# Kolkir/mono_slam_framework

Hardware: AMD Instinct MI355X
Metric: frame-pairs/sec (extract+match) (higher is better)
Workload: dtype u8; 1 GPU; ORB extract+match, 1280x720 pairs, 1024 pairs/GPU/step resident in HBM, ratio 0.60; pairs_per_gpu=1024, width=1280, height=720, synth_mode=0, overflow_pairs=0, ranks=1, rccl_ranks=0

## Files before the change

### include/msf_abi.h

```cpp
#ifndef MSF_ABI_H
#define MSF_ABI_H

#include <stddef.h>
#include <stdint.h>

#ifdef __cplusplus
extern "C" {
#endif

#define MSF_ABI_VERSION 4

typedef struct msf_handle msf_handle;

typedef enum msf_status {
  MSF_OK = 0,
  MSF_ERR_INVALID_ARG = -1,
  MSF_ERR_HIP = -2,
  MSF_ERR_UNSUPPORTED = -3,
  MSF_ERR_CAPACITY = -4,
  MSF_ERR_IO = -5
} msf_status;

typedef enum msf_kind {
  MSF_KIND_ORB = 0,
// ... 4 lines not shown
#define MSF_FLAG_PROFILE 2u
#define MSF_FLAG_KEEP_DEBUG 4u
#define MSF_FLAG_LEVEL_SIZE_MUL_INV 32u
#define MSF_FLAG_NO_FRAME_CACHE 16u
#define MSF_FLAG_FAST_STREAM 64u
#define MSF_FLAG_LOFTR_F32 128u
#define MSF_FLAG_BLUR_SUM256 256u
#define MSF_FLAG_FAST_DENSE 8u

typedef struct msf_config {
  uint32_t struct_size;
  int32_t kind;
  int32_t device;
  float threshold;
  int32_t image_width;
  int32_t image_height;
  int32_t max_batch_pairs;
  uint32_t flags;
  const char* weights_path;
} msf_config;

typedef struct msf_image {
  const uint8_t* data;
  int32_t width, height;
  int64_t stride;
} msf_image;

typedef struct msf_match {
  int32_t x1, y1, x2, y2;
} msf_match;

typedef struct msf_keypoint {
  float x, y;
  float response;
  float angle;
  int32_t octave;
  int32_t lx, ly;
  int32_t fast_score;
} msf_keypoint;

int msf_abi_version(void);
void msf_default_config(msf_config* cfg, int kind);

int msf_weights_info(const char* path, uint64_t* digest, int32_t* n_tensors, int64_t* n_floats);
int msf_convert_weights(const char* src_path, const char* dst_blob_path);

int msf_create(const msf_config* cfg, msf_handle** out);
void msf_destroy(msf_handle* h);
int msf_set_threshold(msf_handle* h, float value);
const char* msf_last_error(const msf_handle* h);

int msf_match_pair(msf_handle* h, const msf_image* a, const msf_image* b,
                   msf_match* out, int32_t cap, int32_t* n_out);
int msf_frame_cache_stats(msf_handle* h, uint64_t* hits, uint64_t* misses, int32_t* capacity);
int msf_match_batch(msf_handle* h, int32_t n_pairs, const msf_image* a, const msf_image* b,
                    msf_match* out, int32_t cap_per_pair, int32_t* n_out);

int msf_match_batch_device(msf_handle* h, int32_t n_pairs, const uint8_t* d_a, const uint8_t* d_b,
                           int64_t frame_stride, int64_t row_stride,
                           msf_match* d_out, int32_t cap_per_pair, int32_t* d_n_out, void* stream);

int msf_extract_device(msf_handle* h, int32_t n_frames, const uint8_t* d_frames, int64_t frame_stride,
                       int64_t row_stride, int32_t first_slot, void* stream);
int msf_match_slots_device(msf_handle* h, int32_t n_pairs, const int32_t* d_slot_a, const int32_t* d_slot_b,
                           msf_match* d_out, int32_t cap_per_pair, int32_t* d_n_out, void* stream);

int msf_set_mappoints(msf_handle* h, int32_t map_slot, const int32_t* keys, int32_t n_keys);
int msf_count_mappoint_matches_device(msf_handle* h, int32_t n_pairs, const msf_match* d_matches,
                                      int32_t cap_per_pair, const int32_t* d_n_matches, const int32_t* d_map_a,
                                      const int32_t* d_map_b, int32_t* d_num_mp, void* stream);

int msf_store_frame(msf_handle* h, int32_t slot, const msf_image* img);
int msf_match_one_to_many(msf_handle* h, int32_t query_slot, int32_t n, const int32_t* slots, int32_t* num_matches,
                          int32_t* num_mp, msf_match* out, int32_t cap_per_pair);

#define MSF_MODEL_HOMOGRAPHY 0
#define MSF_MODEL_FUNDAMENTAL 1
int msf_check_hypotheses(msf_handle* h, int32_t model, int32_t n_hyp, const float* m21, const float* m12,
                         int32_t n_matches, const msf_match* matches, float sigma, float* scores, int32_t* best,
                         uint8_t* best_inliers);

typedef struct msf_ransac_result {
  uint32_t struct_size;
  uint32_t reserved;
  float* m21;
  float* m12;
  float* fn;
  float* null_vec;
  float* scores;
  int32_t* best;
  uint8_t* best_inliers;
  float* T1;
  float* T2;
} msf_ransac_result;
int msf_find_models(msf_handle* h, int32_t n_matches, const msf_match* matches, int32_t n_hyp, const int32_t* sets,
                    float sigma, msf_ransac_result* homography, msf_ransac_result* fundamental);
typedef struct msf_ransac_batch {
  uint32_t struct_size;
  uint32_t reserved;
  int32_t* sets;
  msf_ransac_result homography;
  msf_ransac_result fundamental;
} msf_ransac_batch;
int msf_find_models_device(msf_handle* h, int32_t n_lists, const msf_match* d_matches, int32_t cap_per_pair,
                           const int32_t* d_n_out, int32_t n_hyp, uint64_t seed, float sigma,
                           msf_ransac_batch* out, void* stream);

int msf_render_match_image(msf_handle* h, const msf_image* f1, const msf_image* f2, const msf_match* matches,
                           int32_t n_matches, const uint8_t* has_mp1, const uint8_t* has_mp2, uint8_t* out_rgb,
                           int64_t out_stride);

int msf_pack_matches_device(msf_handle* h, int32_t n_pairs, const msf_match* d_in, int32_t cap_per_pair,
                            const int32_t* d_n_out, msf_match* d_packed, int32_t* d_offsets, void* stream);

typedef struct msf_multi msf_multi;
int msf_multi_create(const msf_config* cfg, int32_t n_devices, const int32_t* device_ids, msf_multi** out);
void msf_multi_destroy(msf_multi* m);
int32_t msf_multi_device_count(const msf_multi* m);
msf_handle* msf_multi_handle(msf_multi* m, int32_t shard);
int msf_multi_set_threshold(msf_multi* m, float value);
const char* msf_multi_last_error(const msf_multi* m);
void msf_multi_shard_range(int32_t n_pairs, int32_t n_shards, int32_t shard, int32_t* first, int32_t* count);
int msf_multi_match_batch(msf_multi* m, int32_t n_pairs, const msf_image* a, const msf_image* b, msf_match* out,
                          int32_t cap_per_pair, int32_t* n_out);
int msf_multi_match_batch_device(msf_multi* m, const int32_t* n_pairs, const uint8_t* const* d_a,
                                 const uint8_t* const* d_b, int64_t frame_stride, int64_t row_stride,
                                 msf_match* const* d_out, int32_t cap_per_pair, int32_t* const* d_n_out);

typedef struct msf_gather msf_gather;
int msf_gather_unique_id(uint8_t* id128);
int msf_gather_create(int32_t device, int32_t rank, int32_t n_ranks, const uint8_t* id128, int32_t pairs_per_rank,
                      int64_t cap_records, msf_gather** out);
void msf_gather_destroy(msf_gather* g);
const char* msf_gather_last_error(const msf_gather* g);
int msf_gather_plan(int32_t n_ranks, int32_t pairs_per_rank, const int32_t* all_offsets, int64_t cap_records,
                    int32_t* totals, int64_t* recv_first);
int msf_gather_matches_device(msf_gather* g, const msf_match* d_packed, const int32_t* d_offsets, int32_t* d_all_offsets,
                              msf_match* d_recv, int32_t* totals, void* stream);


typedef enum msf_debug_what {
  MSF_DBG_LEVEL_SIZES = 0,
  MSF_DBG_LEVEL_PIXELS = 1,
  MSF_DBG_FAST_CANDS = 2,
  MSF_DBG_KEYPOINTS = 3,
  MSF_DBG_DESCRIPTORS = 4,
  MSF_DBG_STAGE1 = 5,
  MSF_DBG_LOFTR_CONF = 6,
  MSF_DBG_LOFTR_FEAT = 7,
  MSF_DBG_FAST_TAU = 8,
  MSF_DBG_WALK_MODE = 10,
  MSF_DBG_LOFTR_ACT = 9,
  MSF_DBG_LOFTR_TOK = 11,
  MSF_DBG_ORB_MATCH_FORM = 12
} msf_debug_what;
int msf_debug_get(msf_handle* h, int32_t what, int32_t slot, int32_t level,
                  void* host_out, size_t cap_bytes, size_t* n_bytes);
int msf_debug_loftr_head(msf_handle* h, int32_t n_pairs, const float* d_feat0, const float* d_feat1,
                         msf_match* d_out, int32_t cap_per_pair, int32_t* d_n_out, void* stream);

int msf_debug_loftr_transformer(msf_handle* h, int32_t n_pairs, int32_t first_block, int32_t n_blocks,
                                const float* d_in0, const float* d_in1, float* d_out0, float* d_out1, void* stream);

int msf_debug_loftr_backbone(msf_handle* h, int32_t n, const uint8_t* d_a, const uint8_t* d_b, int64_t frame_stride,
                             int64_t row_stride, int32_t act_image, float* d_tok_a, float* d_tok_b, void* stream);

int msf_debug_orb_set_features(msf_handle* h, int32_t slot, int32_t n, const msf_keypoint* kp, const uint8_t* desc);

int msf_debug_orb_tail(msf_handle* h, int32_t n_frames, const uint8_t* d_frames, int64_t frame_stride, int64_t row_stride,
                       int32_t first_slot, const int32_t* counts, const int32_t* cands, int32_t form);

int msf_stage_times(msf_handle* h, const char** names, float* ms, int32_t cap);

#ifdef __cplusplus
}
#endif
#endif
```

### mono_slam_framework_amd/_lib.py

```python
import ctypes as C
import os

import numpy as np

from . import build as _build

MSF_OK = 0
MSF_ERR_INVALID_ARG = -1
MSF_ERR_HIP = -2
MSF_ERR_UNSUPPORTED = -3
MSF_ERR_CAPACITY = -4
MSF_ERR_IO = -5

MSF_KIND_ORB = 0
MSF_KIND_LOFTR = 1

MSF_FLAG_BLUR_TIE_HALF_UP = 1
MSF_FLAG_PROFILE = 2
MSF_FLAG_KEEP_DEBUG = 4
MSF_FLAG_FAST_DENSE = 8
MSF_FLAG_NO_FRAME_CACHE = 16
MSF_FLAG_LEVEL_SIZE_MUL_INV = 32
MSF_FLAG_FAST_STREAM = 64
MSF_FLAG_LOFTR_F32 = 128
MSF_FLAG_BLUR_SUM256 = 256

(DBG_LEVEL_SIZES, DBG_LEVEL_PIXELS, DBG_FAST_CANDS, DBG_KEYPOINTS, DBG_DESCRIPTORS, DBG_STAGE1,
 DBG_LOFTR_CONF, DBG_LOFTR_FEAT, DBG_FAST_TAU, DBG_LOFTR_ACT, DBG_WALK_MODE, DBG_LOFTR_TOK,
 DBG_ORB_MATCH_FORM) = range(13)

ABI_SYMBOLS = ["msf_abi_version", "msf_default_config", "msf_create", "msf_destroy", "msf_set_threshold",
               "msf_last_error", "msf_match_pair", "msf_match_batch", "msf_match_batch_device",
               "msf_extract_device", "msf_match_slots_device", "msf_pack_matches_device", "msf_debug_get",
               "msf_debug_loftr_head", "msf_debug_loftr_transformer", "msf_debug_loftr_backbone",
               "msf_debug_orb_set_features", "msf_debug_orb_tail",
               "msf_stage_times", "msf_set_mappoints", "msf_count_mappoint_matches_device",
               "msf_store_frame", "msf_match_one_to_many", "msf_check_hypotheses",
               "msf_find_models", "msf_find_models_device",
               "msf_render_match_image", "msf_weights_info", "msf_convert_weights",
               "msf_frame_cache_stats", "msf_multi_create", "msf_multi_destroy", "msf_multi_device_count",
               "msf_multi_handle", "msf_multi_set_threshold", "msf_multi_last_error", "msf_multi_shard_range",
               "msf_multi_match_batch", "msf_multi_match_batch_device",
               "msf_gather_unique_id", "msf_gather_create", "msf_gather_destroy", "msf_gather_last_error",
               "msf_gather_plan", "msf_gather_matches_device"]

INITIALIZER_SYMBOLS = ["msf_initializer_version", "msf_reconstruct", "msf_reconstruct_device"]

LOCAL_MAPPING_SYMBOLS = ["msf_local_mapping_version", "msf_new_points", "msf_new_points_device", "msf_create_map_points"]

PNP_SYMBOLS = ["msf_pnp_version", "msf_pnp_ransac", "msf_pnp_ransac_device"]

POSE_SYMBOLS = ["msf_pose_version", "msf_pose_optimize", "msf_pose_optimize_device"]

BA_SYMBOLS = ["msf_ba_version", "msf_bundle_adjust", "msf_bundle_adjust_device"]

GLOBAL_BA_SYMBOLS = ["msf_global_ba_version", "msf_global_ba_tile_rows", "msf_global_bundle_adjust",
                     "msf_global_bundle_adjust_device"]
GBA_MAX_FREE_CAMS = 1024

TRACKING_SYMBOLS = ["msf_tracking_version", "msf_frustum", "msf_frustum_device", "msf_claim_points_device",
                    "msf_search_local_points"]
MSF_POINT_BAD, MSF_POINT_SEEN = 1, 2
MSF_SEARCH_KEEP_ON_DEVICE = 1


class Config(C.Structure):
    _fields_ = [("struct_size", C.c_uint32), ("kind", C.c_int32), ("device", C.c_int32), ("threshold", C.c_float),
                ("image_width", C.c_int32), ("image_height", C.c_int32), ("max_batch_pairs", C.c_int32),
                ("flags", C.c_uint32), ("weights_path", C.c_char_p)]


class Image(C.Structure):
    _fields_ = [("data", C.c_void_p), ("width", C.c_int32), ("height", C.c_int32), ("stride", C.c_int64)]


class RansacResult(C.Structure):
    _fields_ = [("struct_size", C.c_uint32), ("reserved", C.c_uint32), ("m21", C.c_void_p), ("m12", C.c_void_p),
                ("fn", C.c_void_p), ("null_vec", C.c_void_p), ("scores", C.c_void_p), ("best", C.c_void_p),
                ("best_inliers", C.c_void_p), ("T1", C.c_void_p), ("T2", C.c_void_p)]


class RansacBatch(C.Structure):
    _fields_ = [("struct_size", C.c_uint32), ("reserved", C.c_uint32), ("sets", C.c_void_p),
                ("homography", RansacResult), ("fundamental", RansacResult)]


class MotionParams(C.Structure):
    _fields_ = [("struct_size", C.c_uint32), ("reserved", C.c_uint32), ("K", C.c_float * 9), ("sigma", C.c_float),
                ("min_triangulated", C.c_int32), ("min_parallax", C.c_float)]


MOTION_ARRAYS = [("ok", "int32", "list", ()), ("model", "int32", "list", ()), ("R21", "float32", "list", (9,)),
                 ("t21", "float32", "list", (3,)), ("points", "float32", "list", ("cap", 3)),
                 ("triangulated", "uint8", "list", ("cap",)), ("n_cand", "int32", "list", ()),
                 ("cand_R", "float32", "list", (8, 9)), ("cand_t", "float32", "list", (8, 3)),
                 ("cand_good", "int32", "list", (8,)), ("cand_parallax", "float32", "list", (8,)),
                 ("winner", "int32", "list", ())]


class MotionResult(C.Structure):
    _fields_ = [("struct_size", C.c_uint32), ("reserved", C.c_uint32)] + [(a[0], C.c_void_p) for a in MOTION_ARRAYS]


class View(C.Structure):
    _fields_ = [("Rcw", C.c_float * 9), ("tcw", C.c_float * 3), ("fx", C.c_float), ("fy", C.c_float),
                ("cx", C.c_float), ("cy", C.c_float)]


class NewPointsParams(C.Structure):
    _fields_ = [("struct_size", C.c_uint32), ("reserved", C.c_uint32), ("max_cos_parallax", C.c_double),
                ("chi2", C.c_double)]


NEW_POINT_DTYPE = np.dtype([("match", "<i4"), ("x", "<f4"), ("y", "<f4"), ("z", "<f4")])
NEW_POINTS_ARRAYS = [("n_new", "int32", "list", ()), ("packed", NEW_POINT_DTYPE, "list", ("cap",)),
                     ("status", "uint8", "list", ("cap",)), ("points", "float32", "list", ("cap", 3)),
                     ("hom", "float32", "list", ("cap", 4)), ("cos_parallax", "float64", "list", ("cap",))]


class NewPointsResult(C.Structure):
    _fields_ = [("struct_size", C.c_uint32), ("reserved", C.c_uint32)] + [(a[0], C.c_void_p) for a in NEW_POINTS_ARRAYS]


class PnpParams(C.Structure):
    _fields_ = [("struct_size", C.c_uint32), ("reserved", C.c_uint32), ("fx", C.c_float), ("fy", C.c_float),
                ("cx", C.c_float), ("cy", C.c_float), ("th2", C.c_float), ("min_inliers", C.c_int32),
                ("n_iterations", C.c_int32), ("max_records", C.c_int32), ("seed", C.c_uint64)]


PNP_ARRAYS = [("n_records", "int32", "list", ()), ("counts", "int32", "hyp", ()),
              ("iteration", "int32", "rec", ()), ("n_inliers", "int32", "rec", ()), ("refined_ok", "int32", "rec", ()),
              ("n_refined", "int32", "rec", ()), ("Tcw_best", "float32", "rec", (12,)), ("Tcw_refined", "float32", "rec", (12,)),
              ("inliers_best", "uint8", "rec", ("cap",)), ("inliers_refined", "uint8", "rec", ("cap",)),
              ("sets", "int32", "hyp", (4,)), ("pose_f64", "float64", "hyp", (12,)), ("cws", "float64", "hyp", (4, 3)),
              ("ut_tail", "float64", "hyp", (4, 12)), ("betas", "float64", "hyp", (3, 4)), ("rep_errors", "float64", "hyp", (3,)),
              ("pca", "float64", "hyp", (3, 3)),
              ("rec_pose_f64", "float64", "rec", (12,)), ("rec_cws", "float64", "rec", (4, 3)),
              ("rec_ut_tail", "float64", "rec", (4, 12)), ("rec_betas", "float64", "rec", (3, 4)),
              ("rec_rep_errors", "float64", "rec", (3,)), ("rec_pca", "float64", "rec", (3, 3))]


class PnpResult(C.Structure):
    _fields_ = [("struct_size", C.c_uint32), ("reserved", C.c_uint32)] + [(a[0], C.c_void_p) for a in PNP_ARRAYS]


def pnp_shapes(lists, n_iterations, max_records, cap):
    lead = {"list": (lists,), "hyp": (lists, n_iterations), "rec": (lists, max_records)}
    return {name: (lead[per] + tuple(cap if t == "cap" else t for t in tail), dt) for name, dt, per, tail in PNP_ARRAYS}


class PoseParams(C.Structure):
    _fields_ = [("struct_size", C.c_uint32), ("reserved", C.c_uint32), ("fx", C.c_float), ("fy", C.c_float),
                ("cx", C.c_float), ("cy", C.c_float), ("chi2", C.c_float)]


POSE_ARRAYS = [("n_good", "int32", "list", ()), ("Tcw", "float32", "list", (12,)), ("outliers", "uint8", "list", ("cap",)),
               ("n_edges", "int32", "list", ()), ("rounds_run", "int32", "list", ()), ("pose_f64", "float64", "list", (12,)),
               ("round_pose_f64", "float64", "round", (12,)), ("round_n_bad", "int32", "round", ()),
               ("round_iterations", "int32", "round", ()),
               ("it_trials", "int32", "it", ()), ("it_lambda_in", "float64", "it", ()), ("it_lambda_out", "float64", "it", ()),
               ("it_cost_in", "float64", "it", ()), ("it_cost_out", "float64", "it", ()), ("it_H", "float64", "it", (21,)),
               ("it_b", "float64", "it", (6,)), ("it_pose_out", "float64", "it", (7,))]


class PoseResult(C.Structure):
    _fields_ = [("struct_size", C.c_uint32), ("reserved", C.c_uint32)] + [(a[0], C.c_void_p) for a in POSE_ARRAYS]


def pose_shapes(lists, cap):
    lead = {"list": (lists,), "round": (lists, 4), "it": (lists, 4, 10)}
    return {name: (lead[per] + tuple(cap if t == "cap" else t for t in tail), dt) for name, dt, per, tail in POSE_ARRAYS}


class BaParams(C.Structure):
    _fields_ = [("struct_size", C.c_uint32), ("reserved", C.c_uint32), ("fx", C.c_float), ("fy", C.c_float),
                ("cx", C.c_float), ("cy", C.c_float), ("n_rounds", C.c_int32), ("iterations", C.c_int32 * 2),
                ("robust", C.c_int32 * 2), ("huber_delta2", C.c_double), ("chi2", C.c_double)]


BA_SLOTS = 64
BA_PROBLEM_DTYPE = np.dtype([("n_cams", "<i4"), ("n_points", "<i4"), ("n_edges", "<i4"), ("cam0", "<i4"), ("point0", "<i4"),
                             ("edge0", "<i4")])
# ... 176 lines not shown
```

### mono_slam_framework_amd/csrc/orb_kernels.hip

```cpp
#include <type_traits>
#include "orb_pipeline.h"

#include <math.h>
#include <stdlib.h>
#include <string.h>

#include "orb_blur_tiles.h"
#include "orb_pattern.h"

namespace msf {

constexpr int SW = TW + 2, SH = TH + 2;
constexpr int kTileCandCap = TW * TH / 4;
constexpr int kTileY0 = kEdge;

constexpr uint32_t kStatusOverflow = 1u;

__constant__ __attribute__((aligned(16))) signed char c_pattern[1024];
__constant__ uint32_t c_disc[2 * kDiscTasks];

__device__ __forceinline__ __amdgpu_buffer_rsrc_t uniform_rsrc(const void* p, uint32_t bytes) {
  const unsigned long long v = (unsigned long long)p;
  const uint32_t lo = (uint32_t)__builtin_amdgcn_readfirstlane((int)(uint32_t)v);
  const uint32_t hi = (uint32_t)__builtin_amdgcn_readfirstlane((int)(uint32_t)(v >> 32));
// ... 233 lines not shown
  const int txlo = max(-1, kLo - x0), txhi = min(TW, L.w - kLo - 1 - x0);
  const bool inner1 = txlo == -1 && txhi == TW && y0 - 1 >= kLo && y0 + TH < L.h - kLo;
  for (int i0 = 0; i0 < GPR * SH; i0 += kFastThreads) {
    const int i = i0 + tid;
    if (i0 + (tid & ~63) >= GPR * SH) continue;
    const int ic = i < GPR * SH ? i : GPR * SH - 1;
    const int sr = ic / GPR, gq = ic % GPR;
    const int ty = sr - 1, tx0 = 4 * gq - 4;
    const int b = ((ty + HY) * PW2 + tx0 + HX) >> 2;
    const uint32_t C = T[b], Lf = T[b - 1], Rt = T[b + 1];
    const uint32_t U = T[b - 3 * (PW2 / 4)], D = T[b + 3 * (PW2 / 4)];
    const uint32_t W3 = __builtin_amdgcn_alignbyte(C, Lf, 1);
    const uint32_t E3 = __builtin_amdgcn_alignbyte(Rt, C, 3);
    const uint32_t nC = ~C;
    const uint32_t l0 = __builtin_amdgcn_lerp(D, nC, 0), l4 = __builtin_amdgcn_lerp(E3, nC, 0);
    const uint32_t l8 = __builtin_amdgcn_lerp(U, nC, 0), l12 = __builtin_amdgcn_lerp(W3, nC, 0);
    const uint32_t b0 = __builtin_amdgcn_lerp(l0, lerp_bright, 0), b4 = __builtin_amdgcn_lerp(l4, lerp_bright, 0);
    const uint32_t b8 = __builtin_amdgcn_lerp(l8, lerp_bright, 0), b12 = __builtin_amdgcn_lerp(l12, lerp_bright, 0);
    const uint32_t n0 = __builtin_amdgcn_lerp(l0, lerp_not_dark, 0), n4 = __builtin_amdgcn_lerp(l4, lerp_not_dark, 0);
    const uint32_t n8 = __builtin_amdgcn_lerp(l8, lerp_not_dark, 0), n12 = __builtin_amdgcn_lerp(l12, lerp_not_dark, 0);
    uint32_t vm = 0;
    if (inner1) {
      vm = gq == 0 ? 0x80000000u : gq == GPR - 1 ? 0x00000080u : 0x80808080u;
      vm = i < GPR * SH ? vm : 0u;
    } else {
      const int gy = y0 + ty;
      int first = txlo - tx0, last = txhi - tx0;
      first = first < 0 ? 0 : first;
      last = last > 3 ? 3 : last;
      if (i < GPR * SH && gy >= kLo && gy < L.h - kLo && first <= last)
        vm = (0x80808080u << (8 * first)) & (0x80808080u >> (8 * (3 - last)));
    }
    const uint32_t cb = ((b0 | b8) & (b4 | b12)) & vm;
    const uint32_t cd = ~((n0 & n8) | (n4 & n12)) & vm;
    if (__ballot((cb | cd) != 0u) == 0ull) continue;
    const uint32_t e0 = (uint32_t)b << 2;
    const uint32_t slots = reserve_packed(__popc(cb) | (__popc(cd) << 16), &S_.nbd, lane);
    uint32_t k = slots & 0xFFFFu;
    if (cb & 0x80u) list1[k++] = (uint16_t)e0;
    if (cb & 0x8000u) list1[k++] = (uint16_t)(e0 + 1);
    if (cb & 0x800000u) list1[k++] = (uint16_t)(e0 + 2);
    if (cb & 0x80000000u) list1[k++] = (uint16_t)(e0 + 3);
    k = kList1Cap - 1 - (slots >> 16);
    if (cd & 0x80u) list1[k--] = (uint16_t)e0;
    if (cd & 0x8000u) list1[k--] = (uint16_t)(e0 + 1);
    if (cd & 0x800000u) list1[k--] = (uint16_t)(e0 + 2);
    if (cd & 0x80000000u) list1[k--] = (uint16_t)(e0 + 3);
  }
  __syncthreads();

  const uint32_t mb = S_.nbd & 0xFFFFu, md = S_.nbd >> 16;
  if (mb | md) {
    for (uint32_t i = tid; i < mb; i += kFastThreads) {
      const int e = list1[i];
      const int s = fast_score_pol<true>(&px[e], tau);
      if (s) sc[SCO + e] = (uint8_t)s;
    }
    for (uint32_t i = tid; i < md; i += kFastThreads) {
      const int e = list1[kList1Cap - 1 - i];
      const int s = fast_score_pol<false>(&px[e], tau);
      if (s) sc[SCO + e] = (uint8_t)s;
    }
    __syncthreads();

    const uint32_t* S = reinterpret_cast<const uint32_t*>(sc) + SCO / 4;
    constexpr int SPD = PW2 / 4;
    const int txlo3 = max(0, kEdge - x0), txhi3 = min(TW - 1, L.w - kEdge - 1 - x0);
    const bool inner3 = txlo3 == 0 && txhi3 == TW - 1;
    for (int i = tid; i < (TW / 4) * TH; i += kFastThreads) {
      const int ty = i / (TW / 4), j = i % (TW / 4);
      const int w = (ty + HY) * SPD + HX / 4 + j;
      const uint32_t C = S[w];
      uint32_t keep = 0;
      const int gy = y0 + ty;
      const bool live = C != 0 && gy >= kEdge && gy < L.h - kEdge;
      if (__ballot(live) == 0ull) continue;
      if (live) {
        const uint32_t Cl = S[w - 1], Cr = S[w + 1];
        const uint32_t U = S[w - SPD], Ul = S[w - SPD - 1], Ur = S[w - SPD + 1];
        const uint32_t D = S[w + SPD], Dl = S[w + SPD - 1], Dr = S[w + SPD + 1];
        keep = __builtin_amdgcn_lerp(C, ~__builtin_amdgcn_alignbyte(C, Cl, 3), 0);
        keep &= __builtin_amdgcn_lerp(C, ~__builtin_amdgcn_alignbyte(Cr, C, 1), 0);
        keep &= __builtin_amdgcn_lerp(C, ~U, 0);
        keep &= __builtin_amdgcn_lerp(C, ~__builtin_amdgcn_alignbyte(U, Ul, 3), 0);
        keep &= __builtin_amdgcn_lerp(C, ~__builtin_amdgcn_alignbyte(Ur, U, 1), 0);
        keep &= __builtin_amdgcn_lerp(C, ~D, 0);
        keep &= __builtin_amdgcn_lerp(C, ~__builtin_amdgcn_alignbyte(D, Dl, 3), 0);
        keep &= __builtin_amdgcn_lerp(C, ~__builtin_amdgcn_alignbyte(Dr, D, 1), 0);
        if (!inner3) {
          int first = txlo3 - 4 * j, last = txhi3 - 4 * j;
          first = first < 0 ? 0 : first;
          last = last > 3 ? 3 : last;
          keep &= first <= last ? (0x80808080u << (8 * first)) & (0x80808080u >> (8 * (3 - last))) : 0u;
        } else {
          keep &= 0x80808080u;
        }
        if (emit_min > 0u) {
          uint32_t ge = 0u;
#pragma unroll
          for (int b = 0; b < 4; b++)
            if (((C >> (8 * b)) & 0xFFu) >= emit_min) ge |= 0x80u << (8 * b);
          keep &= ge;
        }
      }
      const uint32_t mine = __popc(keep);
      uint32_t k = reserve_packed(mine, &S_.lcount, lane);
      const uint32_t key = ((uint32_t)gy << 16) | (uint32_t)(x0 + 4 * j);
      if (keep & 0x80u) llist[k++] = make_uint2(key, C & 0xFFu);
      if (keep & 0x8000u) llist[k++] = make_uint2(key + 1, (C >> 8) & 0xFFu);
      if (keep & 0x800000u) llist[k++] = make_uint2(key + 2, (C >> 16) & 0xFFu);
      if (keep & 0x80000000u) llist[k++] = make_uint2(key + 3, C >> 24);
    }
    __syncthreads();
    const uint32_t n = S_.lcount;
    if (hist) {
      uint32_t* const hl = hist + (size_t)(slot * kOrbLevels + l) * 256u;
      for (uint32_t i = tid; i < n; i += kFastThreads) atomicAdd(&hl[llist[i].y], 1u);
    } else if (n != 0) {
      if (tid == 0) S_.gbase = atomicAdd(&cand_cnt[slot * kOrbLevels + l], n);
      __syncthreads();
      const uint32_t base = S_.gbase;
      const uint2 cm = cmap[slot * kOrbLevels + l];
      uint32_t* outk = cand_key + cm.x;
      uint8_t* outs = cand_sc + cm.x;
      for (uint32_t i = tid; i < n; i += kFastThreads)
        if (base + i < cm.y) {
          const uint2 e = llist[i];
          outk[base + i] = e.x;
          outs[base + i] = (uint8_t)e.y;
        }
    }
  }
}

__global__ __launch_bounds__(kFastThreads) void k_fast(OrbGeometry g, FrameSrc src, const uint8_t* pyr,
                                                       uint32_t* cand_cnt, uint32_t* cand_key, uint8_t* cand_sc,
                                                       const uint2* cmap) {
  __shared__ FastSmem sm;
  int G;
  {
    const uint32_t total = gridDim.x, lin = blockIdx.x;
    const uint32_t xcd = lin & 7u, q = total >> 3, r = total & 7u;
    G = (int)(xcd * q + (xcd < r ? xcd : r) + (lin >> 3));
  }
  const int fi = G / g.total_tiles, bt = G - fi * g.total_tiles;
  int l = 0;
#pragma unroll
  for (int i = 1; i < kOrbLevels; i++)
    if (i < g.nlevels && bt >= g.lv[i].tile_base) l = i;
  fast_tile(g, src, pyr, fi, l, bt - g.lv[l].tile_base, kFastT, cand_cnt, cand_key, cand_sc, cmap, sm);
}

constexpr int kTauBins = 64;
constexpr int kQDone = kTauBins, kQTau = kTauBins + 1, kQFirst = kTauBins + 2, kQAll = kTauBins + 3;
constexpr int kQStat = kTauBins + 4;
constexpr uint32_t kQReady = 0x80000000u;
constexpr int RK = 16;
constexpr int kSGCap = 288, kSPCap = 256, kSHCap = 64, kSOCap = 64;
constexpr uint32_t kSGFlush = 32;
static_assert(kSGCap >= (int)kSGFlush + 256, "record list capacity");
constexpr int kFlushRows = 8;
static_assert(kFlushRows < RK - 5 && kFlushRows % 4 == 0, "ring too short for the flush interval");
constexpr int kTau2MarginPct = 200, kTau2MinStrips = 1;
constexpr int kTau2MarginPctMany = 150, kTau2ManyStrips = 8;

struct StreamSmem {
  __attribute__((aligned(16))) uint8_t px[RK * 256];
  __attribute__((aligned(16))) uint8_t sc[RK * 256];
  uint32_t g[kSGCap];
  uint16_t p[kSPCap];
  uint16_t h[kSHCap];
  uint32_t opk[kSOCap];
};
static_assert(sizeof(StreamSmem) == 10240, "16 waves per CU need 10 240 B per wave");

__device__ __forceinline__ int stream_score(const uint8_t* ring, uint32_t r0, uint32_t x, bool dark, int tau) {
  uint32_t rb[7];
#pragma unroll
  for (int d = 0; d < 7; d++) rb[d] = (((r0 + (uint32_t)(d + RK - 3)) & (uint32_t)(RK - 1)) << 8) + x;
  constexpr int dx[16] = {0, 1, 2, 3, 3, 3, 2, 1, 0, -1, -2, -3, -3, -3, -2, -1};
  constexpr int dy[16] = {3, 3, 2, 1, 0, -1, -2, -3, -3, -3, -2, -1, 0, 1, 2, 3};
  const uint32_t flip = dark ? 255u : 0u;
  int q[16];
#pragma unroll
  for (int k = 0; k < 16; k++) q[k] = (int)((uint32_t)ring[rb[dy[k] + 3] + dx[k]] ^ flip);
  const int v = (int)((uint32_t)ring[rb[3]] ^ flip);
  int m3[16];
#pragma unroll
  for (int k = 0; k < 16; k++) m3[k] = min(min(q[k], q[(k + 1) & 15]), q[(k + 2) & 15]);
  int W = -1;
#pragma unroll
  for (int k = 0; k < 16; k++) W = max(W, min(min(m3[k], m3[(k + 3) & 15]), m3[(k + 6) & 15]));
  const int A = W - v;
  return A > tau ? A - 1 : 0;
}

constexpr uint32_t kSpinMax = 1u << 19;

__device__ __forceinline__ uint32_t ld_agent(const uint32_t* p) {
  return __hip_atomic_load(p, __ATOMIC_RELAXED, __HIP_MEMORY_SCOPE_AGENT);
}
__device__ __forceinline__ void unit_stall(uint32_t* status, int slot, uint32_t* abort_word, int lane) {
  if (lane == 0) {
    atomicOr(&status[slot], kStatusOverflow);
    __hip_atomic_store(abort_word, 1u, __ATOMIC_RELAXED, __HIP_MEMORY_SCOPE_AGENT);
    atomicAdd(abort_word + 1, 1u);
  }
}

template <bool RESIZE>
__device__ __forceinline__ void walk_strip(StreamSmem& sm, const OrbGeometry& g, const FrameSrc& src, uint8_t* pyr,
                                           const uint32_t* __restrict__ tab, uint32_t* qstat, uint32_t* cand_cnt,
                                           uint32_t* cand_key, uint8_t* cand_sc, const uint2* cmap, uint32_t* status,
                                           uint32_t* abort_word, int margin_pct, int dyn, int chain, const int l, const int fi,
                                           const int ts) {
  const int lane = threadIdx.x;
  const bool quarter = (ts & 3) == 0;
  const OrbLevelInfo L = g.lv[l];
  const int slot = src.slot0 + fi, idx = slot * kOrbLevels + l;
  const int sy = ts / L.wk_nx, sx = ts - sy * L.wk_nx;
  uint32_t* const qs = qstat + (size_t)idx * kQStat;
  const int n_strips = L.wk_nx * L.wk_ny;
  const int qa = (n_strips + 3) >> 2;
  const bool count_me = dyn && quarter;

  const int xs = sx * L.wk_px;
  const int xb = xs + 4 * lane;
  const int R0 = sy * L.wk_rows, R1 = min(R0 + L.wk_rows, L.h);
  const int ya = RESIZE ? R0 : max(R0, kEdge), yb = RESIZE ? R1 : min(R1, L.h - kEdge);
  const int ox0 = sx == 0 ? 0 : xs + 4, ox1 = sx == L.wk_nx - 1 ? L.w : xs + 4 + L.wk_px;
  const int y0 = ya - 1;
  int pitch;
  const uint8_t* img = level_ptr(g, src, pyr, fi, l, &pitch);
  const int need_lo = RESIZE ? xs : max(ox0 - 4, xs);
  const int need_hi = sx == L.wk_nx - 1 ? pitch : (RESIZE ? xs + L.wk_px + 16 : ox1 + 4);
  const int xl = min(max(xb, need_lo & ~3), ((need_hi + 3) & ~3) - 4);
  const uint32_t xoff = (uint32_t)(xl + 4 <= pitch ? xl : pitch - 4);
  const int ylim = L.h - 1;
  const uint32_t pitch_u = uniform_u32((uint32_t)pitch);
  const __amdgpu_buffer_rsrc_t img_rs = uniform_rsrc(img, (uint32_t)L.h * (uint32_t)pitch);
#define LOAD_ROW(y_) ((uint32_t)__builtin_amdgcn_raw_buffer_load_b32(img_rs, xoff, (uint32_t)max(min((y_), ylim), 0) * pitch_u, 0))
  const bool early = !(chain && l > 0);
  uint32_t w0_ = 0, w1_ = 0, w2_ = 0, w3_ = 0, w4_ = 0, w5_ = 0, q0 = 0, q1 = 0, q2 = 0, q3 = 0;
  if (early) {
    w0_ = LOAD_ROW(y0 - 3); w1_ = LOAD_ROW(y0 - 2); w2_ = LOAD_ROW(y0 - 1); w3_ = LOAD_ROW(y0); w4_ = LOAD_ROW(y0 + 1);
    w5_ = LOAD_ROW(y0 + 2);
    q0 = LOAD_ROW(y0 + 3); q1 = LOAD_ROW(y0 + 4); q2 = LOAD_ROW(y0 + 5); q3 = LOAD_ROW(y0 + 6);
  }

  const bool need_q = dyn && !quarter && qa >= kTau2MinStrips;
  uint32_t qv = ld_agent(&qs[lane]);
  uint32_t qx = ld_agent(&qs[kTauBins + (lane & 3)]);
  {
    bool ready = false;
    for (uint32_t it = 0; it < kSpinMax; it++) {
      const uint32_t first = (uint32_t)__builtin_amdgcn_readlane((int)qx, kQFirst - kTauBins);
      const uint32_t done = (uint32_t)__builtin_amdgcn_readlane((int)qx, kQDone - kTauBins);
      ready = (first & kQReady) != 0u && (!need_q || done >= (uint32_t)qa);
      if (ready || ld_agent(abort_word) != 0u) break;
      __builtin_amdgcn_s_sleep(20);
      qv = ld_agent(&qs[lane]);
      qx = ld_agent(&qs[kTauBins + (lane & 3)]);
    }
    if (!ready) {
      unit_stall(status, slot, abort_word, lane);
      return;
    }
  }
  if (!early) {
    __builtin_amdgcn_fence(__ATOMIC_ACQUIRE, "agent");
    w0_ = LOAD_ROW(y0 - 3); w1_ = LOAD_ROW(y0 - 2); w2_ = LOAD_ROW(y0 - 1); w3_ = LOAD_ROW(y0); w4_ = LOAD_ROW(y0 + 1);
    w5_ = LOAD_ROW(y0 + 2);
    q0 = LOAD_ROW(y0 + 3); q1 = LOAD_ROW(y0 + 4); q2 = LOAD_ROW(y0 + 5); q3 = LOAD_ROW(y0 + 6);
  }
  int tv = (int)((uint32_t)__builtin_amdgcn_readlane((int)qx, kQFirst - kTauBins) & ~kQReady);
  tv = max(tv, (int)__builtin_amdgcn_readlane((int)qx, kQTau - kTauBins));
  if (need_q && tv > kFastT) {
    uint32_t c = qv;
#pragma unroll
    for (int o = 1; o < 64; o <<= 1) {
      const uint32_t up = __shfl_down(c, o);
      if (lane + o < 64) c += up;
    }
    const uint32_t mp = (qa >= kTau2ManyStrips && margin_pct == kTau2MarginPct) ? (uint32_t)kTau2MarginPctMany : (uint32_t)margin_pct;
    const uint32_t den = 100u * (uint32_t)n_strips;
    const uint32_t need = (mp * 2u * (uint32_t)L.quota * (uint32_t)qa + den - 1u) / den;
    const unsigned long long ok = __ballot(c >= need && 4 * lane >= tv);
    if (ok) {
      const int t2 = 4 * (63 - __builtin_clzll(ok));
      if (t2 > tv) {
        tv = t2;
        if (lane == 0) atomicMax(&qs[kQTau], (uint32_t)t2);
      }
    }
  }
  const bool do_fast = tv > kFastT && L.tiles_x > 0;
  const bool empty = !RESIZE && (!do_fast || ya >= yb || max(ox0, kEdge) >= min(ox1, L.w - kEdge));
  if (!empty) {
  const int r_last = yb - y0;
  const int s_lo = max(0, kEdge - 1 - y0), s_hi = min(r_last, L.h - kEdge - y0);
  const int o_lo = max(1, kEdge - y0), o_hi = min(r_last, L.h - kEdge - y0);
  uint32_t vm = 0, om = 0;
  if (do_fast) {
#pragma unroll
    for (int j = 0; j < 4; j++) {
      const int x = xb + j;
      if (x >= max(ox0 - 1, kEdge - 1) && x < min(ox1 + 1, L.w - (kEdge - 1)) && x >= xs + 3 && x < xs + 253) vm |= 0x80u << (8 * j);
      if (x >= max(ox0, kEdge) && x < min(ox1, L.w - kEdge)) om |= 0x80u << (8 * j);
    }
  }
  const int ox_lo = max(ox0, kEdge), ox_hi = min(ox1, L.w - kEdge);
  const uint32_t lerp_bright = 0x01010101u * (uint32_t)(128 - tv / 2);
  const uint32_t lerp_not_dark = 0x01010101u * (uint32_t)(255 - (254 - tv) / 2);
  uint32_t* const out_cnt = cand_cnt + idx;
  const uint2 cm = cmap[idx];
  uint32_t* const outk = cand_key + cm.x;
  uint8_t* const outs = cand_sc + cm.x;
  const uint32_t out_cap = min(cm.y, (uint32_t)L.cand_cap);
  uint32_t* pxw = reinterpret_cast<uint32_t*>(sm.px);
  uint32_t* scw = reinterpret_cast<uint32_t*>(sm.sc);
  uint8_t* pxb = sm.px;
  uint8_t* scb = sm.sc;

  uint32_t rsel[4] = {0, 0, 0, 0}, rwxp[4] = {0, 0, 0, 0}, roff0 = 0, roff3 = 0, em0 = 0, em1 = 0, em2 = 0, em3 = 0;
  __amdgpu_buffer_rsrc_t dst_rs = img_rs;
  uint32_t dxoff = 0;
  bool rz_lane = false;
  uint32_t dpitch = 0;
  if (RESIZE) {
    const OrbLevelInfo Ld = g.lv[l + 1];
    const int groups = (Ld.w + 3) >> 2;
    const uint4* xsel = reinterpret_cast<const uint4*>(tab + Ld.tab_off);
    const uint4* xwxp = xsel + groups;
    const uint4* xoff = xwxp + groups;
    const uint32_t* yemit = tab + Ld.tab_yemit;
    const int g_first = g.lv[l + 1].wk_xg[sx], g_end = g.lv[l + 1].wk_xg[sx + 1];
    const int gq = min(g_first + lane, groups - 1);
    rz_lane = g_first + lane < g_end;
    const uint4 qsv = xsel[gq], qwv = xwxp[gq], qov = xoff[gq];
    rsel[0] = qsv.x; rsel[1] = qsv.y; rsel[2] = qsv.z; rsel[3] = qsv.w;
    rwxp[0] = qwv.x; rwxp[1] = qwv.y; rwxp[2] = qwv.z; rwxp[3] = qwv.w;
    roff0 = rz_lane ? qov.x - (uint32_t)xs : 0u;
    roff3 = rz_lane ? qov.w - (uint32_t)xs : 0u;
    dpitch = uniform_u32((uint32_t)Ld.pitch);
    dst_rs = uniform_rsrc(pyr + (long long)slot * g.pyr_bytes + Ld.pix_off, (uint32_t)Ld.h * (uint32_t)Ld.pitch);
    dxoff = rz_lane ? 4u * (uint32_t)gq : kRzNoStore;
    const int ra = R0 - 4 + lane, rb = ra + 64;
    if (ra >= R0 && ra < R1) em0 = yemit[ra];
    if (rb >= R0 && rb < R1) em1 = yemit[rb];
    if (rb + 64 >= R0 && rb + 64 < R1) em2 = yemit[rb + 64];
    if (rb + 128 >= R0 && rb + 128 < R1) em3 = yemit[rb + 128];
  }

  uint32_t em_a = em0, em_b = em1;
  int em_k = 0;
  uint32_t nG = 0, nH = 0, nO = 0;
  int nms_lo = 1, last_flush = -1;

#define PUT_ROW(k_, v_)                                                                      \
  do {                                                                                       \
    const int sl_ = (k_) & (RK - 1);                                                         \
    pxw[sl_ * 64 + lane] = (v_);                                                             \
    scw[sl_ * 64 + lane] = 0u;                                                               \
  } while (0)
#define RZ_HSUM(k_, h_)                                                                                                \
  do {                                                                                                                 \
    const uint8_t* rr_ = pxb + (((k_) & (RK - 1)) << 8);                                                               \
    const uint32_t* pa_ = reinterpret_cast<const uint32_t*>(rr_ + roff0);                                              \
    const uint32_t* pb_ = reinterpret_cast<const uint32_t*>(rr_ + roff3);                                              \
    const uint32_t a0_ = pa_[0], a1_ = pa_[1], b0_ = pb_[0], b1_ = pb_[1];                                             \
    h_[0] = udot2_u16(__builtin_amdgcn_perm(a1_, a0_, rsel[0]), rwxp[0], 0u);                                          \
    h_[1] = udot2_u16(__builtin_amdgcn_perm(a1_, a0_, rsel[1]), rwxp[1], 0u);                                          \
    h_[2] = udot2_u16(__builtin_amdgcn_perm(a1_, a0_, rsel[2]), rwxp[2], 0u);                                          \
    h_[3] = udot2_u16(__builtin_amdgcn_perm(b1_, b0_, rsel[3]), rwxp[3], 0u);                                          \
  } while (0)
#define RZ_EMIT(j_, hu_, hl_)                                                                                          \
  do {                                                                                                                 \
    const int jj_ = (j_);                                                                                              \
                                     \
    const uint32_t em_ = (uint32_t)__builtin_amdgcn_readlane((int)((jj_ >> 6) == em_k ? em_a : em_b), jj_ & 63);        \
    const uint32_t wy1_ = (em_ >> 16) & 0x1FFu, wy0_ = 256u - wy1_, rnd_ = 32768u;                                     \
    const uint32_t v0_ = mad_u24_s(hu_[0], wy0_, mad_u24_s(hl_[0], wy1_, rnd_));                                       \
    const uint32_t v1_ = mad_u24_s(hu_[1], wy0_, mad_u24_s(hl_[1], wy1_, rnd_));                                       \
    const uint32_t v2_ = mad_u24_s(hu_[2], wy0_, mad_u24_s(hl_[2], wy1_, rnd_));                                       \
    const uint32_t v3_ = mad_u24_s(hu_[3], wy0_, mad_u24_s(hl_[3], wy1_, rnd_));                                       \
    const uint32_t pk_ = __builtin_amdgcn_perm(v1_, v0_, 0x0c0c0602u) | __builtin_amdgcn_perm(v3_, v2_, 0x06020c0cu);   \
       \
        \
           \
          \
          \
                                                                                     \
    const bool has_ = (int)em_ < 0;                                                                                    \
    __builtin_amdgcn_raw_buffer_store_b32(pk_, dst_rs, dxoff | (has_ ? 0u : kRzNoStore),                                \
                                          (has_ ? em_ & 0xFFFFu : 0u) * dpitch, 16);                                   \
  } while (0)

  auto flush_out = [&]() {
    if (nO == 0) return;
    MSF_WAVE_SYNC();
    uint32_t base = 0;
    if (lane == 0) base = atomicAdd(out_cnt, nO);
    base = __builtin_amdgcn_readfirstlane(base);
    for (uint32_t i = lane; i < nO; i += 64) {
      const uint32_t pk = sm.opk[i], sc_ = pk >> 16;
      if (base + i < out_cap) {
        outk[base + i] = ((uint32_t)(y0 + (int)((pk >> 8) & 255u)) << 16) | (uint32_t)(xs + (int)(pk & 255u));
        outs[base + i] = (uint8_t)sc_;
      }
      if (count_me) atomicAdd(&qs[sc_ >> 2], 1u);
    }
    MSF_WAVE_SYNC();
    nO = 0;
  };

  static_assert(kSOCap >= 32, "output buffer smaller than one half-wave");
  auto emit = [&](bool keep, uint32_t xl, uint32_t rr, uint32_t score) {
    if (__ballot(keep) == 0ull) return;
#pragma unroll
    for (int half = 0; half < 2; half++) {
      const bool kh = keep && (lane >> 5) == half;
      const unsigned long long bal = __ballot(kh);
      if (bal == 0ull) continue;
      const uint32_t cnt = (uint32_t)__popcll(bal);
      if (nO + cnt > (uint32_t)kSOCap) flush_out();
      if (kh) sm.opk[nO + mbcnt64(bal)] = xl | (rr << 8) | (score << 16);
      MSF_WAVE_SYNC();
      nO += cnt;
    }
  };

  auto flush = [&](int s) __attribute__((always_inline)) {
    bool overflow = nH > (uint32_t)kSHCap;
    uint32_t nP = 0;
    auto score_pending = [&]() {
      MSF_WAVE_SYNC();
      for (uint32_t i0 = 0; i0 < nP; i0 += 64) {
        const uint32_t i = i0 + lane;
        int sv = 0;
        uint32_t pe = 0;
        if (i < nP) {
          pe = sm.p[i];
          sv = stream_score(pxb, (pe >> 8) & 15u, pe & 255u, (pe & 0x1000u) != 0u, tv);
          if (sv) scb[pe & 0xFFFu] = (uint8_t)sv;
        }
        const unsigned long long bal = __ballot(sv != 0);
        if (bal) {
          const uint32_t cnt = (uint32_t)__popcll(bal);
          if (overflow || nH + cnt > (uint32_t)kSHCap) overflow = true;
          else {
            if (sv) sm.h[nH + mbcnt64(bal)] = (uint16_t)(pe & 0x0FFFu);
            nH += cnt;
          }
        }
      }
      MSF_WAVE_SYNC();
      nP = 0;
    };
    for (uint32_t c0 = 0; c0 < nG;) {
      uint32_t e0 = 0, mb = 0, md = 0;
      if (c0 + lane < nG) {
        const uint32_t rec = sm.g[c0 + lane];
        e0 = ((rec & 63u) << 2) | ((rec + 0x300u) & 0xF00u);
        mb = rec & 0x80808080u;
        md = (rec << 1) & 0x80808080u;
      }
      const uint32_t mine = __popc(mb) + __popc(md);
      const uint32_t incl = wave_incl_scan(mine);
      uint32_t total = __builtin_amdgcn_readlane(incl, 63), take = 64;
      if (total > (uint32_t)kSPCap) {
        take = 32;
        total = __builtin_amdgcn_readlane(incl, 31);
        if (lane >= 32) mb = md = 0u;
      }
      if (nP + total > (uint32_t)kSPCap) score_pending();
      uint32_t k = nP + incl - mine;
      if (mb & 0x80u) sm.p[k++] = (uint16_t)e0;
      if (mb & 0x8000u) sm.p[k++] = (uint16_t)(e0 + 1);
      if (mb & 0x800000u) sm.p[k++] = (uint16_t)(e0 + 2);
      if (mb & 0x80000000u) sm.p[k++] = (uint16_t)(e0 + 3);
      e0 |= 0x1000u;
      if (md & 0x80u) sm.p[k++] = (uint16_t)e0;
      if (md & 0x8000u) sm.p[k++] = (uint16_t)(e0 + 1);
      if (md & 0x800000u) sm.p[k++] = (uint16_t)(e0 + 2);
      if (md & 0x80000000u) sm.p[k++] = (uint16_t)(e0 + 3);
      nP += total;
      c0 += take;
    }
    score_pending();
    nG = 0;
    const int hi = s - 1;
    if (!overflow) {
      for (uint32_t i0 = 0; i0 < nH; i0 += 64) {
        const uint32_t i = i0 + lane;
        bool keep = false;
        uint32_t key = 0, krr = 0, c = 0;
        if (i < nH) {
          const uint32_t he = sm.h[i];
          const uint32_t xl = he & 255u, row = (he >> 8) & 15u;
          const int rr = nms_lo + (int)((row - (uint32_t)(nms_lo + 3)) & (uint32_t)(RK - 1));
          const uint8_t* qc = scb + (row << 8) + xl;
          const uint8_t* qu = scb + (((row + RK - 1) & (RK - 1)) << 8) + xl;
          const uint8_t* qd = scb + (((row + 1) & (RK - 1)) << 8) + xl;
          c = qc[0];
          const int x = xs + (int)xl;
          keep = rr >= nms_lo && rr <= hi && rr >= o_lo && rr < o_hi && x >= ox_lo && x < ox_hi;
          keep = keep && c > qc[-1] && c > qc[1] && c > qu[-1] && c > qu[0] && c > qu[1] && c > qd[-1] && c > qd[0] &&
                 c > qd[1];
          key = xl;
          krr = (uint32_t)rr;
        }
        emit(keep, key, krr, c);
      }
    } else {
      for (int rr = nms_lo; rr <= hi; rr++) {
        if (rr < o_lo || rr >= o_hi) continue;
        const int row = (rr + 3) & (RK - 1);
        const int w = (row << 6) + lane, wu = (((row + RK - 1) & (RK - 1)) << 6) + lane, wd = (((row + 1) & (RK - 1)) << 6) + lane;
        const uint32_t C = scw[w];
        if (__ballot(C != 0u) == 0ull) continue;
        const uint32_t U = scw[wu], D = scw[wd];
#define SHR1(v_) __builtin_amdgcn_update_dpp(0u, (v_), 0x138, 0xf, 0xf, true)
#define SHL1(v_) __builtin_amdgcn_update_dpp(0u, (v_), 0x130, 0xf, 0xf, true)
        uint32_t keep = __builtin_amdgcn_lerp(C, ~__builtin_amdgcn_alignbyte(C, SHR1(C), 3), 0);
        keep &= __builtin_amdgcn_lerp(C, ~__builtin_amdgcn_alignbyte(SHL1(C), C, 1), 0);
        keep &= __builtin_amdgcn_lerp(C, ~U, 0);
        keep &= __builtin_amdgcn_lerp(C, ~__builtin_amdgcn_alignbyte(U, SHR1(U), 3), 0);
        keep &= __builtin_amdgcn_lerp(C, ~__builtin_amdgcn_alignbyte(SHL1(U), U, 1), 0);
        keep &= __builtin_amdgcn_lerp(C, ~D, 0);
        keep &= __builtin_amdgcn_lerp(C, ~__builtin_amdgcn_alignbyte(D, SHR1(D), 3), 0);
        keep &= __builtin_amdgcn_lerp(C, ~__builtin_amdgcn_alignbyte(SHL1(D), D, 1), 0);
#undef SHR1
#undef SHL1
        keep &= om;
#pragma unroll
        for (int j = 0; j < 4; j++) emit((keep >> (8 * j + 7)) & 1u, (uint32_t)(4 * lane + j), (uint32_t)rr, (C >> (8 * j)) & 255u);
      }
    }
    nH = 0;
    {
      const uint32_t row = (uint32_t)(s + 3) & (RK - 1);
      const uint32_t C = scw[(row << 6) + lane];
      if (__ballot(C != 0u) != 0ull)
#pragma unroll
      for (int j = 0; j < 4; j++) {
        const bool hit = ((C >> (8 * j)) & 255u) != 0u;
        const unsigned long long bal = __ballot(hit);
        if (bal) {
          const uint32_t cnt = (uint32_t)__popcll(bal);
          if (hit && nH + mbcnt64(bal) < (uint32_t)kSHCap) sm.h[nH + mbcnt64(bal)] = (uint16_t)((4u * lane + j) | (row << 8));
          nH += cnt;
        }
      }
    }
    MSF_WAVE_SYNC();
    nms_lo = s;
    last_flush = s;
  };

  PUT_ROW(0, w0_); PUT_ROW(1, w1_); PUT_ROW(2, w2_); PUT_ROW(3, w3_); PUT_ROW(4, w4_); PUT_ROW(5, w5_);
  uint32_t hp[4] = {0, 0, 0, 0};
  if (RESIZE) {
    uint32_t hu[4];
    RZ_HSUM(4, hu);
    RZ_HSUM(5, hp);
    RZ_EMIT(4, hu, hp);
  }
#define STREAM_PRE(C_, D_, bu_, nu_, vmr_, cb_, cd_, b0o_, n0o_)                                                        \
  do {                                                                                                                 \
    const uint32_t Lf_ = __builtin_amdgcn_update_dpp(0u, C_, 0x138, 0xf, 0xf, true);    \
    const uint32_t Rt_ = __builtin_amdgcn_update_dpp(0u, C_, 0x130, 0xf, 0xf, true);    \
    const uint32_t W3_ = __builtin_amdgcn_alignbyte(C_, Lf_, 1);                                                       \
    const uint32_t E3_ = __builtin_amdgcn_alignbyte(Rt_, C_, 3);                                                       \
    const uint32_t nC_ = ~(C_);                                                                                        \
    const uint32_t l0_ = __builtin_amdgcn_lerp(D_, nC_, 0), l4_ = __builtin_amdgcn_lerp(E3_, nC_, 0);                  \
    const uint32_t l12_ = __builtin_amdgcn_lerp(W3_, nC_, 0);                                                          \
    const uint32_t b0_ = __builtin_amdgcn_lerp(l0_, lerp_bright, 0), b4_ = __builtin_amdgcn_lerp(l4_, lerp_bright, 0);     \
    const uint32_t b12_ = __builtin_amdgcn_lerp(l12_, lerp_bright, 0);                                                 \
    const uint32_t n0_ = __builtin_amdgcn_lerp(l0_, lerp_not_dark, 0), n4_ = __builtin_amdgcn_lerp(l4_, lerp_not_dark, 0); \
    const uint32_t n12_ = __builtin_amdgcn_lerp(l12_, lerp_not_dark, 0);                                               \
    cb_ = ((b0_ | ~(nu_)) & (b4_ | b12_)) & (vmr_);                                                                    \
    cd_ = ~((n0_ & ~(bu_)) | (n4_ & n12_)) & (vmr_);                                                                   \
    b0o_ = b0_;                                                                                                        \
    n0o_ = n0_;                                                                                                        \
  } while (0)
#define STREAM_PRE_DOWN(C_, D_, b0o_, n0o_)                                                                            \
  do {                                                                                                                 \
    const uint32_t l0_ = __builtin_amdgcn_lerp(D_, ~(C_), 0);                                                          \
    b0o_ = __builtin_amdgcn_lerp(l0_, lerp_bright, 0);                                                                 \
    n0o_ = __builtin_amdgcn_lerp(l0_, lerp_not_dark, 0);                                                               \
  } while (0)
#define STREAM_APPEND(s_, cb_, cd_)                                                                                    \
  do {                                                                                                                 \
    const bool has_ = ((cb_) | (cd_)) != 0u;                                                                           \
    const unsigned long long bal_ = __ballot(has_);                                                                    \
    if (bal_) {                                                                                                        \
       \
      if (has_) sm.g[nG + mbcnt64(bal_)] = (cb_) | ((cd_) >> 1) | lane_rec | ((((uint32_t)(s_) & 63u) << 8) | (((uint32_t)(s_) >> 6) << 16)); \
      nG += (uint32_t)__popcll(bal_);                                                                                  \
    }                                                                                                                  \
  } while (0)
  const uint32_t lane_rec = (uint32_t)lane;
  static_assert(kWkMaxRows + 12 < 256, "rel rows: 8 bits in a buffered corner, 4 x 64 emit entries");
  static_assert(RK == 16, "the group body below exists in four copies, one per position of the group in the 16-row ring");
  uint32_t pb1, pn1, pb2, pn2, pb3, pn3;
  STREAM_PRE_DOWN(w0_, w3_, pb1, pn1);
  STREAM_PRE_DOWN(w1_, w4_, pb2, pn2);
  STREAM_PRE_DOWN(w2_, w5_, pb3, pn3);
  auto group = [&](auto ph_, const int s) __attribute__((always_inline)) {
    constexpr int P_ = decltype(ph_)::value * 4;
    if (RESIZE && ((s + 5) >> 6) != em_k) {
      em_k++;
      em_a = em_b;
      em_b = em_k == 1 ? em2 : em_k == 2 ? em3 : 0u;
    }
    const uint32_t d0 = q0, d1 = q1, d2 = q2, d3 = q3;
    PUT_ROW(P_ + 6, d0); q0 = LOAD_ROW(y0 + s + 7);
    PUT_ROW(P_ + 7, d1); q1 = LOAD_ROW(y0 + s + 8);
    PUT_ROW(P_ + 8, d2); q2 = LOAD_ROW(y0 + s + 9);
    PUT_ROW(P_ + 9, d3); q3 = LOAD_ROW(y0 + s + 10);
    const uint32_t c0 = pxw[((P_ + 3) & (RK - 1)) * 64 + lane];
    const uint32_t c1 = pxw[((P_ + 4) & (RK - 1)) * 64 + lane], c2 = pxw[((P_ + 5) & (RK - 1)) * 64 + lane];
    if (RESIZE) {
      uint32_t ha[4], hb[4], hc[4], hd[4];
      RZ_HSUM(P_ + 6, ha);
      RZ_HSUM(P_ + 7, hb);
      RZ_HSUM(P_ + 8, hc);
      RZ_HSUM(P_ + 9, hd);
      RZ_EMIT(s + 5, hp, ha);
      RZ_EMIT(s + 6, ha, hb);
      RZ_EMIT(s + 7, hb, hc);
      RZ_EMIT(s + 8, hc, hd);
#pragma unroll
      for (int k = 0; k < 4; k++) hp[k] = hd[k];
    }
    uint32_t cb0, cd0, cb1, cd1, cb2, cd2, cb3, cd3;
    uint32_t vm0 = vm, vm1 = vm, vm2 = vm, vm3 = vm;
    if (s < s_lo || s + 3 > s_hi) {
      vm0 = (s >= s_lo && s <= s_hi) ? vm : 0u;
      vm1 = (s + 1 >= s_lo && s + 1 <= s_hi) ? vm : 0u;
      vm2 = (s + 2 >= s_lo && s + 2 <= s_hi) ? vm : 0u;
      vm3 = (s + 3 >= s_lo && s + 3 <= s_hi) ? vm : 0u;
    }
    uint32_t rb0, rn0;
    STREAM_PRE(c0, d0, pb1, pn1, vm0, cb0, cd0, rb0, rn0);
    STREAM_PRE(c1, d1, pb2, pn2, vm1, cb1, cd1, pb1, pn1);
    STREAM_PRE(c2, d2, pb3, pn3, vm2, cb2, cd2, pb2, pn2);
    STREAM_PRE(d0, d3, rb0, rn0, vm3, cb3, cd3, pb3, pn3);
    STREAM_APPEND(s, cb0, cd0);
    STREAM_APPEND(s + 1, cb1, cd1);
    STREAM_APPEND(s + 2, cb2, cd2);
    STREAM_APPEND(s + 3, cb3, cd3);
  };
  auto after = [&](const int s) __attribute__((always_inline)) {
    const int sl = min(s + 3, r_last);
    if (do_fast && (nG > kSGFlush || sl - last_flush >= kFlushRows || sl == r_last)) {
      MSF_WAVE_SYNC();
      flush(sl);
    }
    return s + 4 > r_last;
  };
  if (r_last >= 0)
    for (int s = 0;; s += 16) {
      group(std::integral_constant<int, 0>{}, s);
      if (after(s)) break;
      group(std::integral_constant<int, 1>{}, s + 4);
      if (after(s + 4)) break;
      group(std::integral_constant<int, 2>{}, s + 8);
      if (after(s + 8)) break;
      group(std::integral_constant<int, 3>{}, s + 12);
      if (after(s + 12)) break;
    }
#undef STREAM_PRE
#undef STREAM_PRE_DOWN
#undef STREAM_APPEND
  flush_out();
#undef LOAD_ROW
#undef PUT_ROW
#undef RZ_HSUM
#undef RZ_EMIT
  }
  if (count_me || RESIZE) {
    asm volatile("s_waitcnt vmcnt(0)" ::: "memory");
    if (lane == 0) {
      if (count_me) atomicAdd(&qs[kQDone], 1u);
      if (RESIZE) atomicAdd(&qs[kQAll], 1u);
    }
  }
}

constexpr int kTauMinHits = 24;
constexpr int kTauOversample = 10;

__device__ __forceinline__ int fast_score_px(const uint8_t* p, int pitch) {
  const int off[16][2] = {{0, 3}, {1, 3}, {2, 2}, {3, 1}, {3, 0}, {3, -1}, {2, -2}, {1, -3},
                          {0, -3}, {-1, -3}, {-2, -2}, {-3, -1}, {-3, 0}, {-3, 1}, {-2, 2}, {-1, 3}};
  int q[16];
#pragma unroll
  for (int k = 0; k < 16; k++) q[k] = (int)p[off[k][1] * pitch + off[k][0]];
  int mn3[16], mx3[16];
#pragma unroll
  for (int k = 0; k < 16; k++) {
    mn3[k] = min(min(q[k], q[(k + 1) & 15]), q[(k + 2) & 15]);
    mx3[k] = max(max(q[k], q[(k + 1) & 15]), q[(k + 2) & 15]);
  }
  int Wb = -1, Wd = 1000;
#pragma unroll
  for (int k = 0; k < 16; k++) {
    Wb = max(Wb, min(min(mn3[k], mn3[(k + 3) & 15]), mn3[(k + 6) & 15]));
    Wd = min(Wd, max(max(mx3[k], mx3[(k + 3) & 15]), mx3[(k + 6) & 15]));
  }
  const int v = p[0];
  const int A = max(Wb - v, v - Wd);
  return A > kFastT ? A - 1 : 0;
}

__device__ __forceinline__ uint32_t hash_u32(uint32_t x) {
  x ^= x >> 16; x *= 0x7feb352du; x ^= x >> 15; x *= 0x846ca68bu; x ^= x >> 16;
  return x;
}

constexpr int kTauPre = 40, kTauPreHigh = 64;
constexpr int kTauListCap = 2048;
struct TauSmem {
  uint32_t hist[kTauBins];
  uint32_t nlist, pad[3];
  uint32_t list[kTauListCap];
};
static_assert(sizeof(TauSmem) <= sizeof(StreamSmem), "the threshold unit works in the walker's LDS block");

__device__ __forceinline__ void tau_unit(TauSmem& T, const OrbGeometry& g, const FrameSrc& src, const uint8_t* pyr,
                                         uint32_t* tau, uint32_t* tau_first, uint32_t* redo_cnt, uint32_t* redo_list,
                                         uint32_t* qstat, uint32_t* status, uint32_t* abort_word, int force_tau,
                                         int predict_pct, int chain, const int l, const int fi) {
  const int lane = threadIdx.x, slot = src.slot0 + fi, idx = slot * kOrbLevels + l;
  const OrbLevelInfo L = g.lv[l];
  uint32_t* const qs = qstat + (size_t)idx * kQStat;
  int tv = kFastT, pre_used = kTauPre, predicted = 0;
  if (chain && l > 0) {
    const OrbLevelInfo Lp = g.lv[l - 1];
    const uint32_t* pq = qstat + (size_t)(idx - 1) * kQStat;
    const int n_prev = Lp.wk_nx * Lp.wk_ny, qa = (n_prev + 3) >> 2;
    uint32_t pv = ld_agent(&pq[lane]);
    uint32_t px = ld_agent(&pq[kTauBins + (lane & 3)]);
    bool ready = false;
    for (uint32_t it = 0; it < kSpinMax; it++) {
      ready = (uint32_t)__builtin_amdgcn_readlane((int)px, kQAll - kTauBins) >= (uint32_t)n_prev;
      if (ready || ld_agent(abort_word) != 0u) break;
      __builtin_amdgcn_s_sleep(20);
      pv = ld_agent(&pq[lane]);
      px = ld_agent(&pq[kTauBins + (lane & 3)]);
    }
    if (!ready) {
      unit_stall(status, slot, abort_word, lane);
      return;
    }
    __builtin_amdgcn_fence(__ATOMIC_ACQUIRE, "agent");
    if (predict_pct > 0 && force_tau == 0 && L.tiles_x > 0) {
      const uint32_t done = (uint32_t)__builtin_amdgcn_readlane((int)px, kQDone - kTauBins);
      const uint32_t t_q = (uint32_t)__builtin_amdgcn_readlane((int)px, kQFirst - kTauBins) & ~kQReady;
      uint32_t c = pv;
#pragma unroll
      for (int o = 1; o < 64; o <<= 1) {
        const uint32_t up = __shfl_down(c, o);
        if (lane + o < 64) c += up;
      }
      if (qa >= kTau2MinStrips && done >= (uint32_t)qa && t_q > (uint32_t)kFastT) {
        const long long a_prev = (long long)(Lp.w - 2 * kEdge) * (Lp.h - 2 * kEdge), a_cur = (long long)(L.w - 2 * kEdge) * (L.h - 2 * kEdge);
        const long long need = ((long long)predict_pct * 2 * L.quota * a_prev * qa + 100ll * a_cur * n_prev - 1) / (100ll * a_cur * n_prev);
        const unsigned long long ok = __ballot((long long)c >= need && 4u * (uint32_t)lane >= t_q);
        if (ok) predicted = 4 * (63 - __builtin_clzll(ok));
      }
    }
  }
  if (predicted > kFastT) {
    tv = predicted;
  } else if (force_tau > 0) {
    tv = force_tau;
  } else if (L.samp_rows > 0) {
    if (lane < kTauBins) T.hist[lane] = 0;
    if (lane == 0) T.nlist = 0;
    MSF_WAVE_SYNC();
    int pitch;
    const uint8_t* img = level_ptr(g, src, pyr, fi, l, &pitch);
    const int rh = L.h - 2 * kEdge;
    const uint32_t factor_px = (uint32_t)(L.samp_sx * L.samp_sy);
    uint32_t need_hits = ((uint32_t)kTauOversample * 2u * (uint32_t)L.quota + factor_px - 1u) / factor_px;
    need_hits = need_hits < (uint32_t)kTauMinHits ? (uint32_t)kTauMinHits : need_hits;
    int pre = kTauPreHigh;
    for (int attempt = 0; attempt < 2; attempt++) {
      const uint32_t lb = 0x01010101u * (uint32_t)(128 - pre / 2), lnd = 0x01010101u * (uint32_t)(255 - (254 - pre) / 2);
      const int x_first = (kEdge + 3) & ~3;
      const int n_dw = (L.w - kEdge - x_first) >> 2;
      for (int j0 = 0; j0 < L.samp_rows; j0 += 4) {
        for (int k = lane; k < L.samp_cols; k += 64) {
          uint32_t Cv[4], Lv[4], Rv[4], Uv[4], Dv[4], pos[4];
#pragma unroll
          for (int u = 0; u < 4; u++) {
            const int j = min(j0 + u, L.samp_rows - 1);
            const uint32_t hj = hash_u32((uint32_t)(l * 4099 + j) * 2654435761u + 12345u);
            int y = j * L.samp_sy + (int)(hj % (uint32_t)L.samp_sy);
            y = kEdge + (y < rh ? y : rh - 1);
            int d = k * L.samp_sx + (int)((hj >> 16) % (uint32_t)L.samp_sx);
            d = d < n_dw ? d : n_dw - 1;
            const int x = x_first + 4 * d;
            const uint8_t* p = img + (long long)y * pitch + x;
            Cv[u] = *reinterpret_cast<const uint32_t*>(p);
            Lv[u] = *reinterpret_cast<const uint32_t*>(p - 4);
            Rv[u] = *reinterpret_cast<const uint32_t*>(p + 4);
            Uv[u] = *reinterpret_cast<const uint32_t*>(p - 3 * pitch);
            Dv[u] = *reinterpret_cast<const uint32_t*>(p + 3 * pitch);
            pos[u] = ((uint32_t)y << 16) | (uint32_t)x;
          }
#pragma unroll
          for (int u = 0; u < 4; u++) {
            const uint32_t W3 = __builtin_amdgcn_alignbyte(Cv[u], Lv[u], 1), E3 = __builtin_amdgcn_alignbyte(Rv[u], Cv[u], 3);
            const uint32_t nC = ~Cv[u];
            const uint32_t l0 = __builtin_amdgcn_lerp(Dv[u], nC, 0), l4 = __builtin_amdgcn_lerp(E3, nC, 0);
            const uint32_t l8 = __builtin_amdgcn_lerp(Uv[u], nC, 0), l12 = __builtin_amdgcn_lerp(W3, nC, 0);
            const uint32_t cb = (__builtin_amdgcn_lerp(l0, lb, 0) | __builtin_amdgcn_lerp(l8, lb, 0)) &
                                (__builtin_amdgcn_lerp(l4, lb, 0) | __builtin_amdgcn_lerp(l12, lb, 0));
            const uint32_t cd = ~((__builtin_amdgcn_lerp(l0, lnd, 0) & __builtin_amdgcn_lerp(l8, lnd, 0)) |
                                  (__builtin_amdgcn_lerp(l4, lnd, 0) & __builtin_amdgcn_lerp(l12, lnd, 0)));
            uint32_t m = (cb | cd) & 0x80808080u;
            if (j0 + u >= L.samp_rows) m = 0u;
            if (m) {
              const uint32_t idx0 = atomicAdd(&T.nlist, (uint32_t)__popc(m));
              uint32_t q = idx0;
#pragma unroll
              for (int b4 = 0; b4 < 4; b4++)
                if ((m >> (8 * b4 + 7)) & 1u) {
                  if (q < (uint32_t)kTauListCap) T.list[q] = pos[u] + (uint32_t)b4;
                  q++;
                }
            }
          }
        }
      }
      MSF_WAVE_SYNC();
      if (attempt == 1 || T.nlist >= 6u * need_hits) break;
      MSF_WAVE_SYNC();
      if (lane == 0) T.nlist = 0;
      pre = kTauPre;
      MSF_WAVE_SYNC();
    }
    pre_used = pre;
    const uint32_t n = min(T.nlist, (uint32_t)kTauListCap);
    for (uint32_t i = lane; i < n; i += 64) {
      const uint32_t e = T.list[i];
      const int sc = fast_score_px(img + (long long)(e >> 16) * pitch + (e & 0xFFFFu), pitch);
      if (sc >= pre_used) atomicAdd(&T.hist[sc >> 2], 1u);
    }
    MSF_WAVE_SYNC();
    {
      uint32_t c = T.hist[lane];
#pragma unroll
      for (int o = 1; o < 64; o <<= 1) {
        const uint32_t up = __shfl_down(c, o);
        if (lane + o < 64) c += up;
      }
      const unsigned long long ok = __ballot(c >= need_hits && 4 * lane >= pre_used);
      const int top = ok ? 63 - __builtin_clzll(ok) : 0;
      tv = ok ? 4 * top : kFastT;
    }
    MSF_WAVE_SYNC();
  }
  if (lane == 0) {
    tau[idx] = (uint32_t)tv;
    tau_first[idx] = (uint32_t)tv;
    if (tv <= kFastT && L.tiles_x > 0) redo_list[atomicAdd(redo_cnt, 1u)] = (uint32_t)(fi * kOrbLevels + l);
    __hip_atomic_store(&qs[kQFirst], kQReady | (uint32_t)tv, __ATOMIC_RELAXED, __HIP_MEMORY_SCOPE_AGENT);
  }
}

__global__ __launch_bounds__(64) void k_walk(OrbGeometry g, FrameSrc src, uint8_t* pyr, const uint32_t* __restrict__ tab,
                                             uint32_t* tau, uint32_t* tau_first, uint32_t* qstat, uint32_t* cand_cnt,
                                             uint32_t* cand_key, uint8_t* cand_sc, const uint2* cmap,
                                             uint32_t* redo_cnt, uint32_t* redo_list,
                                             uint32_t* status, uint32_t* abort_word, int l_lo, int l_hi, int n_frames,
                                             int margin_pct, int dyn, int force_tau, int predict_pct, int chain,
                                             int resize_mask, int test_stall_frame) {
  __shared__ StreamSmem sm;
  const int xcd = (int)(blockIdx.x & 7u);
  int r = (int)(blockIdx.x >> 3);
  const int nf8 = n_frames >> 3, nrem = n_frames & 7;
  const int nfx = nf8 + (xcd < nrem ? 1 : 0), f0 = xcd * nf8 + (xcd < nrem ? xcd : nrem);
  int l = l_lo, S = 0;
  for (;; l++) {
    if (l > l_hi) return;
    S = g.lv[l].wk_nx * g.lv[l].wk_ny;
    const int units = nfx * (1 + S);
    if (r < units) break;
    r -= units;
  }
  if (r < nfx) {
    if (f0 + r == test_stall_frame && l == 3) return;
    tau_unit(*reinterpret_cast<TauSmem*>(&sm), g, src, pyr, tau, tau_first, redo_cnt, redo_list, qstat, status, abort_word,
             force_tau, predict_pct, chain, l, f0 + r);
    return;
  }
  r -= nfx;
  const int Sq = (S + 3) >> 2, Sr = S - Sq;
  int fi, ts;
  if (r < nfx * Sq) {
    fi = f0 + r / Sq;
    ts = 4 * (r % Sq);
  } else {
    r -= nfx * Sq;
    fi = f0 + r / Sr;
    const int ip = r % Sr;
    ts = 4 * (ip / 3) + ip % 3 + 1;
  }
  if ((resize_mask >> l) & 1)
    walk_strip<true>(sm, g, src, pyr, tab, qstat, cand_cnt, cand_key, cand_sc, cmap, status, abort_word, margin_pct, dyn, chain, l, fi, ts);
  else
    walk_strip<false>(sm, g, src, pyr, tab, qstat, cand_cnt, cand_key, cand_sc, cmap, status, abort_word, margin_pct, dyn, chain, l, fi, ts);
}

__global__ __launch_bounds__(64) void k_fast_check(OrbGeometry g, int slot0, int n_frames, uint32_t* tau, uint32_t* tau_first,
                                                   uint32_t* cand_cnt, const uint8_t* cand_sc, const uint2* cmap,
                                                   uint32_t* redo_cnt, uint32_t* redo_list, const uint32_t* qstat) {
  const int fi = blockIdx.x / kOrbLevels, l = blockIdx.x - fi * kOrbLevels, lane = threadIdx.x;
  if (fi >= n_frames || l >= g.nlevels) return;
  const int idx = (slot0 + fi) * kOrbLevels + l;
  if (tau[idx] <= (uint32_t)kFastT) return;
  const uint32_t T = max(tau[idx], qstat[(size_t)idx * kQStat + kQTau]);
  const OrbLevelInfo L = g.lv[l];
  const uint2 cm = cmap[idx];
  const bool over = cand_cnt[idx] > cm.y;
  const uint32_t n = min(cand_cnt[idx], cm.y);
  const uint8_t* scs = cand_sc + cm.x;
  uint32_t found = 0;
  for (uint32_t i = 16u * lane; i < n; i += 16u * 64u) {
    const uint4 v = *reinterpret_cast<const uint4*>(scs + i);
    const uint32_t w[4] = {v.x, v.y, v.z, v.w};
#pragma unroll
    for (int b = 0; b < 16; b++)
      if (i + b < n && ((w[b >> 2] >> (8 * (b & 3))) & 255u) >= T) found++;
  }
#pragma unroll
  for (int o = 32; o >= 1; o >>= 1) found += __shfl_xor(found, o);
  if (lane == 0) {
    if (over || found < 2u * (uint32_t)L.quota) {
      tau[idx] = kFastT;
      cand_cnt[idx] = 0;
      redo_list[atomicAdd(redo_cnt, 1u)] = (uint32_t)(fi * kOrbLevels + l);
    } else {
      tau[idx] = T;
      tau_first[idx] = T;
    }
  }
}

__global__ __launch_bounds__(kFastThreads) void k_fast_redo(OrbGeometry g, FrameSrc src, const uint8_t* pyr,
                                                            const uint32_t* __restrict__ redo_cnt,
                                                            const uint32_t* __restrict__ redo_list, int max_tiles,
                                                            uint32_t* cand_cnt, uint32_t* cand_key, uint8_t* cand_sc,
                                                            const uint2* cmap, uint32_t* hist, const uint32_t* emit_thr) {
  __shared__ FastSmem sm;
  const uint32_t n = *redo_cnt;
  const unsigned long long units = (unsigned long long)n * (unsigned)max_tiles;
  const unsigned long long per_xcd = (units + 7ull) >> 3;
  const unsigned long long u_begin = (blockIdx.x & 7u) * per_xcd;
  const unsigned long long u_end = u_begin + per_xcd < units ? u_begin + per_xcd : units;
  for (unsigned long long u = u_begin + (blockIdx.x >> 3); u < u_end; u += (gridDim.x >> 3)) {
    const uint32_t item = redo_list[u / (unsigned)max_tiles];
    const int t = (int)(u % (unsigned)max_tiles);
    const int fi = (int)(item / kOrbLevels), l = (int)(item % kOrbLevels);
    if (t >= g.lv[l].tiles_x * g.lv[l].tiles_y) continue;
    uint32_t emit_min = 0u;
    if (emit_thr) {
      emit_min = emit_thr[(src.slot0 + fi) * kOrbLevels + l];
      if (emit_min > 255u) continue;
    }
    fast_tile(g, src, pyr, fi, l, t, kFastT, cand_cnt, cand_key, cand_sc, cmap, sm, hist, emit_min);
    __syncthreads();
  }
}

__global__ __launch_bounds__(64) void k_redo_thr(OrbGeometry g, int slot0, const uint32_t* __restrict__ redo_cnt,
                                                 const uint32_t* __restrict__ redo_list, const uint2* cmap, uint32_t* hist,
                                                 uint32_t* emit_thr) {
  const uint32_t n = *redo_cnt;
  const int lane = threadIdx.x;
  for (uint32_t q = blockIdx.x; q < n; q += gridDim.x) {
    const uint32_t item = redo_list[q];
    const int fi = (int)(item / kOrbLevels), l = (int)(item % kOrbLevels);
    const int idx = (slot0 + fi) * kOrbLevels + l;
    uint4* const hl = reinterpret_cast<uint4*>(hist + (size_t)idx * 256u);
    const uint4 hv = hl[lane];
    hl[lane] = make_uint4(0u, 0u, 0u, 0u);
    const uint32_t keep = 2u * (uint32_t)g.lv[l].quota;
    uint32_t above = hv.x + hv.y + hv.z + hv.w;
#pragma unroll
    for (int o = 1; o < 64; o <<= 1) {
      const uint32_t up = __shfl_down(above, o);
      if (lane + o < 64) above += up;
    }
    const uint32_t total = __shfl(above, 0);
    above -= hv.x + hv.y + hv.z + hv.w;
    const uint32_t c3 = above + hv.w, c2 = c3 + hv.z, c1 = c2 + hv.y, c0 = c1 + hv.x;
    const int mine = c3 >= keep ? 4 * lane + 3 : c2 >= keep ? 4 * lane + 2 : c1 >= keep ? 4 * lane + 1 : c0 >= keep ? 4 * lane : -1;
    const unsigned long long ok = __ballot(mine >= 0);
    uint32_t thr = 0;
    if (total > keep && total > cmap[idx].y) {
      thr = 256;
      if (keep > 0 && ok) thr = (uint32_t)__shfl(mine, 63 - __builtin_clzll(ok));
    }
    if (lane == 0) emit_thr[idx] = thr;
  }
}

__device__ __forceinline__ float harris_at(const uint8_t* img, int step, int x0, int y0) {
  const int xb = (x0 - 4) & ~3;
  const uint32_t o = (uint32_t)(x0 - 4) & 3u;
  const uint8_t* base = img + (long long)(y0 - 4) * step + xb;
  constexpr int kWG = 0x000100FF;
  constexpr int kWH = 0x00010201;
  int Gm2[7], Gm1[7], Hm2[7], Hm1[7];
  int a = 0, b = 0, c = 0;
#pragma unroll
  for (int t = 0; t < 9; t++) {
    const uint32_t* rp = reinterpret_cast<const uint32_t*>(base + (long long)t * step);
    const uint32_t d0 = rp[0] ^ 0x80808080u, d1 = rp[1] ^ 0x80808080u, d2 = rp[2] ^ 0x80808080u;
    const uint32_t w0 = __builtin_amdgcn_alignbyte(d1, d0, o);
    const uint32_t w1 = __builtin_amdgcn_alignbyte(d2, d1, o);
    const uint32_t w2 = d2 >> (8u * o);
    const uint32_t win[7] = {w0, __builtin_amdgcn_alignbyte(w1, w0, 1), __builtin_amdgcn_alignbyte(w1, w0, 2),
                             __builtin_amdgcn_alignbyte(w1, w0, 3), w1, __builtin_amdgcn_alignbyte(w2, w1, 1),
                             __builtin_amdgcn_alignbyte(w2, w1, 2)};
    int G[7], H[7];
#pragma unroll
    for (int j = 0; j < 7; j++) {
      G[j] = __builtin_amdgcn_sdot4((int)win[j], kWG, 0, false);
      H[j] = __builtin_amdgcn_sdot4((int)win[j], kWH, 0, false);
    }
    if (t >= 2) {
#pragma unroll
      for (int j = 0; j < 7; j++) {
        const int Ix = Gm2[j] + 2 * Gm1[j] + G[j];
        const int Iy = H[j] - Hm2[j];
        a += Ix * Ix;
        b += Iy * Iy;
        c += Ix * Iy;
      }
    }
#pragma unroll
    for (int j = 0; j < 7; j++) { Gm2[j] = Gm1[j]; Gm1[j] = G[j]; Hm2[j] = Hm1[j]; Hm1[j] = H[j]; }
  }
  const float scale = 1.f / ((1 << 2) * 7 * 255.f);
  const float scale_sq_sq = scale * scale * scale * scale;
  const float fa = (float)a, fb = (float)b, fc = (float)c;
  return (fa * fb - fc * fc - 0.04f * (fa + fb) * (fa + fb)) * scale_sq_sq;
}

__global__ __launch_bounds__(256) void k_thr_harris(OrbGeometry g, FrameSrc src, const uint8_t* pyr,
                                                    const uint32_t* cand_cnt, const uint32_t* cand_key,
                                                    const uint8_t* cand_sc, const uint2* cmap,
                                                    uint32_t* s1_cnt, uint4* s1, uint32_t* status, int do_harris) {
  __shared__ uint32_t hist[256];
  __shared__ uint32_t thr_s, lcount;
  const int l = blockIdx.x, fi = blockIdx.y, slot = src.slot0 + fi, tid = threadIdx.x;
  const uint32_t nt = blockDim.x;
  if (l >= g.nlevels) return;
  const OrbLevelInfo L = g.lv[l];
  uint32_t n = cand_cnt[slot * kOrbLevels + l];
  const uint2 cm = cmap[slot * kOrbLevels + l];
  if (n > cm.y) {
    if (tid == 0) atomicOr(&status[slot], kStatusOverflow);
    n = cm.y;
  }
  const uint32_t* keys = cand_key + cm.x;
  const uint8_t* scs = cand_sc + cm.x;
  uint4* out = s1 + (long long)slot * g.s1_total + L.s1_off;
  for (uint32_t b = tid; b < 256u; b += nt) hist[b] = 0;
  if (tid == 0) lcount = 0;
  __syncthreads();
  for (uint32_t i = 16u * tid; i < n; i += 16u * nt) {
    const uint4 v = *reinterpret_cast<const uint4*>(scs + i);
    const uint32_t w[4] = {v.x, v.y, v.z, v.w};
#pragma unroll
    for (int b = 0; b < 16; b++)
      if (i + b < n) atomicAdd(&hist[(w[b >> 2] >> (8 * (b & 3))) & 255u], 1u);
  }
  __syncthreads();
  if (tid < 64) {
    const uint32_t keep = 2u * (uint32_t)L.quota;
    const uint32_t h0 = hist[4 * tid], h1 = hist[4 * tid + 1], h2 = hist[4 * tid + 2], h3 = hist[4 * tid + 3];
    uint32_t above = h0 + h1 + h2 + h3;
#pragma unroll
    for (int o = 1; o < 64; o <<= 1) {
      const uint32_t up = __shfl_down(above, o);
      if (tid + o < 64) above += up;
    }
    above -= h0 + h1 + h2 + h3;
    const uint32_t c3 = above + h3, c2 = c3 + h2, c1 = c2 + h1, c0 = c1 + h0;
    const int mine = c3 >= keep ? 4 * tid + 3 : c2 >= keep ? 4 * tid + 2 : c1 >= keep ? 4 * tid + 1 : c0 >= keep ? 4 * tid : -1;
    const unsigned long long ok = __ballot(mine >= 0);
    uint32_t thr = 0;
    if (n > keep) {
      thr = 256;
      if (keep > 0 && ok) thr = (uint32_t)__shfl(mine, 63 - __builtin_clzll(ok));
    }
    if (tid == 0) thr_s = thr;
  }
  __syncthreads();
  const uint32_t thr = thr_s;
  int pitch;
  const uint8_t* img = level_ptr(g, src, pyr, fi, l, &pitch);
  for (uint32_t i0 = 0; i0 < n; i0 += 16u * nt) {
    const uint32_t i = i0 + 16u * tid;
    uint32_t mask = 0;
    uint4 v = make_uint4(0u, 0u, 0u, 0u);
    if (i < n) {
      v = *reinterpret_cast<const uint4*>(scs + i);
      const uint32_t w[4] = {v.x, v.y, v.z, v.w};
#pragma unroll
      for (int b = 0; b < 16; b++)
        if (i + b < n && ((w[b >> 2] >> (8 * (b & 3))) & 255u) >= thr) mask |= 1u << b;
    }
    if (__ballot(mask != 0u) == 0ull) continue;
    uint32_t k = reserve_packed(__popc(mask), &lcount, tid & 63);
    const uint32_t w[4] = {v.x, v.y, v.z, v.w};
    while (mask) {
      const int b = __ffs(mask) - 1;
      mask &= mask - 1;
      if (k < (uint32_t)kS1Cap)
        out[k] = make_uint4(keys[i + b], 0u, (w[b >> 2] >> (8 * (b & 3))) & 255u, 0u);
      k++;
    }
  }
  __syncthreads();
  const uint32_t kept = !do_harris ? 0u : min(lcount, (uint32_t)kS1Cap);
  for (uint32_t i = tid; i < kept; i += nt) {
    const uint32_t key = out[i].x;
    const float r = harris_at(img, pitch, key & 0xFFFF, key >> 16);
    out[i].y = __float_as_uint(r);
  }
  __syncthreads();
  if (tid == 0) {
    uint32_t m = lcount;
    if (m > (uint32_t)kS1Cap) { atomicOr(&status[slot], kStatusOverflow); m = kS1Cap; }
    s1_cnt[slot * kOrbLevels + l] = m;
  }
}

__global__ __launch_bounds__(256) void k_harris_flat(OrbGeometry g, FrameSrc src, const uint8_t* pyr, HarrisUnits hw,
                                                     const uint32_t* __restrict__ s1_cnt, uint4* s1) {
  const int fi = blockIdx.y, slot = src.slot0 + fi, lane = threadIdx.x & 63;
  const int u = blockIdx.x * 4 + (threadIdx.x >> 6);
  if (u >= hw.base[g.nlevels]) return;
  int l = 0;
#pragma unroll
  for (int i = 1; i < kOrbLevels; i++)
    if (i < g.nlevels && u >= hw.base[i]) l = i;
  const OrbLevelInfo L = g.lv[l];
  const uint32_t kept = min(s1_cnt[slot * kOrbLevels + l], (uint32_t)kS1Cap);
  uint4* out = s1 + (long long)slot * g.s1_total + L.s1_off;
  int pitch;
  const uint8_t* img = level_ptr(g, src, pyr, fi, l, &pitch);
  const uint32_t step = 64u * (uint32_t)hw.n[l];
  for (uint32_t i = 64u * (uint32_t)(u - hw.base[l]) + lane; i < kept; i += step) {
    const uint32_t key = out[i].x;
    out[i].y = __float_as_uint(harris_at(img, pitch, key & 0xFFFF, key >> 16));
  }
}

constexpr int kSelCap = kKpCap;
__global__ __launch_bounds__(256) void k_select(OrbGeometry g, int slot0, const uint32_t* s1_cnt, const uint4* s1,
                                                msf_keypoint* kp, uint32_t* kp_cnt, uint32_t* status) {
  __shared__ uint4 kept[kSelCap];
  constexpr int kRespCap = 4096;
  __shared__ __attribute__((aligned(16))) float resp[kRespCap];
  __shared__ __attribute__((aligned(16))) uint32_t keys[kSelCap];
  __shared__ uint32_t nkept;
  const int slot = slot0 + blockIdx.x, tid = threadIdx.x;
  msf_keypoint* out = kp + (long long)slot * kKpCap;
  uint32_t base = 0;
  bool overflow = false;
  for (int l = 0; l < g.nlevels; l++) {
    const OrbLevelInfo L = g.lv[l];
    const uint32_t n = s1_cnt[slot * kOrbLevels + l];
    const uint4* in = s1 + (long long)slot * g.s1_total + L.s1_off;
    const uint32_t keep = (uint32_t)L.quota;
    if (tid == 0) nkept = 0;
    const bool staged = n > keep && n <= (uint32_t)kRespCap;
    const uint32_t n4 = (n + 3) >> 2;
    if (staged)
      for (uint32_t i = tid; i < 4 * n4; i += 256) resp[i] = i < n ? __uint_as_float(in[i].y) : -INFINITY;
    __syncthreads();
    for (uint32_t i = tid; i < n; i += 256) {
      const uint4 e = in[i];
      bool k = true;
      if (n > keep) {
        const float v = __uint_as_float(e.y);
        uint32_t greater = 0;
        if (staged) {
          const float4* r4 = reinterpret_cast<const float4*>(resp);
          for (uint32_t j = 0; j < n4; j++) {
            const float4 r = r4[j];
            greater += (uint32_t)(r.x > v) + (uint32_t)(r.y > v) + (uint32_t)(r.z > v) + (uint32_t)(r.w > v);
          }
        } else {
          for (uint32_t j = 0; j < n; j++) greater += (__uint_as_float(in[j].y) > v) ? 1u : 0u;
        }
        k = greater < keep;
      }
      if (k) {
        const uint32_t q = atomicAdd(&nkept, 1u);
        if (q < (uint32_t)kSelCap) kept[q] = e;
      }
    }
    __syncthreads();
    uint32_t m = nkept;
    if (m > (uint32_t)kSelCap) { overflow = true; m = kSelCap; }
    if (base + m > (uint32_t)kKpCap) { overflow = true; m = kKpCap - base; }
    const uint32_t m4 = (m + 3) >> 2;
    for (uint32_t i = tid; i < 4 * m4; i += 256) keys[i] = i < m ? kept[i].x : 0xFFFFFFFFu;
    __syncthreads();
    for (uint32_t i = tid; i < m; i += 256) {
      const uint4 e = kept[i];
      uint32_t rank = 0;
      const uint4* k4 = reinterpret_cast<const uint4*>(keys);
      for (uint32_t j = 0; j < m4; j++) {
        const uint4 kk = k4[j];
        rank += (uint32_t)(kk.x < e.x) + (uint32_t)(kk.y < e.x) + (uint32_t)(kk.z < e.x) + (uint32_t)(kk.w < e.x);
      }
      msf_keypoint k;
      k.lx = e.x & 0xFFFF;
      k.ly = e.x >> 16;
      k.x = (float)k.lx * L.scale;
      k.y = (float)k.ly * L.scale;
      k.response = __uint_as_float(e.y);
      k.angle = -1.f;
      k.octave = l;
      k.fast_score = (int)e.z;
      out[base + rank] = k;
    }
    base += m;
    __syncthreads();
  }
  if (tid == 0) {
    kp_cnt[slot] = base;
    if (overflow) atomicOr(&status[slot], kStatusOverflow);
  }
}

__device__ __forceinline__ float fast_atan2_deg(float y, float x) {
  const float k = (float)(180.0 / 3.14159265358979323846);
  const float p1 = 0.9997878412794807f * k, p3 = -0.3258083974640975f * k, p5 = 0.1555786518463281f * k,
              p7 = -0.04432655554792128f * k;
  const float ax = fabsf(x), ay = fabsf(y);
  float a, c, c2;
  if (ax >= ay) {
    c = ay / (ax + (float)2.2204460492503131e-16);
    c2 = c * c;
    a = (((p7 * c2 + p5) * c2 + p3) * c2 + p1) * c;
  } else {
    c = ax / (ay + (float)2.2204460492503131e-16);
    c2 = c * c;
    a = 90.f - (((p7 * c2 + p5) * c2 + p3) * c2 + p1) * c;
  }
  if (x < 0) a = 180.f - a;
  if (y < 0) a = 360.f - a;
  return a;
}

__device__ __forceinline__ void det_sincosf(float t, float* s, float* c) {
  const double x = (double)t;
  const int k = (int)(x * 6.36619772367581382433e-01 + 0.5);
  const double kd = (double)k;
  const double r = (x - kd * 1.57079632673412561417e+00) - kd * 6.07710050650619224932e-11;
  const double z = r * r;
  double p = 1.58969099521155010221e-10;
  p = p * z + -2.50507602534068634195e-08;
  p = p * z + 2.75573137070700676789e-06;
  p = p * z + -1.98412698298579493134e-04;
  p = p * z + 8.33333333332248946124e-03;
  p = p * z + -1.66666666666666324348e-01;
  const double sr = r + (r * z) * p;
  double q = -1.13596475577881948265e-11;
  q = q * z + 2.08757232129817482790e-09;
  q = q * z + -2.75573143513906633035e-07;
  q = q * z + 2.48015872894767294178e-05;
  q = q * z + -1.38888888888741095749e-03;
  q = q * z + 4.16666666666666019037e-02;
  const double cr = (1.0 - 0.5 * z) + (z * z) * q;
  double sv, cv;
  switch (k & 3) {
    case 0: sv = sr; cv = cr; break;
    case 1: sv = cr; cv = -sr; break;
    case 2: sv = -sr; cv = -cr; break;
    default: sv = -cr; cv = sr; break;
  }
  *s = (float)sv;
  *c = (float)cv;
}

constexpr int PR = 22;
constexpr int PD = 2 * PR + 1;
constexpr int PP = blur_tiles::kRawPitch;
constexpr int HP = blur_tiles::kHbCols;
constexpr int HC = blur_tiles::kHbPitch;
static_assert(PD == blur_tiles::kRawRows && PD * (PP / 4) == blur_tiles::kFetchLoads * blur_tiles::kFetchLanes, "patch fetch");
typedef int v4i_t __attribute__((ext_vector_type(4)));

template <bool HALF_UP, bool SUM256>
__global__ __launch_bounds__(256) void k_describe(OrbGeometry g, FrameSrc src, const uint8_t* pyr,
// ... 210 lines not shown
    const bool pass = have_q && n2 >= 2 && ((float)d0 < ratio * (float)d1);
    const unsigned long long bal = __ballot(pass);
    const uint32_t before = __popcll(bal & ((1ull << lane) - 1ull));
    if (lane == 0) wave_cnt[wave] = __popcll(bal);
    __syncthreads();
    uint32_t off = running;
    for (int w = 0; w < wave; w++) off += wave_cnt[w];
    if (pass) {
      const uint32_t idx = off + before;
      if (idx < (uint32_t)cap) {
        msf_match m;
        m.x1 = (int)ka[q].x; m.y1 = (int)ka[q].y;
        m.x2 = (int)kb[i0].x; m.y2 = (int)kb[i0].y;
        o[idx] = m;
      }
    }
    __syncthreads();
    if (tid == 0) running += wave_cnt[0] + wave_cnt[1] + wave_cnt[2] + wave_cnt[3];
    __syncthreads();
  }
  if (tid == 0) n_out[pair] = (int32_t)running;
}

constexpr int kSplitBlocks = kKpCap / 64;
constexpr int kSplitMaxPairs = 128;
__global__ __launch_bounds__(256) void k_match_split(int n_pairs, const int32_t* slot_a, const int32_t* slot_b,
                                                     const msf_keypoint* kp, const uint32_t* kp_cnt,
                                                     const uint8_t* desc, const uint32_t* status, float ratio,
                                                     msf_match* out, int cap, int32_t* n_out, int chunk,
                                                     uint32_t* qres, uint32_t* done, int slot_base, int max_slots) {
  __shared__ __attribute__((aligned(16))) unsigned long long train[kTrainChunk * 4];
  __shared__ int part[3][4][64];
  __shared__ uint32_t wave_cnt[4];
  __shared__ uint32_t running, last_s;
  const int pair = blockIdx.y, qb = blockIdx.x, tid = threadIdx.x, lane = tid & 63, wave = tid >> 6;
  const int sa = slot_a ? slot_a[pair] : slot_base + pair;
  const int sb = slot_b ? slot_b[pair] : slot_base + n_pairs + pair;
  if (sa < 0 || sa >= max_slots || sb < 0 || sb >= max_slots || ((status[sa] | status[sb]) & kStatusOverflow)) {
    if (qb == 0 && tid == 0) n_out[pair] = -1;
    return;
  }
  const uint32_t n1 = min(kp_cnt[sa], (uint32_t)kKpCap), n2 = min(kp_cnt[sb], (uint32_t)kKpCap);
  const unsigned long long* tsrc = reinterpret_cast<const unsigned long long*>(desc + (long long)sb * kKpCap * 32);
  uint32_t* qr = qres + (long long)pair * kKpCap;
  const uint32_t q = (uint32_t)qb * 64u + lane;
  if ((uint32_t)qb * 64u < n1) {
    const bool have_q = q < n1;
    unsigned long long q0w = 0, q1w = 0, q2w = 0, q3w = 0;
    if (have_q) {
      const unsigned long long* qd = reinterpret_cast<const unsigned long long*>(desc + ((long long)sa * kKpCap + q) * 32);
      q0w = qd[0]; q1w = qd[1]; q2w = qd[2]; q3w = qd[3];
    }
    int d0 = 0x7fffffff, d1 = 0x7fffffff, i0 = 0x7fffffff;
    for (uint32_t t0 = 0; t0 < n2; t0 += chunk) {
      const uint32_t tn = min(n2 - t0, (uint32_t)chunk);
      __syncthreads();
      for (uint32_t i = tid; i < tn * 4; i += 256) train[i] = tsrc[(size_t)t0 * 4 + i];
      __syncthreads();
      const uint32_t ta = (tn * wave) >> 2, tb = (tn * (wave + 1)) >> 2;
      for (uint32_t t = ta; t < tb; t++) {
        const unsigned long long* tr = &train[t * 4];
        const int d = __popcll(q0w ^ tr[0]) + __popcll(q1w ^ tr[1]) + __popcll(q2w ^ tr[2]) + __popcll(q3w ^ tr[3]);
        if (d < d1) {
          if (d < d0) { d1 = d0; d0 = d; i0 = (int)(t0 + t); }
          else d1 = d;
        }
      }
    }
    part[0][wave][lane] = d0;
    part[1][wave][lane] = i0;
    part[2][wave][lane] = d1;
    __syncthreads();
    if (wave == 0) {
      int b0 = 0x7fffffff, bi = 0x7fffffff, b1 = 0x7fffffff;
#pragma unroll
      for (int w = 0; w < 4; w++) {
        const int e0 = part[0][w][lane], ei = part[1][w][lane], e1 = part[2][w][lane];
        if (e0 < b0 || (e0 == b0 && ei < bi)) { b1 = min(b0, e1); b0 = e0; bi = ei; }
        else b1 = min(b1, e0);
        b1 = min(b1, e1);
      }
      const bool pass = have_q && n2 >= 2 && ((float)b0 < ratio * (float)b1);
      if (have_q) qr[q] = pass ? (0x80000000u | (uint32_t)bi) : 0u;
    }
  }
  __threadfence();
  __syncthreads();
  if (tid == 0) last_s = atomicAdd(&done[pair], 1u) == (uint32_t)gridDim.x - 1u;
  __syncthreads();
  if (!last_s) return;
  __threadfence();
  if (tid == 0) { running = 0; done[pair] = 0; }
  __syncthreads();
  const msf_keypoint* ka = kp + (long long)sa * kKpCap;
  const msf_keypoint* kb = kp + (long long)sb * kKpCap;
  msf_match* o = out + (long long)pair * cap;
  for (uint32_t q0 = 0; q0 < n1; q0 += 256) {
    const uint32_t qq = q0 + tid;
    const uint32_t r = qq < n1 ? __hip_atomic_load(&qr[qq], __ATOMIC_RELAXED, __HIP_MEMORY_SCOPE_AGENT) : 0u;
    const bool pass = (r & 0x80000000u) != 0u;
    const unsigned long long bal = __ballot(pass);
    const uint32_t before = __popcll(bal & ((1ull << lane) - 1ull));
    if (lane == 0) wave_cnt[wave] = __popcll(bal);
    __syncthreads();
    uint32_t off = running;
    for (int w = 0; w < wave; w++) off += wave_cnt[w];
    if (pass) {
      const uint32_t idx = off + before;
      if (idx < (uint32_t)cap) {
        const uint32_t t = r & 0x7fffffffu;
        msf_match m;
        m.x1 = (int)ka[qq].x; m.y1 = (int)ka[qq].y;
        m.x2 = (int)kb[t].x; m.y2 = (int)kb[t].y;
        o[idx] = m;
      }
    }
    __syncthreads();
    if (tid == 0) running += wave_cnt[0] + wave_cnt[1] + wave_cnt[2] + wave_cnt[3];
    __syncthreads();
  }
  if (tid == 0) n_out[pair] = (int32_t)running;
}

OrbPipeline::~OrbPipeline() { destroy(); }

void OrbPipeline::destroy() {
  if (h_walk_abort_) hipHostFree(h_walk_abort_);
  h_walk_abort_ = nullptr;
  for (auto& set : evr_)
    for (auto& e : set.ev) {
      if (e) hipEventDestroy(e);
      e = nullptr;
    }
  ev_ok_ = false;
}

#define MSF_HIP_TRY(expr)                                                                 \
  do {                                                                                    \
    hipError_t e_ = (expr);                                                               \
    if (e_ != hipSuccess) return std::string(#expr) + ": " + hipGetErrorString(e_);       \
  } while (0)

void OrbPipeline::read_env() {
  if (const char* e = getenv("MSF_ORB_FAST_TAU")) {
    const int v = atoi(e) & ~1;
    if (v >= kFastT && v <= 254) force_tau_ = v;
  }
  if (const char* e = getenv("MSF_ORB_RESIZE_GENERIC")) resize_generic_ = atoi(e) != 0;
  if (const char* e = getenv("MSF_ORB_FAST_ONE_PART")) fast_two_part_ = atoi(e) == 0;
  if (const char* e = getenv("MSF_ORB_UNFUSED")) fused_ = atoi(e) == 0;
  if (getenv("MSF_TEST_HOOKS"))
    if (const char* e = getenv("MSF_ORB_TEST_STALL_FRAME")) test_stall_frame_ = atoi(e);
  if (const char* e = getenv("MSF_ORB_WALK_PER_LEVEL")) walk_per_level_ = atoi(e) != 0;
  if (const char* e = getenv("MSF_ORB_TAU_PREDICT")) {
    const int v = atoi(e);
    if (v >= 0 && v <= 2000) tau_predict_pct_ = v;
  }
  tau2_margin_pct_ = kTau2MarginPct;
  if (const char* e = getenv("MSF_ORB_TAU2_MARGIN_PCT")) {
    const int v = atoi(e);
    if (v >= 1 && v <= 10000) tau2_margin_pct_ = v;
  }
}

std::string OrbPipeline::init(const OrbOptions& o) {
  max_slots_ = o.max_slots;
  half_up_ = o.blur_half_up;
  blur_sum256_ = o.blur_sum256;
  profile_ = o.profile;
  force_tau_ = o.dense_fast ? kFastT : 0;
  stream_min_frames_ = o.stream_min_frames;
  read_env();

  OrbPlanRequest rq;
  rq.width = o.width;
  rq.height = o.height;
  rq.max_slots = o.max_slots;
  rq.work_frames = o.work_frames;
  rq.level_size_mul_inv = o.level_size_mul_inv;
  rq.resize_generic = resize_generic_;
  rq.force_tau = force_tau_;
  rq.stream_min_frames = stream_min_frames_;
  OrbPlan plan;
  const std::string err = plan_orb(rq, &plan);
  if (!err.empty()) return err;
  g_ = plan.g;
  prim_ = plan.prim;
  harris_ = plan.harris;
  work_frames_ = plan.work_frames;
  for (int l = 0; l < kOrbLevels; l++) resize_shared_[l] = plan.resize_shared[l];

  const OrbGeometry& g = g_;
  const size_t S = (size_t)max_slots_, Wk = (size_t)work_frames_;
  const size_t total = (size_t)(g.pool_base + (long long)g.pool_entries);
  MSF_HIP_TRY(d_pyr_.reserve(Wk * g.pyr_bytes));
  MSF_HIP_TRY(d_tab_.reserve(plan.tab.size() * sizeof(uint32_t)));
  MSF_HIP_TRY(hipMemcpy(d_tab_, plan.tab.data(), plan.tab.size() * sizeof(uint32_t), hipMemcpyHostToDevice));
  MSF_HIP_TRY(d_cand_cnt_.reserve(Wk * kOrbLevels * sizeof(uint32_t)));
  MSF_HIP_TRY(d_tau_.reserve(2 * Wk * kOrbLevels * sizeof(uint32_t)));
  MSF_HIP_TRY(hipMemset(d_tau_, 0, 2 * Wk * kOrbLevels * sizeof(uint32_t)));
  MSF_HIP_TRY(d_redo_.reserve((1 + Wk * kOrbLevels) * sizeof(uint32_t)));
  MSF_HIP_TRY(d_redo_hist_.reserve(Wk * kOrbLevels * 256 * sizeof(uint32_t)));
  MSF_HIP_TRY(hipMemset(d_redo_hist_, 0, Wk * kOrbLevels * 256 * sizeof(uint32_t)));
  MSF_HIP_TRY(d_redo_thr_.reserve(Wk * kOrbLevels * sizeof(uint32_t)));
  MSF_HIP_TRY(d_qstat_.reserve(Wk * kOrbLevels * kQStat * sizeof(uint32_t)));
  MSF_HIP_TRY(hipMemset(d_qstat_, 0, Wk * kOrbLevels * kQStat * sizeof(uint32_t)));
  MSF_HIP_TRY(d_cand_.reserve(total * sizeof(uint32_t)));
  MSF_HIP_TRY(d_cand_sc_.reserve(total));
  MSF_HIP_TRY(d_cmap_.reserve(Wk * kOrbLevels * sizeof(uint2)));
  MSF_HIP_TRY(hipMemset(d_cmap_, 0, Wk * kOrbLevels * sizeof(uint2)));
  MSF_HIP_TRY(d_walk_abort_.reserve(16));
  MSF_HIP_TRY(hipMemset(d_walk_abort_, 0, 16));
  MSF_HIP_TRY(hipHostMalloc(&h_walk_abort_, 16, hipHostMallocDefault));
  h_walk_abort_[0] = h_walk_abort_[1] = 0u;
  MSF_HIP_TRY(d_s1_cnt_.reserve(Wk * kOrbLevels * sizeof(uint32_t)));
  MSF_HIP_TRY(d_s1_.reserve(Wk * g.s1_total * sizeof(uint4)));
  MSF_HIP_TRY(d_kp_.reserve(S * kKpCap * sizeof(msf_keypoint)));
  MSF_HIP_TRY(d_desc_.reserve(S * kKpCap * 32));
  MSF_HIP_TRY(d_kp_cnt_.reserve(S * sizeof(uint32_t)));
  MSF_HIP_TRY(d_status_.reserve(S * sizeof(uint32_t)));
  MSF_HIP_TRY(d_qres_.reserve((size_t)kSplitMaxPairs * kKpCap * sizeof(uint32_t)));
  MSF_HIP_TRY(d_done_.reserve((size_t)kSplitMaxPairs * sizeof(uint32_t)));
  MSF_HIP_TRY(hipMemset(d_done_, 0, (size_t)kSplitMaxPairs * sizeof(uint32_t)));
  MSF_HIP_TRY(hipMemset(d_kp_cnt_, 0, S * sizeof(uint32_t)));
  MSF_HIP_TRY(hipMemset(d_status_, 0, S * sizeof(uint32_t)));
  MSF_HIP_TRY(hipMemset(d_cand_cnt_, 0, Wk * kOrbLevels * sizeof(uint32_t)));
  MSF_HIP_TRY(hipMemset(d_s1_cnt_, 0, Wk * kOrbLevels * sizeof(uint32_t)));
  MSF_HIP_TRY(hipMemcpyToSymbol(HIP_SYMBOL(c_pattern), k_orb_bit_pattern_31, 1024));
  MSF_HIP_TRY(hipMemcpyToSymbol(HIP_SYMBOL(c_disc), plan.disc.data(), sizeof(uint32_t) * 2 * kDiscTasks));
  if (profile_) {
    for (auto& set : evr_)
      for (auto& e : set.ev) MSF_HIP_TRY(hipEventCreate(&e));
    ev_ok_ = true;
  }
  return "";
}

__global__ __launch_bounds__(256) void k_fill_u32(uint32_t* a, uint32_t* b, uint32_t v, int n) {
  const int i = blockIdx.x * 256 + threadIdx.x;
  if (i < n) { a[i] = v; b[i] = v; }
}

hipError_t OrbPipeline::extract(const FrameSrc& src, int n, hipStream_t st) {
  if (n <= 0) return hipSuccess;
  if (src.slot0 < 0 || src.slot0 + n > max_slots_ || n > work_frames_) return hipErrorInvalidValue;
  last_src_ = src;
  last_n_ = n;
  if (h_walk_abort_ && !walk_per_level_ && __atomic_load_n(&h_walk_abort_[1], __ATOMIC_RELAXED) != 0u) {
    walk_per_level_ = true;
    degraded_note_ = true;
  }
  if (test_stall_frame_ >= 0 && test_stall_calls_++ > 0) test_stall_frame_ = -1;
  if (ev_ok_) ev_begin_call();
  const hipError_t e = extract_range(src, n, st, ev_ok_ ? ev_ : nullptr);
  if (ev_ok_) ev_extract_pending_ = true;
  return e;
}

hipError_t OrbPipeline::extract_range(const FrameSrc& src, int n, hipStream_t st, hipEvent_t* evs) {
  const OrbGeometry& g = g_;
  hipError_t e;
  const ptrdiff_t back = (ptrdiff_t)src.slot0;
  uint8_t* const d_pyr_ = this->d_pyr_ - back * g.pyr_bytes;
  uint32_t* const d_cand_cnt_ = this->d_cand_cnt_ - back * kOrbLevels;
  uint2* const d_cmap_ = this->d_cmap_ - back * kOrbLevels;
  uint32_t* const d_qstat_ = this->d_qstat_ - back * kOrbLevels * kQStat;
  uint32_t* const d_redo_hist_ = this->d_redo_hist_ - back * kOrbLevels * 256;
  uint32_t* const d_redo_thr_ = this->d_redo_thr_ - back * kOrbLevels;
  if ((e = hipMemsetAsync(this->d_cand_cnt_, 0, (size_t)n * kOrbLevels * 4, st))) return e;
  if ((e = hipMemsetAsync(d_status_ + src.slot0, 0, (size_t)n * 4, st))) return e;
  if ((e = hipMemsetAsync(d_redo_, 0, 4, st))) return e;
  if (evs) hipEventRecord(evs[0], st);
  uint32_t* tau = d_tau_ - back * kOrbLevels;
  uint32_t* tau_first = d_tau_ + (ptrdiff_t)work_frames_ * kOrbLevels - back * kOrbLevels;
  const int force_tau = call_force_tau(n);
  const bool dense = force_tau == kFastT;
  if (dense && (long long)n * g.cand_total > (long long)g.pool_entries) return hipErrorInvalidValue;
  hipLaunchKernelGGL(k_cand_reset, dim3((n * kOrbLevels + 255) / 256), dim3(256), 0, st, g, prim_, this->d_cmap_, n, dense ? 1 : 0);
  const int dyn = (fast_two_part_ && force_tau == 0) ? 1 : 0;
  bool fused = fused_ && !dense && g.total_tiles > 0;
  for (int l = 1; l < g.nlevels; l++) fused = fused && g.lv[l].wk_fused != 0;
  auto launch_walk = [&](int l_lo, int l_hi, int chain, int resize_mask, int predict_pct) {
    long long per_frame = 0;
    for (int l = l_lo; l <= l_hi; l++) per_frame += 1 + g.lv[l].wk_nx * g.lv[l].wk_ny;
    const long long wgs = 8ll * ((n + 7) / 8) * per_frame;
    hipLaunchKernelGGL(k_walk, dim3((unsigned)wgs), dim3(64), 0, st, g, src, d_pyr_, d_tab_, tau, tau_first, d_qstat_,
                       d_cand_cnt_, d_cand_, d_cand_sc_, d_cmap_, d_redo_, d_redo_ + 1, d_status_, d_walk_abort_, l_lo, l_hi, n,
                       tau2_margin_pct_, dyn, force_tau, predict_pct, chain, resize_mask, test_stall_frame_);
  };
  last_fused_ = fused;
  last_dense_ = dense;
  if (!dense && g.total_tiles > 0) {
    if ((e = hipMemsetAsync(this->d_qstat_, 0, (size_t)n * kOrbLevels * kQStat * 4, st))) return e;
    if ((e = hipMemsetAsync(d_walk_abort_, 0, 4, st))) return e;
  }
  if (fused) {
    const int mask = (1 << (g.nlevels - 1)) - 1;
    const int predict = dyn ? tau_predict_pct_ : 0;
    if (walk_per_level_) {
      for (int l = 0; l < g.nlevels; l++) launch_walk(l, l, 1, mask, predict);
    } else {
      launch_walk(0, g.nlevels - 1, 1, mask, predict);
    }
    hipMemcpyAsync(h_walk_abort_, d_walk_abort_, 8, hipMemcpyDeviceToHost, st);
    if (evs) hipEventRecord(evs[1], st);
  } else {
    for (int l = 1; l < g.nlevels; l++) launch_resize(src, n, l, st);
    if (evs) hipEventRecord(evs[1], st);
    if (g.total_tiles > 0) {
      if (dense) {
        hipLaunchKernelGGL(k_fill_u32, dim3((n * kOrbLevels + 255) / 256), dim3(256), 0, st, tau + (size_t)src.slot0 * kOrbLevels,
                           tau_first + (size_t)src.slot0 * kOrbLevels, (uint32_t)kFastT, n * kOrbLevels);
        hipLaunchKernelGGL(k_fast, dim3((unsigned)g.total_tiles * (unsigned)n), dim3(kFastThreads), 0, st, g, src, d_pyr_,
                           d_cand_cnt_, d_cand_, d_cand_sc_, d_cmap_);
      } else {
        launch_walk(0, g.nlevels - 1, 0, 0, 0);
      }
    }
  }
  if (g.total_tiles > 0 && !dense) {
    hipLaunchKernelGGL(k_fast_check, dim3((unsigned)n * kOrbLevels), dim3(64), 0, st, g, src.slot0, n, tau, tau_first,
                       d_cand_cnt_, d_cand_sc_, d_cmap_, d_redo_, d_redo_ + 1, d_qstat_);
    long long units = (long long)n * kOrbLevels * g.max_level_tiles;
    unsigned grid = (unsigned)(units < 2048 ? units : 2048);
    grid = (grid + 7u) & ~7u;
    hipLaunchKernelGGL(k_fast_redo, dim3(grid), dim3(kFastThreads), 0, st, g, src, d_pyr_, d_redo_, d_redo_ + 1,
                       g.max_level_tiles, d_cand_cnt_, d_cand_, d_cand_sc_, d_cmap_, d_redo_hist_, (const uint32_t*)nullptr);
    hipLaunchKernelGGL(k_redo_thr, dim3((unsigned)std::min<long long>((long long)n * kOrbLevels, 1024)), dim3(64), 0, st, g,
                       src.slot0, d_redo_, d_redo_ + 1, d_cmap_, d_redo_hist_, d_redo_thr_);
    hipLaunchKernelGGL(k_fast_redo, dim3(grid), dim3(kFastThreads), 0, st, g, src, d_pyr_, d_redo_, d_redo_ + 1,
                       g.max_level_tiles, d_cand_cnt_, d_cand_, d_cand_sc_, d_cmap_, (uint32_t*)nullptr, d_redo_thr_);
  }
  if (evs) hipEventRecord(evs[2], st);
  launch_tail(src, n, dense, st, evs);
  return hipGetLastError();
}

void OrbPipeline::launch_resize(const FrameSrc& src, int n, int l, hipStream_t st) {
  const OrbGeometry& g = g_;
  uint8_t* const d_pyr_ = this->d_pyr_ - (ptrdiff_t)src.slot0 * g.pyr_bytes;
  const OrbLevelInfo& L = g.lv[l];
  const int sw16 = (g.lv[l - 1].w + 16 + 15) & ~15;
  const int groups = (L.w + 3) >> 2;
  int rth = 8;
  const int threads = 256;
  while (rth > 4 && ((rth * 5 + 3) / 4 + 3) * sw16 > 60000) rth -= 4;
  const int lds_rows = (rth * 5 + 3) / 4 + 3;
  const uint32_t magic_n16 = (uint32_t)(0x100000000ull / (uint32_t)(sw16 >> 4)) + 1u;
  const uint32_t magic_groups = groups > 1 ? (uint32_t)(0x100000000ull / (uint32_t)groups) + 1u : 0u;
  hipLaunchKernelGGL(resize_shared_[l] ? k_resize<true> : k_resize<false>, dim3((L.h + rth - 1) / rth, n), dim3(threads),
                     (size_t)lds_rows * sw16 + 8 * kResizeMaxRows, st, g, src, d_pyr_, d_tab_, l, rth, lds_rows, magic_n16,
                     magic_groups);
}

void OrbPipeline::launch_tail(const FrameSrc& src, int n, bool dense, hipStream_t st, hipEvent_t* evs) {
  const OrbGeometry& g = g_;
  const ptrdiff_t back = (ptrdiff_t)src.slot0;
  uint8_t* const d_pyr_ = this->d_pyr_ - back * g.pyr_bytes;
  uint32_t* const d_cand_cnt_ = this->d_cand_cnt_ - back * kOrbLevels;
  uint2* const d_cmap_ = this->d_cmap_ - back * kOrbLevels;
  uint32_t* const d_s1_cnt_ = this->d_s1_cnt_ - back * kOrbLevels;
  uint4* const d_s1_ = this->d_s1_ - back * g.s1_total;
  hipLaunchKernelGGL(k_thr_harris, dim3(g.nlevels, n), dim3(dense ? 256 : 64), 0, st, g, src, d_pyr_,
                     d_cand_cnt_, d_cand_, d_cand_sc_, d_cmap_, d_s1_cnt_, d_s1_, d_status_, dense ? 1 : 0);
  if (!dense) {
    const HarrisUnits& hw = harris_;
    const int nu = hw.base[kOrbLevels];
    hipLaunchKernelGGL(k_harris_flat, dim3((nu + 3) / 4, n), dim3(256), 0, st, g, src, d_pyr_, hw, d_s1_cnt_, d_s1_);
  }
  hipLaunchKernelGGL(k_select, dim3(n), dim3(256), 0, st, g, src.slot0, d_s1_cnt_, d_s1_, d_kp_, d_kp_cnt_,
                     d_status_);
  if (evs) hipEventRecord(evs[3], st);
  {
    int bx = 2048 / n;
    bx = bx < 8 ? 8 : bx > 128 ? 128 : bx;
    auto kd = blur_sum256_ ? k_describe<true, true> : half_up_ ? k_describe<true, false> : k_describe<false, false>;
    hipLaunchKernelGGL(kd, dim3(bx, n), dim3(256), 0, st, g, src, d_pyr_, d_kp_, d_kp_cnt_, d_desc_);
  }
  if (evs) hipEventRecord(evs[4], st);
}

std::string OrbPipeline::tail_refusal(int n, const int32_t* counts, const int32_t* cands) const {
  if (n < 1 || n > work_frames_) return "n_frames outside [1, 2*max_batch_pairs]";
  const bool dense = call_force_tau(n) == kFastT;
  int cap[kOrbLevels];
  for (int l = 0; l < kOrbLevels; l++) cap[l] = l < g_.nlevels ? (dense ? g_.lv[l].cand_cap : prim_.cap[l]) : 0;
  return check_tail_lists(g_, cap, n, counts, cands);
}

hipError_t OrbPipeline::tail(const FrameSrc& src, int n, const int32_t* counts, const int32_t* cands, int form,
                             hipStream_t st) {
  if (n <= 0) return hipSuccess;
  if (src.slot0 < 0 || src.slot0 + n > max_slots_ || n > work_frames_) return hipErrorInvalidValue;
  const OrbGeometry& g = g_;
  const bool dense = call_force_tau(n) == kFastT;
  if (dense && (long long)n * g.cand_total > (long long)g.pool_entries) return hipErrorInvalidValue;
  last_src_ = src;
  last_n_ = n;
  last_fused_ = false;
  last_dense_ = true;
  hipError_t e;
  if ((e = hipMemsetAsync(d_status_ + src.slot0, 0, (size_t)n * 4, st))) return e;
  hipLaunchKernelGGL(k_cand_reset, dim3((n * kOrbLevels + 255) / 256), dim3(256), 0, st, g, prim_, this->d_cmap_, n, dense ? 1 : 0);
  hipLaunchKernelGGL(k_fill_u32, dim3((n * kOrbLevels + 255) / 256), dim3(256), 0, st, d_tau_,
                     d_tau_ + (size_t)work_frames_ * kOrbLevels, (uint32_t)kFastT, n * kOrbLevels);
  for (int l = 1; l < g.nlevels; l++) launch_resize(src, n, l, st);
  std::vector<uint2> cmap((size_t)n * kOrbLevels);
  if ((e = hipMemcpyAsync(cmap.data(), this->d_cmap_, cmap.size() * sizeof(uint2), hipMemcpyDeviceToHost, st))) return e;
  if ((e = hipStreamSynchronize(st))) return e;
  size_t total = 0;
  for (int i = 0; i < n * kOrbLevels; i++) total += (size_t)counts[i];
  std::vector<uint32_t> keys(total ? total : 1), cnt((size_t)n * kOrbLevels);
  std::vector<uint8_t> scs(total ? total : 1);
  for (size_t i = 0; i < total; i++) {
    keys[i] = (uint32_t)cands[3 * i] | (uint32_t)cands[3 * i + 1] << 16;
    scs[i] = (uint8_t)cands[3 * i + 2];
  }
  size_t off = 0;
  for (int i = 0; i < n * kOrbLevels; i++) {
    cnt[i] = (uint32_t)counts[i];
    const size_t m = std::min<size_t>(cnt[i], cmap[i].y);
    if (m) {
      if ((e = hipMemcpyAsync(d_cand_ + (size_t)cmap[i].x, keys.data() + off, m * 4, hipMemcpyHostToDevice, st))) break;
      if ((e = hipMemcpyAsync(d_cand_sc_ + (size_t)cmap[i].x, scs.data() + off, m, hipMemcpyHostToDevice, st))) break;
    }
    off += cnt[i];
  }
  if (!e) e = hipMemcpyAsync(this->d_cand_cnt_, cnt.data(), cnt.size() * 4, hipMemcpyHostToDevice, st);
  if (!e) {
    launch_tail(src, n, form == 0, st, nullptr);
    e = hipGetLastError();
  }
  const hipError_t es = hipStreamSynchronize(st);
  return e ? e : es;
}

static int train_chunk() {
  static const int chunk = [] {
    const char* e = getenv("MSF_ORB_TRAIN_CHUNK");
    const int v = e ? atoi(e) : kTrainChunk;
    return v >= 16 && v <= kTrainChunk ? v : kTrainChunk;
  }();
  return chunk;
}

hipError_t OrbPipeline::set_features(int slot, int n, const msf_keypoint* kp, const uint8_t* desc, hipStream_t st) {
  hipError_t e = hipSuccess;
  if (n > 0) {
    e = hipMemcpyAsync(d_kp_ + (size_t)slot * kKpCap, kp, (size_t)n * sizeof(msf_keypoint), hipMemcpyHostToDevice, st);
    if (e != hipSuccess) return e;
    e = hipMemcpyAsync(d_desc_ + (size_t)slot * kKpCap * 32, desc, (size_t)n * 32, hipMemcpyHostToDevice, st);
    if (e != hipSuccess) return e;
  }
  set_words_[0] = (uint32_t)n;
  set_words_[1] = 0u;
  e = hipMemcpyAsync(d_kp_cnt_ + slot, &set_words_[0], sizeof(uint32_t), hipMemcpyHostToDevice, st);
  if (e != hipSuccess) return e;
  return hipMemcpyAsync(d_status_ + slot, &set_words_[1], sizeof(uint32_t), hipMemcpyHostToDevice, st);
}

hipError_t OrbPipeline::match(int n_pairs, const int32_t* d_slot_a, const int32_t* d_slot_b, float ratio,
                              msf_match* d_out, int cap, int32_t* d_n_out, hipStream_t st, int slot_base, int slot_limit) {
  if (n_pairs <= 0) return hipSuccess;
  const int limit = slot_limit > 0 && slot_limit < max_slots_ ? slot_limit : max_slots_;
  if (ev_ok_ && !ev_extract_pending_) {
    ev_begin_call();
    hipEventRecord(ev_[4], st);
  }
  const int chunk = train_chunk();
  const bool split = n_pairs <= kSplitMaxPairs && d_qres_;
  last_match_form_ = split ? 1 : 2;
  if (split)
    hipLaunchKernelGGL(k_match_split, dim3(kSplitBlocks, n_pairs), dim3(256), 0, st, n_pairs, d_slot_a, d_slot_b, d_kp_,
                       d_kp_cnt_, d_desc_, d_status_, ratio, d_out, cap, d_n_out, chunk, d_qres_, d_done_, slot_base, limit);
  else
    hipLaunchKernelGGL(k_match, dim3(n_pairs), dim3(256), 0, st, n_pairs, d_slot_a, d_slot_b, d_kp_, d_kp_cnt_,
                       d_desc_, d_status_, ratio, d_out, cap, d_n_out, chunk, slot_base, limit);
  if (ev_ok_) {
    hipEventRecord(ev_[5], st);
    EvSet& set = evr_[ev_cur_];
    set.recorded = true;
    set.match_only = !ev_extract_pending_;
    ev_extract_pending_ = false;
  }
  return hipGetLastError();
}

void OrbPipeline::ev_begin_call() {
  if (evr_[ev_cur_].recorded) {
    ev_cur_ = (ev_cur_ + 1) % kEvRing;
    if (evr_[ev_cur_].recorded) ev_harvest(ev_cur_);
  }
  ev_ = evr_[ev_cur_].ev;
}

void OrbPipeline::ev_harvest(int i) {
  EvSet& set = evr_[i];
  if (!set.recorded) return;
  set.recorded = false;
  if (hipEventSynchronize(set.ev[5]) != hipSuccess) return;
  for (int k = set.match_only ? 4 : 0; k < 5; k++) {
    float t = 0.f;
    if (hipEventElapsedTime(&t, set.ev[k], set.ev[k + 1]) == hipSuccess) acc_ms_[k] += t;
  }
  if (set.match_only) acc_match_only_++;
  else acc_full_++;
}

int OrbPipeline::stage_times(const char** names, float* ms, int cap) {
  const char* kNames[5] = {last_fused_ ? "pyramid_fast" : "pyramid", "fast_nms", "select_harris", "orient_describe", "match"};
  if (!ev_ok_) return 0;
  for (int k = 0; k < kEvRing; k++) ev_harvest((ev_cur_ + 1 + k) % kEvRing);
  if (acc_full_ + acc_match_only_ == 0) return 0;
  int n = 0;
  for (int i = acc_full_ ? 0 : 4; i < 5 && n < cap; i++, n++) {
    names[n] = kNames[i];
    ms[n] = acc_ms_[i];
  }
  for (auto& a : acc_ms_) a = 0.f;
  acc_full_ = acc_match_only_ = 0;
  return n;
}

int OrbPipeline::debug_get(int what, int slot, int level, void* host_out, size_t cap, size_t* n_bytes,
                           std::string* err) {
  const OrbGeometry& g = g_;
  auto fail = [&](const char* m) { *err = m; return (int)MSF_ERR_INVALID_ARG; };
  auto copy_out = [&](const void* dsrc, size_t bytes) -> int {
    *n_bytes = bytes;
    const size_t n = bytes < cap ? bytes : cap;
    if (n && hipMemcpy(host_out, dsrc, n, hipMemcpyDeviceToHost) != hipSuccess) {
      *err = "hipMemcpy failed in debug_get";
      return (int)MSF_ERR_HIP;
    }
    return 0;
  };
  if (hipDeviceSynchronize() != hipSuccess) { *err = "hipDeviceSynchronize failed"; return MSF_ERR_HIP; }
  if (what == MSF_DBG_LEVEL_SIZES) {
    int32_t v[kOrbLevels][4];
    for (int l = 0; l < kOrbLevels; l++) { v[l][0] = g.lv[l].w; v[l][1] = g.lv[l].h; v[l][2] = g.lv[l].pitch; v[l][3] = g.lv[l].quota; }
    *n_bytes = sizeof(v);
    memcpy(host_out, v, sizeof(v) < cap ? sizeof(v) : cap);
    return 0;
  }
  if (what == MSF_DBG_ORB_MATCH_FORM) {
    const int32_t v[2] = {last_match_form_, train_chunk()};
    *n_bytes = sizeof(v);
    memcpy(host_out, v, sizeof(v) < cap ? sizeof(v) : cap);
    return 0;
  }
  if (what == MSF_DBG_WALK_MODE) {
    uint32_t stalls = 0;
    if (d_walk_abort_ && hipMemcpy(&stalls, d_walk_abort_ + 1, 4, hipMemcpyDeviceToHost) != hipSuccess) {
      *err = "hipMemcpy failed in debug_get";
      return (int)MSF_ERR_HIP;
    }
    const int32_t v[2] = {walk_per_level_ || stalls != 0u ? 1 : 0, (int32_t)stalls};
    *n_bytes = sizeof(v);
    memcpy(host_out, v, sizeof(v) < cap ? sizeof(v) : cap);
    return 0;
  }
  if (slot < 0 || slot >= max_slots_) return fail("slot out of range");
  const int row = slot - last_src_.slot0;
  if (what != MSF_DBG_KEYPOINTS && what != MSF_DBG_DESCRIPTORS && (row < 0 || row >= last_n_))
    return fail("only the frames of the last extraction have a pyramid / candidate lists (per-call workspace)");
  switch (what) {
    case MSF_DBG_LEVEL_PIXELS: {
      if (level < 1 || level >= g.nlevels) return fail("level must be 1..7 (level 0 is the input frame)");
      return copy_out(d_pyr_ + (size_t)row * g.pyr_bytes + g.lv[level].pix_off, (size_t)g.lv[level].pitch * g.lv[level].h);
    }
    case MSF_DBG_FAST_CANDS: {
      if (level < 0 || level >= g.nlevels) return fail("bad level");
      uint32_t n = 0;
      uint2 cm = make_uint2(0u, 0u);
      hipMemcpy(&n, d_cand_cnt_ + (size_t)row * kOrbLevels + level, 4, hipMemcpyDeviceToHost);
      hipMemcpy(&cm, d_cmap_ + (size_t)row * kOrbLevels + level, sizeof(cm), hipMemcpyDeviceToHost);
      if (n > cm.y) n = cm.y;
      std::vector<uint32_t> tk(n);
      std::vector<uint8_t> ts(n);
      if (n) {
        hipMemcpy(tk.data(), d_cand_ + (size_t)cm.x, n * sizeof(uint32_t), hipMemcpyDeviceToHost);
        hipMemcpy(ts.data(), d_cand_sc_ + (size_t)cm.x, n, hipMemcpyDeviceToHost);
      }
      uint32_t tfin = 0;
      hipMemcpy(&tfin, d_tau_ + (size_t)row * kOrbLevels + level, 4, hipMemcpyDeviceToHost);
      uint32_t cut = 0;
      if (!last_dense_ && tfin == (uint32_t)kFastT && level >= 1)
        hipMemcpy(&cut, d_redo_thr_ + (size_t)row * kOrbLevels + level, 4, hipMemcpyDeviceToHost);
      if (cut > 0u) {
        const OrbLevelInfo& L = g.lv[level];
        const size_t cap_l = (size_t)L.cand_cap;
        DevBuf<uint32_t> d_tmp;
        const size_t words = 2 + kOrbLevels + 2 * kOrbLevels + cap_l + (cap_l + 3) / 4;
        if (d_tmp.reserve(words * 4) != hipSuccess) return fail("hipMalloc failed in debug_get");
        if (hipDeviceSynchronize() != hipSuccess) return fail("hipDeviceSynchronize failed in debug_get");
        uint32_t head[2 + kOrbLevels + 2 * kOrbLevels] = {};
        head[0] = 1u;
        head[1] = (uint32_t)(row * kOrbLevels + level);
        head[2 + kOrbLevels + 2 * level] = (uint32_t)(2 + 3 * kOrbLevels);
        head[2 + kOrbLevels + 2 * level + 1] = (uint32_t)cap_l;
        hipMemcpy(d_tmp, head, sizeof(head), hipMemcpyHostToDevice);
        const ptrdiff_t back = (ptrdiff_t)slot * kOrbLevels;
        uint32_t* const cnt = d_tmp + 2 - back;
        const uint2* const map = reinterpret_cast<const uint2*>(d_tmp + 2 + kOrbLevels) - back;
        uint32_t* const keys = d_tmp;
        uint8_t* const scs = reinterpret_cast<uint8_t*>(d_tmp + 2 + 3 * kOrbLevels + cap_l) - (2 + 3 * kOrbLevels);
        const uint8_t* const pyr = d_pyr_ - (ptrdiff_t)last_src_.slot0 * g.pyr_bytes;
        const int tiles = L.tiles_x * L.tiles_y;
        if (tiles > 0)
          hipLaunchKernelGGL(k_fast_redo, dim3((unsigned)((std::min(tiles, 2048) + 7) & ~7)), dim3(kFastThreads), 0, 0, g,
                             last_src_, pyr, d_tmp, d_tmp + 1, tiles, cnt, keys, scs, map, (uint32_t*)nullptr,
                             (const uint32_t*)nullptr);
        hipError_t e2 = hipDeviceSynchronize();
        n = 0;
        if (e2 == hipSuccess) e2 = hipMemcpy(&n, d_tmp + 2 + level, 4, hipMemcpyDeviceToHost);
        if (n > (uint32_t)cap_l) n = (uint32_t)cap_l;
        tk.assign(n, 0u);
        ts.assign(n, 0u);
        if (e2 == hipSuccess && n) {
          e2 = hipMemcpy(tk.data(), d_tmp + 2 + 3 * kOrbLevels, n * sizeof(uint32_t), hipMemcpyDeviceToHost);
          if (e2 == hipSuccess) e2 = hipMemcpy(ts.data(), d_tmp + 2 + 3 * kOrbLevels + cap_l, n, hipMemcpyDeviceToHost);
        }
        if (e2 != hipSuccess) return fail("dense FAST pass failed in debug_get");
      }
      std::vector<int32_t> o;
      o.reserve(n * 3);
      for (uint32_t i = 0; i < n; i++)
        if (tfin <= (uint32_t)kFastT || ts[i] >= tfin) {
          o.push_back(tk[i] & 0xFFFF); o.push_back(tk[i] >> 16); o.push_back(ts[i]);
        }
      *n_bytes = o.size() * 4;
      memcpy(host_out, o.data(), *n_bytes < cap ? *n_bytes : cap);
      return 0;
    }
    case MSF_DBG_FAST_TAU: {
      int32_t v[kOrbLevels][2];
      uint32_t t[2][kOrbLevels];
      hipMemcpy(t[0], d_tau_ + (size_t)row * kOrbLevels, sizeof(t[0]), hipMemcpyDeviceToHost);
      hipMemcpy(t[1], d_tau_ + ((size_t)work_frames_ + row) * kOrbLevels, sizeof(t[1]), hipMemcpyDeviceToHost);
      for (int l = 0; l < kOrbLevels; l++) { v[l][0] = (int32_t)t[0][l]; v[l][1] = (int32_t)t[1][l]; }
      *n_bytes = sizeof(v);
      memcpy(host_out, v, sizeof(v) < cap ? sizeof(v) : cap);
      return 0;
    }
    case MSF_DBG_STAGE1: {
      if (level < 0 || level >= g.nlevels) return fail("bad level");
      uint32_t n = 0;
      hipMemcpy(&n, d_s1_cnt_ + (size_t)row * kOrbLevels + level, 4, hipMemcpyDeviceToHost);
      std::vector<uint4> tmp(n);
      if (n) hipMemcpy(tmp.data(), d_s1_ + (size_t)row * g.s1_total + g.lv[level].s1_off, n * sizeof(uint4), hipMemcpyDeviceToHost);
      std::vector<msf_keypoint> o(n);
      for (uint32_t i = 0; i < n; i++) {
        o[i].lx = tmp[i].x & 0xFFFF; o[i].ly = tmp[i].x >> 16; o[i].x = (float)o[i].lx; o[i].y = (float)o[i].ly;
        memcpy(&o[i].response, &tmp[i].y, 4); o[i].angle = -1.f; o[i].octave = level; o[i].fast_score = tmp[i].z;
      }
      *n_bytes = o.size() * sizeof(msf_keypoint);
      memcpy(host_out, o.data(), *n_bytes < cap ? *n_bytes : cap);
      return 0;
    }
    case MSF_DBG_KEYPOINTS:
    case MSF_DBG_DESCRIPTORS: {
      uint32_t n = 0;
      hipMemcpy(&n, d_kp_cnt_ + slot, 4, hipMemcpyDeviceToHost);
      if (n > (uint32_t)kKpCap) n = kKpCap;
      if (what == MSF_DBG_KEYPOINTS) return copy_out(d_kp_ + (size_t)slot * kKpCap, n * sizeof(msf_keypoint));
      return copy_out(d_desc_ + (size_t)slot * kKpCap * 32, (size_t)n * 32);
    }
    default:
      return fail("unknown debug item for ORB");
  }
}

}
```

### mono_slam_framework_amd/csrc/orb_pipeline.h

```cpp
#pragma once

#include <hip/hip_runtime.h>
#include <stdint.h>

#include <string>
#include <vector>

#include "dev_buf.h"
#include "msf_abi.h"
#include "orb_plan.h"

namespace msf {

constexpr int kOrbStages = 6;

struct FrameSrc {
  const uint8_t* a;
  const uint8_t* b;
  int n_a;
  int slot0;
  long long frame_stride;
  int row_stride;
};

struct OrbOptions {
  int width = 0, height = 0;
  int max_slots = 0;
  int work_frames = 0;
  bool blur_half_up = false;
  bool blur_sum256 = false;
  bool profile = false;
  bool dense_fast = false;
  bool level_size_mul_inv = false;
  int stream_min_frames = 8;
};

class OrbPipeline {
 public:
  OrbPipeline() = default;
  ~OrbPipeline();
  std::string init(const OrbOptions& o);
  void destroy();

  hipError_t extract(const FrameSrc& src, int n_frames, hipStream_t st);
  hipError_t match(int n_pairs, const int32_t* d_slot_a, const int32_t* d_slot_b, float ratio,
                   msf_match* d_out, int cap_per_pair, int32_t* d_n_out, hipStream_t st, int slot_base = 0,
                   int slot_limit = 0);
  hipError_t set_features(int slot, int n, const msf_keypoint* kp, const uint8_t* desc, hipStream_t st);
  hipError_t tail(const FrameSrc& src, int n, const int32_t* counts, const int32_t* cands, int form, hipStream_t st);
  std::string tail_refusal(int n, const int32_t* counts, const int32_t* cands) const;

  const OrbGeometry& geom() const { return g_; }
  int max_slots() const { return max_slots_; }
  int debug_get(int what, int slot, int level, void* host_out, size_t cap, size_t* n_bytes, std::string* err);
  int stage_times(const char** names, float* ms, int cap);
  bool take_degraded_note() { const bool d = degraded_note_; degraded_note_ = false; return d; }
  bool walk_per_level() const { return walk_per_level_; }

 private:
  OrbGeometry g_{};
  OrbPrimLists prim_{};
  HarrisUnits harris_{};
  int max_slots_ = 0;
  int work_frames_ = 0;
  int last_n_ = 0;
  bool half_up_ = false, profile_ = false, blur_sum256_ = false;
  int stream_min_frames_ = 8;
  int force_tau_ = 0;
  DevBuf<uint8_t> d_pyr_;
  DevBuf<uint32_t> d_tab_;
  bool resize_shared_[kOrbLevels] = {};
  DevBuf<uint32_t> d_qstat_;
  DevBuf<uint32_t> d_walk_abort_;
  uint32_t* h_walk_abort_ = nullptr;
  bool degraded_note_ = false;
  int test_stall_calls_ = 0;
  bool fast_two_part_ = true;
  int tau_predict_pct_ = 300;
  bool fused_ = true;
  bool walk_per_level_ = false;
  int test_stall_frame_ = -1;
  int tau2_margin_pct_ = 200;
  bool resize_generic_ = false;
  DevBuf<uint32_t> d_cand_cnt_;
  DevBuf<uint32_t> d_tau_;
  DevBuf<uint32_t> d_redo_;
  DevBuf<uint32_t> d_redo_hist_;
  DevBuf<uint32_t> d_redo_thr_;
  DevBuf<uint32_t> d_cand_;
  DevBuf<uint8_t> d_cand_sc_;
  DevBuf<uint2> d_cmap_;
  DevBuf<uint32_t> d_s1_cnt_;
  DevBuf<uint4> d_s1_;
  DevBuf<msf_keypoint> d_kp_;
  DevBuf<uint8_t> d_desc_;
  DevBuf<uint32_t> d_kp_cnt_;
  DevBuf<uint32_t> d_status_;
  DevBuf<uint32_t> d_qres_;
  DevBuf<uint32_t> d_done_;
  int last_match_form_ = 0;
  uint32_t set_words_[2] = {};
  static constexpr int kEvRing = 32;
  struct EvSet {
    hipEvent_t ev[kOrbStages + 1] = {};
    bool recorded = false, match_only = false;
  };
  EvSet evr_[kEvRing];
  int ev_cur_ = 0;
  hipEvent_t* ev_ = evr_[0].ev;
  float acc_ms_[5] = {};
  int acc_full_ = 0, acc_match_only_ = 0;
  void ev_begin_call();
  void ev_harvest(int i);
  bool ev_ok_ = false, ev_extract_pending_ = false;
  FrameSrc last_src_{};
  bool last_fused_ = false;
  bool last_dense_ = false;
  void read_env();
  hipError_t extract_range(const FrameSrc& src, int n, hipStream_t st, hipEvent_t* evs);
  int call_force_tau(int n) const { return (force_tau_ == 0 && n < stream_min_frames_) ? kFastT : force_tau_; }
  void launch_resize(const FrameSrc& src, int n, int l, hipStream_t st);
  void launch_tail(const FrameSrc& src, int n, bool dense_form, hipStream_t st, hipEvent_t* evs);
};

}
```

### mono_slam_framework_amd/csrc/orb_plan.h

```cpp
#pragma once

#include <math.h>
#include <stdint.h>

#include <algorithm>
#include <string>
#include <vector>

namespace msf {

constexpr int kOrbLevels = 8;
constexpr int kKpCap = 2048;
constexpr int kS1Cap = 8192;

constexpr int kEdge = 31;
constexpr int kFastT = 20;
constexpr int TW = 128, TH = 32;
constexpr int kTileX0 = 16;
constexpr int kDiscTasks = 256;

constexpr int kWkMaxNx = 17;
constexpr int kWkMaxPx = 244;
constexpr int kWkMaxRows = 240;
constexpr int kWkRowsTall = 240, kWkRowsShort = 80, kWkTallMinSlots = 4 * 64;
constexpr int kTauSites = 1024;
constexpr uint32_t kRzNoStore = 0x40000000u;

struct OrbLevelInfo {
  int w, h, pitch;
  int quota;
  float scale;
  int cand_cap;
  int cand_off;
  int s1_off;
  int tiles_x, tiles_y, tile_base;
  int wk_nx, wk_ny, wk_px, wk_rows, wk_base;
  int wk_fused;
  int tab_yemit;
  int tab_xstrip;
  int wk_xg[kWkMaxNx + 1];
  int tab_off;
  int samp_sx, samp_sy, samp_rows, samp_cols;
  long long pix_off;
};

struct OrbPrimLists {
  int cap[kOrbLevels], off[kOrbLevels];
};

struct OrbGeometry {
  int nlevels;
  int w0, h0;
  int total_tiles;
  int total_strips;
  int max_level_tiles;
  int cand_total;
  int prim_total;
  long long pool_base;
  unsigned pool_entries;
  int s1_total;
  long long pyr_bytes;
  OrbLevelInfo lv[kOrbLevels];
  int umax[16];
};
static_assert(sizeof(OrbLevelInfo) == 176,"OrbLevelInfo is a kernel argument: members may not be added or moved");
static_assert(sizeof(OrbGeometry) == 1528, "OrbGeometry is a kernel argument: members may not be added or moved");

struct HarrisUnits {
  int base[kOrbLevels + 1];
  int n[kOrbLevels];
};

struct OrbPlanRequest {
  int width = 0, height = 0;
  int max_slots = 0;
  int work_frames = 0;
  bool level_size_mul_inv = false;
  bool resize_generic = false;
  int force_tau = 0;
  int stream_min_frames = 8;
};

struct OrbPlan {
  OrbGeometry g{};
  OrbPrimLists prim{};
  bool resize_shared[kOrbLevels] = {};
  std::vector<uint32_t> tab;
  std::vector<uint32_t> disc;
  int work_frames = 0;
  HarrisUnits harris{};
};

inline int cv_round_f(float v) { return (int)lrintf(v); }
inline int cv_round_d(double v) { return (int)lrint(v); }

inline void make_table(int src, int dst, uint32_t* tab) {
  const double inv_scale = (double)dst / (double)src;
  const double scale = 1.0 / inv_scale;
  for (int d = 0; d < dst; d++) {
    const double f = scale * ((double)d + 0.5) - 0.5;
    const int i = (int)floor(f);
    if (i >= 0 && src > 1) {
      if (i < src - 1) {
        tab[d] = (uint32_t)i | ((uint32_t)cv_round_d((f - (double)i) * 256.0) << 16);
      } else {
        tab[d] = (uint32_t)(src - 1);
      }
    } else {
      tab[d] = 0;
    }
  }
}

inline std::string plan_orb(const OrbPlanRequest& rq, OrbPlan* out) {
  const int width = rq.width, height = rq.height, max_slots = rq.max_slots, work_frames = rq.work_frames;
  if (width < 64 || height < 64 || width > 8192 || height > 8192) return "arg: ORB image size must be in [64, 8192] x [64, 8192]";
  if (max_slots < 2) return "arg: ORB max_slots < 2";
  *out = OrbPlan();
  out->work_frames = work_frames <= 0 || work_frames > max_slots ? max_slots : work_frames < 2 ? 2 : work_frames;
  OrbGeometry& g = out->g;
  OrbPrimLists& prim_ = out->prim;
  g.nlevels = kOrbLevels;
  g.w0 = width;
  g.h0 = height;
  const float scale_factor_f = 1.2f;
  const double scale_factor = (double)scale_factor_f;
  const int nfeatures = 500;
  {
    const float factor = (float)(1.0 / scale_factor);
    float nd = (float)nfeatures * (1 - factor) / (1 - (float)pow((double)factor, (double)g.nlevels));
    int sum = 0;
    for (int l = 0; l < g.nlevels - 1; l++) {
      g.lv[l].quota = cv_round_f(nd);
      sum += g.lv[l].quota;
      nd *= factor;
    }
    g.lv[g.nlevels - 1].quota = nfeatures - sum > 0 ? nfeatures - sum : 0;
  }
  {
    const int half = 15;
    int umax[17] = {0};
    const int vmax = (int)floor(half * sqrt(2.f) / 2 + 1);
    const int vmin = (int)ceil(half * sqrt(2.f) / 2);
    for (int v = 0; v <= vmax; ++v) umax[v] = cv_round_d(sqrt((double)half * half - v * v));
    for (int v = half, v0 = 0; v >= vmin; --v) {
      while (umax[v0] == umax[v0 + 1]) ++v0;
      umax[v] = v0;
      ++v0;
    }
    for (int v = 0; v < 16; v++) g.umax[v] = umax[v];
  }
  long long pix = 0;
  int cand = 0, prim = 0, tiles = 0, strips = 0, tab = 0, s1 = 0;
  g.max_level_tiles = 0;
  for (int l = 0; l < g.nlevels; l++) {
    OrbLevelInfo& L = g.lv[l];
    const float s = (float)pow(scale_factor, (double)l);
    const float inv = 1.0f / s;
    L.scale = s;
    L.w = rq.level_size_mul_inv ? cv_round_f((float)width * inv) : cv_round_f((float)width / s);
    L.h = rq.level_size_mul_inv ? cv_round_f((float)height * inv) : cv_round_f((float)height / s);
    L.pitch = (L.w + 15) & ~15;
    L.pix_off = pix;
    if (l > 0) pix += (long long)L.pitch * L.h;
    int cap = (int)((long long)L.w * L.h / 8);
    if (cap < 4096) cap = 4096;
    cap = (cap + 15) & ~15;
    L.cand_cap = cap;
    L.cand_off = cand;
    cand += cap;
    int pcap = (int)((long long)L.w * L.h / 64);
    if (pcap < kS1Cap) pcap = kS1Cap;
    pcap = (pcap + 15) & ~15;
    if (pcap > cap || cap <= 16384) pcap = cap;
    prim_.cap[l] = pcap;
    prim_.off[l] = prim;
    prim += pcap;
    L.s1_off = s1;
    s1 += kS1Cap;
    L.tiles_x = L.w > 2 * kEdge ? (L.w - kEdge - kTileX0 + TW - 1) / TW : 0;
    L.tiles_y = L.h > 2 * kEdge ? (L.h - 2 * kEdge + TH - 1) / TH : 0;
    if (L.tiles_x == 0 || L.tiles_y == 0) L.tiles_x = L.tiles_y = 0;
    L.tile_base = tiles;
    tiles += L.tiles_x * L.tiles_y;
    L.wk_nx = L.w > 256 ? (L.w - 256 + kWkMaxPx - 1) / kWkMaxPx + 1 : 1;
    L.wk_px = L.wk_nx > 1 ? (((L.w - 256 + L.wk_nx - 2) / (L.wk_nx - 1)) + 3) & ~3 : kWkMaxPx;
    const int rows_target = max_slots >= kWkTallMinSlots ? kWkRowsTall : kWkRowsShort;
    L.wk_ny = (L.h + rows_target - 1) / rows_target;
    L.wk_rows = (((L.h + L.wk_ny - 1) / L.wk_ny) + 3) & ~3;
    L.wk_ny = (L.h + L.wk_rows - 1) / L.wk_rows;
    L.wk_base = strips;
    strips += L.wk_nx * L.wk_ny;
    L.wk_fused = 0;
    L.tab_yemit = L.tab_xstrip = 0;
    if (L.tiles_x * L.tiles_y > g.max_level_tiles) g.max_level_tiles = L.tiles_x * L.tiles_y;
    L.samp_sx = L.samp_sy = 1;
    L.samp_rows = L.samp_cols = 0;
    if (L.tiles_x > 0) {
      const int rh = L.h - 2 * kEdge;
      const int n_dw = (L.w - kEdge - ((kEdge + 3) & ~3)) >> 2;
      const double s2 = (double)n_dw * rh / (double)kTauSites;
      int sx = (int)(sqrt(s2 > 1.0 ? s2 : 1.0) / 4.0);
      sx = (sx < 1 ? 1 : sx) | 1;
      int sy = (int)(s2 / sx + 0.5);
      sy = sy < 1 ? 1 : sy;
      L.samp_sx = sx;
      L.samp_sy = sy;
      L.samp_rows = (rh + sy - 1) / sy;
      L.samp_cols = n_dw > 0 ? (n_dw + sx - 1) / sx : 0;
      if (L.samp_cols == 0) L.samp_rows = 0;
    }
    L.tab_off = tab;
    if (l > 0) {
      tab += 12 * ((L.w + 3) >> 2) + ((L.h + 3) & ~3);
      L.tab_yemit = tab;
      tab += (g.lv[l - 1].h + 3) & ~3;
      L.tab_xstrip = tab;
      tab += (g.lv[l - 1].wk_nx + 1 + 3) & ~3;
    }
  }
  g.pyr_bytes = (pix + 255) & ~255ll;
  g.cand_total = cand;
  g.prim_total = prim;
  g.s1_total = s1;
// ... 127 lines not shown
```

### mono_slam_framework_amd/matcher.py

```python
import ctypes as C

import numpy as np

from . import _lib


class MsfError(RuntimeError):
    def __init__(self, code, msg):
        super().__init__("msf error %d: %s" % (code, msg))
        self.code = code


def _fill(res, arrays):
    res.struct_size = C.sizeof(type(res))
    for k, v in arrays.items():
        if isinstance(v, np.ndarray):
            setattr(res, k, v.ctypes.data)
        else:
            assert v.is_cuda and v.is_contiguous()
            setattr(res, k, v.data_ptr())
    return res


def _device_lists(d_matches, d_n_out):
# ... 585 lines not shown
        for t, dt in ((d_problems, torch.int32), (d_cam_Tcw, torch.float32), (d_cam_fixed, torch.uint8), (d_points, torch.float32),
                      (d_edge_cam, torch.int32), (d_edge_point, torch.int32), (d_edge_obs, torch.float32)):
            assert t.is_cuda and t.is_contiguous() and t.dtype == dt
        P = d_problems.numel() // 6
        cams, points, edges = d_cam_fixed.numel(), d_points.numel() // 3, d_edge_cam.numel()
        assert d_cam_Tcw.numel() == cams * 12 and d_edge_point.numel() == edges and d_edge_obs.numel() == edges * 2
        if d_stop is not None:
            assert d_stop.is_cuda and d_stop.dtype == torch.int32 and d_stop.numel() == 1
        d = out
        if d is None:
            z = _zeros_on(d_points.device)
            d = {k: z(shape, dt) for k, (shape, dt) in _lib.ba_shapes(P, cams, points, edges).items()}
            if not diagnostics:
                for name, _, per, _ in _lib.BA_ARRAYS:
                    if per.startswith("it"):
                        del d[name]
        res = _fill(_lib.BaResult(), d)
        prm = self._ba_params(K, schedule, huber_delta2, chi2)
        self._check(self._L.msf_bundle_adjust_device(self._h, P, d_problems.data_ptr(), d_cam_Tcw.data_ptr(),
                                                     d_cam_fixed.data_ptr(), d_points.data_ptr(), d_edge_cam.data_ptr(),
                                                     d_edge_point.data_ptr(), d_edge_obs.data_ptr(), cams, points, edges,
                                                     max_free_cams, d_stop.data_ptr() if d_stop is not None else None,
                                                     C.byref(prm), C.byref(res), stream))
        return d

    def global_bundle_adjust(self, cam_Tcw, cam_fixed, points, edge_cam, edge_point, edge_obs, K, schedule=(1, (10, 0), (0, 0)),
                             stop=None, huber_delta2=5.991, chi2=5.991, diagnostics=True):
        tcw = np.ascontiguousarray(cam_Tcw, np.float32).reshape(-1, 12)
        fixed = np.ascontiguousarray(cam_fixed, np.uint8).reshape(-1)
        pts = np.ascontiguousarray(points, np.float32).reshape(-1, 3)
        ec = np.ascontiguousarray(edge_cam, np.int32).reshape(-1)
        ep = np.ascontiguousarray(edge_point, np.int32).reshape(-1)
        obs = np.ascontiguousarray(edge_obs, np.float32).reshape(-1, 2)
        nc, npt, ne = len(tcw), len(pts), len(ec)
        assert len(fixed) == nc and len(ep) == ne and len(obs) == ne
        d = {k: np.zeros(shape, dt) for k, (shape, dt) in _lib.ba_shapes(1, nc, npt, ne).items()}
        if not diagnostics:
            for name, _, per, _ in _lib.BA_ARRAYS:
                if per.startswith("it"):
                    del d[name]
        res = _fill(_lib.BaResult(), d)
        prm = self._ba_params(K, schedule, huber_delta2, chi2)
        if stop is None or isinstance(stop, np.ndarray):
            st = stop
            assert st is None or (st.dtype == np.int32 and st.size == 1)
        else:
            st = np.array([stop], np.int32)
        self._check(self._L.msf_global_bundle_adjust(self._h, nc, tcw.ctypes.data, fixed.ctypes.data, npt, pts.ctypes.data,
                                                     ne, ec.ctypes.data, ep.ctypes.data, obs.ctypes.data,
                                                     st.ctypes.data if st is not None else None, C.byref(prm), C.byref(res)))
        out = dict(d)
        out["status"] = int(d["status"][0])
        out["round_iterations"] = d["round_iterations"][0]
        for name, _, per, _ in _lib.BA_ARRAYS:
            if name not in d:
                continue
            if per == "it":
                out[name] = d[name][0]
            elif per == "it_cam":
                out[name] = d[name].reshape((_lib.BA_SLOTS, nc) + d[name].shape[1:])
            elif per == "it_point":
                out[name] = d[name].reshape((_lib.BA_SLOTS, npt) + d[name].shape[1:])
        return out

    def global_bundle_adjust_device(self, d_cam_Tcw, d_cam_fixed, d_points, d_edge_cam, d_edge_point, d_edge_obs, K,
                                    schedule=(1, (10, 0), (0, 0)), max_free_cams=_lib.GBA_MAX_FREE_CAMS, d_stop=None,
                                    huber_delta2=5.991, chi2=5.991, out=None, diagnostics=True, stream=None):
        import torch
        for t, dt in ((d_cam_Tcw, torch.float32), (d_cam_fixed, torch.uint8), (d_points, torch.float32),
                      (d_edge_cam, torch.int32), (d_edge_point, torch.int32), (d_edge_obs, torch.float32)):
            assert t.is_cuda and t.is_contiguous() and t.dtype == dt
        cams, points, edges = d_cam_fixed.numel(), d_points.numel() // 3, d_edge_cam.numel()
        assert d_cam_Tcw.numel() == cams * 12 and d_edge_point.numel() == edges and d_edge_obs.numel() == edges * 2
        if d_stop is not None:
            assert d_stop.is_cuda and d_stop.dtype == torch.int32 and d_stop.numel() == 1
        d = out
        if d is None:
            z = _zeros_on(d_points.device)
            d = {k: z(shape, dt) for k, (shape, dt) in _lib.ba_shapes(1, cams, points, edges).items()}
            if not diagnostics:
                for name, _, per, _ in _lib.BA_ARRAYS:
                    if per.startswith("it"):
                        del d[name]
        res = _fill(_lib.BaResult(), d)
        prm = self._ba_params(K, schedule, huber_delta2, chi2)
        self._check(self._L.msf_global_bundle_adjust_device(self._h, cams, d_cam_Tcw.data_ptr(), d_cam_fixed.data_ptr(),
                                                            points, d_points.data_ptr(), edges, d_edge_cam.data_ptr(),
                                                            d_edge_point.data_ptr(), d_edge_obs.data_ptr(), max_free_cams,
                                                            d_stop.data_ptr() if d_stop is not None else None,
                                                            C.byref(prm), C.byref(res), stream))
        return d

    def render_match_image(self, frame1, frame2, matches, has_mp1=None, has_mp2=None):
        a, b = self._image(frame1), self._image(frame2)
        m = np.ascontiguousarray(matches, np.int32).reshape(-1, 4)
        f1 = None if has_mp1 is None else np.ascontiguousarray(has_mp1, np.uint8)
        f2 = None if has_mp2 is None else np.ascontiguousarray(has_mp2, np.uint8)
        out = np.zeros((self.height, 2 * self.width, 3), np.uint8)
        self._check(self._L.msf_render_match_image(self._h, C.byref(a), C.byref(b), m.ctypes.data, len(m),
                                                   None if f1 is None else f1.ctypes.data,
                                                   None if f2 is None else f2.ctypes.data, out.ctypes.data,
                                                   out.strides[0]))
        return out

    def store_frame(self, slot, frame):
        img = self._image(frame)
        self._check(self._L.msf_store_frame(self._h, slot, C.byref(img)))

    def match_one_to_many(self, query_slot, slots, with_map_points=False, cap=0):
        slots = np.ascontiguousarray(np.asarray(slots, np.int32).reshape(-1))
        n = slots.size
        num = np.zeros((n,), np.int32)
        nmp = np.zeros((n,), np.int32) if with_map_points else None
        out = np.zeros((n, cap), _lib.MATCH_DTYPE) if cap else None
        self._check(self._L.msf_match_one_to_many(self._h, query_slot, n, slots.ctypes.data, num.ctypes.data,
                                                  nmp.ctypes.data if with_map_points else None,
                                                  out.ctypes.data if cap else None, cap))
        lists = None
        if cap:
            lists = [out[i, :min(max(num[i], 0), cap)].view(np.int32).reshape(-1, 4).copy() for i in range(n)]
        return num, nmp, lists

    def last_error(self):
        return self._L.msf_last_error(self._h).decode()

    def stage_times(self):
        names = (C.c_char_p * 16)()
        ms = (C.c_float * 16)()
        n = self._L.msf_stage_times(self._h, names, ms, 16)
        return {names[i].decode(): float(ms[i]) for i in range(n)}

    def _debug(self, what, slot, level, dtype, cap_bytes):
        buf = np.zeros((cap_bytes,), np.uint8)
        nb = C.c_size_t(0)
        self._check(self._L.msf_debug_get(self._h, what, slot, level, buf.ctypes.data, cap_bytes, C.byref(nb)))
        if nb.value > cap_bytes:
            return self._debug(what, slot, level, dtype, nb.value)
        return buf[:nb.value].view(dtype).copy()


class FeatureMatcher(_Matcher):
    _kind = _lib.MSF_KIND_ORB

    def __init__(self, threshold=0.8, image_width=640, image_height=480, **kw):
        super().__init__(threshold, image_width, image_height, **kw)

    def level_sizes(self):
        return self._debug(_lib.DBG_LEVEL_SIZES, 0, 0, np.int32, 8 * 4 * 4).reshape(8, 4)

    def walk_mode(self):
        v = self._debug(_lib.DBG_WALK_MODE, 0, 0, np.int32, 8)
        return bool(v[0]), int(v[1])

    def walker_launches(self, stage):
        return 8 if (stage == "pyramid_fast" and self.walk_mode()[0]) else 1

    def _slot(self, slot, cache):
        return slot if cache else 2 * self.max_batch_pairs + slot

    def level_pixels(self, slot, level, cache=False):
        w, h, pitch, _ = self.level_sizes()[level]
        return self._debug(_lib.DBG_LEVEL_PIXELS, self._slot(slot, cache), level, np.uint8,
                           int(pitch) * int(h)).reshape(h, pitch)[:, :w]

    def fast_candidates(self, slot, level, cache=False):
        return self._debug(_lib.DBG_FAST_CANDS, self._slot(slot, cache), level, np.int32, 1 << 20).reshape(-1, 3)

    def fast_tau(self, slot, cache=False):
        return self._debug(_lib.DBG_FAST_TAU, self._slot(slot, cache), 0, np.int32, 64).reshape(-1, 2)

    def stage1(self, slot, level, cache=False):
        return self._debug(_lib.DBG_STAGE1, self._slot(slot, cache), level, _lib.KP_DTYPE, 1 << 18)

    def keypoints(self, slot, cache=False):
        return self._debug(_lib.DBG_KEYPOINTS, self._slot(slot, cache), 0, _lib.KP_DTYPE, 2048 * 32)

    def descriptors(self, slot, cache=False):
        return self._debug(_lib.DBG_DESCRIPTORS, self._slot(slot, cache), 0, np.uint8, 2048 * 32).reshape(-1, 32)

    def set_features(self, slot, kp, desc):
        kp = np.asarray(kp)
        if kp.dtype != _lib.KP_DTYPE:
            xy = np.asarray(kp, np.float32).reshape(-1, 2)
            kp = np.zeros(len(xy), _lib.KP_DTYPE)
            kp["x"], kp["y"] = xy[:, 0], xy[:, 1]
        kp = np.ascontiguousarray(kp.reshape(-1))
        desc = np.ascontiguousarray(np.asarray(desc, np.uint8).reshape(-1, 32))
        if len(desc) != len(kp):
            raise ValueError("one descriptor per key point")
        self._check(self._L.msf_debug_orb_set_features(self._h, slot, len(kp), kp.ctypes.data if len(kp) else None,
                                                       desc.ctypes.data if len(kp) else None))

    def orb_tail(self, d_frames, lists, first_slot=0, form=0):
        n = d_frames.shape[0]
        if len(lists) != n:
            raise ValueError("one list of levels per frame")
        counts = np.zeros((n, 8), np.int32)
        rows = []
        for f, levels in enumerate(lists):
            for l, c in enumerate(levels):
                c = np.asarray(c, np.int32).reshape(-1, 3)
                counts[f, l] = len(c)
                rows.append(c)
        cands = np.ascontiguousarray(np.concatenate(rows) if rows else np.zeros((0, 3), np.int32))
        self._check(self._L.msf_debug_orb_tail(self._h, n, d_frames.data_ptr(), d_frames.stride(0), d_frames.stride(1),
                                               first_slot, counts.ctypes.data, cands.ctypes.data if len(cands) else None,
                                               form))

    def match_form(self):
        v = self._debug(_lib.DBG_ORB_MATCH_FORM, 0, 0, np.int32, 8)
        return int(v[0]), int(v[1])


class DNNFeatureMatcher(_Matcher):
    _kind = _lib.MSF_KIND_LOFTR

    def __init__(self, model_file_path=None, threshold=0.15, image_width=640, image_height=480,
                 model_resolution=16, **kw):
        if model_resolution != 16:
            raise MsfError(_lib.MSF_ERR_UNSUPPORTED, "LoFTR_teacher works at 1/16 resolution only")
        super().__init__(threshold, image_width, image_height, weights_path=model_file_path, **kw)

    def conf_matrix(self, pair=0):
        return self._debug(_lib.DBG_LOFTR_CONF, pair, 0, np.float32, 1200 * 1200 * 4).reshape(1200, 1200)

    def coarse_features(self, pair=0):
        return self._debug(_lib.DBG_LOFTR_FEAT, pair, 0, np.float32, 2 * 1200 * 32 * 4).reshape(2, 1200, 32)

    def backbone_tokens(self, pair=0):
        return self._debug(_lib.DBG_LOFTR_TOK, pair, 0, np.float32, 2 * 1200 * 32 * 4).reshape(2, 1200, 32)

    def transformer_device(self, d_in0, d_in1, d_out0, d_out1, first=0, n=8, stream=None):
        import torch
        p = d_in0.shape[0]
        for t in (d_in0, d_in1, d_out0, d_out1):
            assert t.is_cuda and t.dtype == torch.float32 and t.is_contiguous() and tuple(t.shape) == (p, 1200, 32)
        self._check(self._L.msf_debug_loftr_transformer(self._h, p, first, n, d_in0.data_ptr(), d_in1.data_ptr(),
                                                        d_out0.data_ptr(), d_out1.data_ptr(), stream))

    def head_device(self, d_f0, d_f1, d_out, d_n_out, stream=None):
        import torch
        n = d_f0.shape[0]
        for t, dt in ((d_f0, torch.float32), (d_f1, torch.float32), (d_out, torch.int32), (d_n_out, torch.int32)):
            assert t.is_cuda and t.dtype == dt and t.is_contiguous()
        assert tuple(d_f0.shape) == (n, 1200, 32) and d_f1.shape == d_f0.shape
        assert d_out.dim() == 3 and d_out.shape[0] == n and d_out.shape[2] == 4 and tuple(d_n_out.shape) == (n,)
        self._check(self._L.msf_debug_loftr_head(self._h, n, d_f0.data_ptr(), d_f1.data_ptr(), d_out.data_ptr(),
                                                 d_out.shape[1], d_n_out.data_ptr(), stream))

    def backbone_device(self, d_a, d_b, d_tok_a, d_tok_b, act_image=0, frame_stride=None, row_stride=None, n=None,
                        stream=None):
        import torch
        if n is None:
            n = d_a.shape[0]
        row_stride = self.width if row_stride is None else row_stride
        frame_stride = row_stride * self.height if frame_stride is None else frame_stride
        for t in (d_a, d_b):
            assert t is None or (t.is_cuda and t.dtype == torch.uint8 and t.is_contiguous() and t.numel() >= n * frame_stride)
        for t in (d_tok_a,) + ((d_tok_b,) if d_b is not None else ()):
            assert t.is_cuda and t.dtype == torch.float32 and t.is_contiguous() and tuple(t.shape) == (n, 1200, 32)
        self._check(self._L.msf_debug_loftr_backbone(self._h, n, d_a.data_ptr(), None if d_b is None else d_b.data_ptr(),
                                                     frame_stride, row_stride, act_image, d_tok_a.data_ptr(),
                                                     None if d_tok_b is None or d_b is None else d_tok_b.data_ptr(), stream))

    def backbone_activation(self, stage):
        shape = [(8, 240, 320), (16, 120, 160), (32, 60, 80), (32, 30, 40)][stage]
        return self._debug(_lib.DBG_LOFTR_ACT, 0, stage, np.float32, int(np.prod(shape)) * 4).reshape(shape)


class MultiDeviceMatcher:

    def __init__(self, kind, threshold, image_width, image_height, devices=(0,), max_batch_pairs=1, flags=0,
                 weights_path=None):
        self._L = _lib.load()
        self._m = C.c_void_p()
        cfg = _lib.Config()
        self._L.msf_default_config(C.byref(cfg), {"orb": _lib.MSF_KIND_ORB, "loftr": _lib.MSF_KIND_LOFTR}[kind])
        cfg.threshold = threshold
        cfg.image_width = image_width
        cfg.image_height = image_height
        cfg.max_batch_pairs = max_batch_pairs
        cfg.flags = flags
        self._wpath = weights_path.encode() if weights_path else None
        cfg.weights_path = self._wpath
        ids = (C.c_int32 * len(devices))(*devices)
        rc = self._L.msf_multi_create(C.byref(cfg), len(devices), ids, C.byref(self._m))
        if rc != _lib.MSF_OK:
            msg = self._L.msf_multi_last_error(None).decode()
            self._m = C.c_void_p()
            raise MsfError(rc, msg)
        self.devices = tuple(devices)

    def close(self):
        if getattr(self, "_m", None) and self._m.value:
            self._L.msf_multi_destroy(self._m)
            self._m = C.c_void_p()

    def __del__(self):
        try:
            self.close()
        except Exception:
            pass

    def _check(self, rc):
        if rc != _lib.MSF_OK:
            raise MsfError(rc, self._L.msf_multi_last_error(self._m).decode())
# ... 33 lines not shown
```

Measured before the change: 165,900 frame-pairs/sec.

## Fuse per-level threshold and Harris stage-1 into the persistent walker kernel

Adds 'finish' work units to the walker grid. Each one waits until all strips of a level report done, then recounts scores, picks the threshold and computes Harris responses for that level inside the walker, marking a finish flag. The later threshold and Harris kernels check that flag and skip levels already handled. This overlaps stage-1 work with FAST walking of the next level and takes work out of the tail kernels, at the cost of spin-waiting workgroups, extra agent-scope atomic stores, and the risk of stalls if finish units are scheduled before the strips they wait on.

```diff
diff --git a/include/msf_abi.h b/include/msf_abi.h
--- a/include/msf_abi.h
+++ b/include/msf_abi.h
@@ -180,7 +180,8 @@
   MSF_DBG_WALK_MODE = 10,
   MSF_DBG_LOFTR_ACT = 9,
   MSF_DBG_LOFTR_TOK = 11,
-  MSF_DBG_ORB_MATCH_FORM = 12
+  MSF_DBG_ORB_MATCH_FORM = 12,
+  MSF_DBG_WALK_FINISHED = 13
 } msf_debug_what;
 int msf_debug_get(msf_handle* h, int32_t what, int32_t slot, int32_t level,
                   void* host_out, size_t cap_bytes, size_t* n_bytes);
diff --git a/mono_slam_framework_amd/_lib.py b/mono_slam_framework_amd/_lib.py
--- a/mono_slam_framework_amd/_lib.py
+++ b/mono_slam_framework_amd/_lib.py
@@ -27,7 +27,7 @@
 
 (DBG_LEVEL_SIZES, DBG_LEVEL_PIXELS, DBG_FAST_CANDS, DBG_KEYPOINTS, DBG_DESCRIPTORS, DBG_STAGE1,
  DBG_LOFTR_CONF, DBG_LOFTR_FEAT, DBG_FAST_TAU, DBG_LOFTR_ACT, DBG_WALK_MODE, DBG_LOFTR_TOK,
- DBG_ORB_MATCH_FORM) = range(13)
+ DBG_ORB_MATCH_FORM, DBG_WALK_FINISHED) = range(14)
 
 ABI_SYMBOLS = ["msf_abi_version", "msf_default_config", "msf_create", "msf_destroy", "msf_set_threshold",
                "msf_last_error", "msf_match_pair", "msf_match_batch", "msf_match_batch_device",
diff --git a/mono_slam_framework_amd/csrc/orb_kernels.hip b/mono_slam_framework_amd/csrc/orb_kernels.hip
--- a/mono_slam_framework_amd/csrc/orb_kernels.hip
+++ b/mono_slam_framework_amd/csrc/orb_kernels.hip
@@ -409,8 +409,8 @@
 }
 
 constexpr int kTauBins = 64;
-constexpr int kQDone = kTauBins, kQTau = kTauBins + 1, kQFirst = kTauBins + 2, kQAll = kTauBins + 3;
-constexpr int kQStat = kTauBins + 4;
+constexpr int kQDone = kTauBins, kQTau = kTauBins + 1, kQFirst = kTauBins + 2, kQAll = kTauBins + 3, kQFin = kTauBins + 4;
+constexpr int kQStat = kTauBins + 8;
 constexpr uint32_t kQReady = 0x80000000u;
 constexpr int RK = 16;
 constexpr int kSGCap = 288, kSPCap = 256, kSHCap = 64, kSOCap = 64;
@@ -456,6 +456,9 @@
 
 __device__ __forceinline__ uint32_t ld_agent(const uint32_t* p) {
   return __hip_atomic_load(p, __ATOMIC_RELAXED, __HIP_MEMORY_SCOPE_AGENT);
+}
+__device__ __forceinline__ void st_agent(uint32_t* p, uint32_t v) {
+  __hip_atomic_store(p, v, __ATOMIC_RELAXED, __HIP_MEMORY_SCOPE_AGENT);
 }
 __device__ __forceinline__ void unit_stall(uint32_t* status, int slot, uint32_t* abort_word, int lane) {
   if (lane == 0) {
@@ -662,8 +665,8 @@
     for (uint32_t i = lane; i < nO; i += 64) {
       const uint32_t pk = sm.opk[i], sc_ = pk >> 16;
       if (base + i < out_cap) {
-        outk[base + i] = ((uint32_t)(y0 + (int)((pk >> 8) & 255u)) << 16) | (uint32_t)(xs + (int)(pk & 255u));
-        outs[base + i] = (uint8_t)sc_;
+        st_agent(&outk[base + i], ((uint32_t)(y0 + (int)((pk >> 8) & 255u)) << 16) | (uint32_t)(xs + (int)(pk & 255u)));
+        __hip_atomic_store(&outs[base + i], (uint8_t)sc_, __ATOMIC_RELAXED, __HIP_MEMORY_SCOPE_AGENT);
       }
       if (count_me) atomicAdd(&qs[sc_ >> 2], 1u);
     }
@@ -937,11 +940,11 @@
 #undef RZ_HSUM
 #undef RZ_EMIT
   }
-  if (count_me || RESIZE) {
+  {
     asm volatile("s_waitcnt vmcnt(0)" ::: "memory");
     if (lane == 0) {
       if (count_me) atomicAdd(&qs[kQDone], 1u);
-      if (RESIZE) atomicAdd(&qs[kQAll], 1u);
+      atomicAdd(&qs[kQAll], 1u);
     }
   }
 }
@@ -1123,11 +1126,225 @@
     MSF_WAVE_SYNC();
   }
   if (lane == 0) {
-    tau[idx] = (uint32_t)tv;
-    tau_first[idx] = (uint32_t)tv;
+    st_agent(&tau[idx], (uint32_t)tv);
+    st_agent(&tau_first[idx], (uint32_t)tv);
     if (tv <= kFastT && L.tiles_x > 0) redo_list[atomicAdd(redo_cnt, 1u)] = (uint32_t)(fi * kOrbLevels + l);
     __hip_atomic_store(&qs[kQFirst], kQReady | (uint32_t)tv, __ATOMIC_RELAXED, __HIP_MEMORY_SCOPE_AGENT);
   }
+}
+
+template <int RG = 9>
+__device__ __forceinline__ float harris_at(const uint8_t* img, int step, int x0, int y0) {
+  static_assert(9 % RG == 0, "whole groups of rows");
+  const int xb = (x0 - 4) & ~3;
+  const uint32_t o = (uint32_t)(x0 - 4) & 3u;
+  const uint8_t* base = img + (long long)(y0 - 4) * step + xb;
+  constexpr int kWG = 0x000100FF;
+  constexpr int kWH = 0x00010201;
+  int Gm2[7], Gm1[7], Hm2[7], Hm1[7];
+  int a = 0, b = 0, c = 0;
+  auto row = [&](const int t, const uint32_t r0, const uint32_t r1, const uint32_t r2) __attribute__((always_inline)) {
+    const uint32_t d0 = r0 ^ 0x80808080u, d1 = r1 ^ 0x80808080u, d2 = r2 ^ 0x80808080u;
+    const uint32_t w0 = __builtin_amdgcn_alignbyte(d1, d0, o);
+    const uint32_t w1 = __builtin_amdgcn_alignbyte(d2, d1, o);
+    const uint32_t w2 = d2 >> (8u * o);
+    const uint32_t win[7] = {w0, __builtin_amdgcn_alignbyte(w1, w0, 1), __builtin_amdgcn_alignbyte(w1, w0, 2),
+                             __builtin_amdgcn_alignbyte(w1, w0, 3), w1, __builtin_amdgcn_alignbyte(w2, w1, 1),
+                             __builtin_amdgcn_alignbyte(w2, w1, 2)};
+    int G[7], H[7];
+#pragma unroll
+    for (int j = 0; j < 7; j++) {
+      G[j] = __builtin_amdgcn_sdot4((int)win[j], kWG, 0, false);
+      H[j] = __builtin_amdgcn_sdot4((int)win[j], kWH, 0, false);
+    }
+    if (t >= 2) {
+#pragma unroll
+      for (int j = 0; j < 7; j++) {
+        const int Ix = Gm2[j] + 2 * Gm1[j] + G[j];
+        const int Iy = H[j] - Hm2[j];
+        a += Ix * Ix;
+        b += Iy * Iy;
+        c += Ix * Iy;
+      }
+    }
+#pragma unroll
+    for (int j = 0; j < 7; j++) { Gm2[j] = Gm1[j]; Gm1[j] = G[j]; Hm2[j] = Hm1[j]; Hm1[j] = H[j]; }
+  };
+  if (RG == 9) {
+#pragma unroll
+    for (int t = 0; t < 9; t++) {
+      const uint32_t* rp = reinterpret_cast<const uint32_t*>(base + (long long)t * step);
+      row(t, rp[0], rp[1], rp[2]);
+    }
+  } else {
+    uint32_t step_g = (uint32_t)step;
+#pragma unroll
+    for (int t0 = 0; t0 < 9; t0 += RG) {
+      uint32_t ld[RG][3];
+#pragma unroll
+      for (int u = 0; u < RG; u++) {
+        const uint32_t* rp = reinterpret_cast<const uint32_t*>(base + (unsigned long long)((uint32_t)(t0 + u) * step_g));
+        ld[u][0] = rp[0]; ld[u][1] = rp[1]; ld[u][2] = rp[2];
+      }
+#pragma unroll
+      for (int u = 0; u < RG; u++) row(t0 + u, ld[u][0], ld[u][1], ld[u][2]);
+      asm volatile("" : "+v"(step_g) : "v"(a), "v"(b), "v"(c), "v"(Gm1[0]), "v"(Hm1[0]));
+    }
+  }
+  const float scale = 1.f / ((1 << 2) * 7 * 255.f);
+  const float scale_sq_sq = scale * scale * scale * scale;
+  const float fa = (float)a, fb = (float)b, fc = (float)c;
+  return (fa * fb - fc * fc - 0.04f * (fa + fb) * (fa + fb)) * scale_sq_sq;
+}
+
+__device__ __forceinline__ uint32_t count_scores_from(const uint8_t* scs, uint32_t n, uint32_t T, int lane) {
+  uint32_t found = 0;
+  for (uint32_t i = 16u * lane; i < n; i += 16u * 64u) {
+    const uint4 v = *reinterpret_cast<const uint4*>(scs + i);
+    const uint32_t w[4] = {v.x, v.y, v.z, v.w};
+#pragma unroll
+    for (int b = 0; b < 16; b++)
+      if (i + b < n && ((w[b >> 2] >> (8 * (b & 3))) & 255u) >= T) found++;
+  }
+#pragma unroll
+  for (int o = 32; o >= 1; o >>= 1) found += __shfl_xor(found, o);
+  return found;
+}
+
+struct Stage1Smem {
+  uint32_t hist[256];
+  uint32_t thr, lcount;
+};
+template <int RG>
+__device__ __forceinline__ void stage1_from_list(Stage1Smem& S, const OrbGeometry& g, const FrameSrc& src, const uint8_t* pyr,
+                                                 const int l, const int fi, const uint32_t n, const uint2 cm,
+                                                 const uint32_t* cand_key, const uint8_t* cand_sc, uint32_t* s1_cnt,
+                                                 uint4* s1, uint32_t* status, int do_harris, const int tid,
+                                                 const uint32_t nt) {
+  const int slot = src.slot0 + fi;
+  const OrbLevelInfo L = g.lv[l];
+  const uint32_t* keys = cand_key + cm.x;
+  const uint8_t* scs = cand_sc + cm.x;
+  uint4* out = s1 + (long long)slot * g.s1_total + L.s1_off;
+  for (uint32_t b = tid; b < 256u; b += nt) S.hist[b] = 0;
+  if (tid == 0) S.lcount = 0;
+  __syncthreads();
+  for (uint32_t i = 16u * tid; i < n; i += 16u * nt) {
+    const uint4 v = *reinterpret_cast<const uint4*>(scs + i);
+    const uint32_t w[4] = {v.x, v.y, v.z, v.w};
+#pragma unroll
+    for (int b = 0; b < 16; b++)
+      if (i + b < n) atomicAdd(&S.hist[(w[b >> 2] >> (8 * (b & 3))) & 255u], 1u);
+  }
+  __syncthreads();
+  if (tid < 64) {
+    const uint32_t keep = 2u * (uint32_t)L.quota;
+    const uint32_t h0 = S.hist[4 * tid], h1 = S.hist[4 * tid + 1], h2 = S.hist[4 * tid + 2], h3 = S.hist[4 * tid + 3];
+    uint32_t above = h0 + h1 + h2 + h3;
+#pragma unroll
+    for (int o = 1; o < 64; o <<= 1) {
+      const uint32_t up = __shfl_down(above, o);
+      if (tid + o < 64) above += up;
+    }
+    above -= h0 + h1 + h2 + h3;
+    const uint32_t c3 = above + h3, c2 = c3 + h2, c1 = c2 + h1, c0 = c1 + h0;
+    const int mine = c3 >= keep ? 4 * tid + 3 : c2 >= keep ? 4 * tid + 2 : c1 >= keep ? 4 * tid + 1 : c0 >= keep ? 4 * tid : -1;
+    const unsigned long long ok = __ballot(mine >= 0);
+    uint32_t thr = 0;
+    if (n > keep) {
+      thr = 256;
+      if (keep > 0 && ok) thr = (uint32_t)__shfl(mine, 63 - __builtin_clzll(ok));
+    }
+    if (tid == 0) S.thr = thr;
+  }
+  __syncthreads();
+  const uint32_t thr = S.thr;
+  int pitch;
+  const uint8_t* img = level_ptr(g, src, pyr, fi, l, &pitch);
+  for (uint32_t i0 = 0; i0 < n; i0 += 16u * nt) {
+    const uint32_t i = i0 + 16u * tid;
+    uint32_t mask = 0;
+    uint4 v = make_uint4(0u, 0u, 0u, 0u);
+    if (i < n) {
+      v = *reinterpret_cast<const uint4*>(scs + i);
+      const uint32_t w[4] = {v.x, v.y, v.z, v.w};
+#pragma unroll
+      for (int b = 0; b < 16; b++)
+        if (i + b < n && ((w[b >> 2] >> (8 * (b & 3))) & 255u) >= thr) mask |= 1u << b;
+    }
+    if (__ballot(mask != 0u) == 0ull) continue;
+    uint32_t k = reserve_packed(__popc(mask), &S.lcount, tid & 63);
+    const uint32_t w[4] = {v.x, v.y, v.z, v.w};
+    while (mask) {
+      const int b = __ffs(mask) - 1;
+      mask &= mask - 1;
+      if (k < (uint32_t)kS1Cap)
+        out[k] = make_uint4(keys[i + b], 0u, (w[b >> 2] >> (8 * (b & 3))) & 255u, 0u);
+      k++;
+    }
+  }
+  __syncthreads();
+  const uint32_t kept = !do_harris ? 0u : min(S.lcount, (uint32_t)kS1Cap);
+  for (uint32_t i = tid; i < kept; i += nt) {
+    const uint32_t key = out[i].x;
+    const float r = harris_at<RG>(img, pitch, key & 0xFFFF, key >> 16);
+    out[i].y = __float_as_uint(r);
+  }
+  __syncthreads();
+  if (tid == 0) {
+    uint32_t m = S.lcount;
+    if (m > (uint32_t)kS1Cap) { atomicOr(&status[slot], kStatusOverflow); m = kS1Cap; }
+    s1_cnt[slot * kOrbLevels + l] = m;
+  }
+}
+
+using FinishSmem = Stage1Smem;
+static_assert(sizeof(FinishSmem) <= sizeof(StreamSmem), "the finish unit works in the walker's LDS block");
+__device__ __forceinline__ void finish_unit(FinishSmem& S, const OrbGeometry& g, const FrameSrc& src, const uint8_t* pyr,
+                                            uint32_t* tau, uint32_t* tau_first, uint32_t* qstat, uint32_t* cand_cnt,
+                                            const uint32_t* cand_key, const uint8_t* cand_sc, const uint2* cmap,
+                                            uint32_t* redo_cnt, uint32_t* redo_list, uint32_t* s1_cnt, uint4* s1,
+                                            uint32_t* status, uint32_t* abort_word, const int l, const int fi) {
+  const int lane = threadIdx.x, slot = src.slot0 + fi, idx = slot * kOrbLevels + l;
+  uint32_t* const qs = qstat + (size_t)idx * kQStat;
+  const uint32_t n_strips = (uint32_t)(g.lv[l].wk_nx * g.lv[l].wk_ny);
+  uint32_t qx = ld_agent(&qs[kTauBins + (lane & 3)]);
+  bool ready = false;
+  for (uint32_t it = 0; it < kSpinMax; it++) {
+    ready = (uint32_t)__builtin_amdgcn_readlane((int)qx, kQAll - kTauBins) >= n_strips;
+    if (ready || ld_agent(abort_word) != 0u) break;
+    __builtin_amdgcn_s_sleep(20);
+    qx = ld_agent(&qs[kTauBins + (lane & 3)]);
+  }
+  if (!ready) {
+    unit_stall(status, slot, abort_word, lane);
+    return;
+  }
+  __builtin_amdgcn_fence(__ATOMIC_ACQUIRE, "agent");
+  const uint32_t first = (uint32_t)__builtin_amdgcn_readlane((int)qx, kQFirst - kTauBins) & ~kQReady;
+  const uint2 cm = cmap[idx];
+  const uint32_t cnt = ld_agent(&cand_cnt[idx]);
+  const uint32_t n = min(cnt, cm.y);
+  if (first <= (uint32_t)kFastT) {
+    if (g.lv[l].tiles_x > 0) return;
+  } else {
+    const uint32_t T = max(first, ld_agent(&qs[kQTau]));
+    const uint32_t found = count_scores_from(cand_sc + cm.x, n, T, lane);
+    if (cnt > cm.y || found < 2u * (uint32_t)g.lv[l].quota) {
+      if (lane == 0) {
+        st_agent(&tau[idx], (uint32_t)kFastT);
+        st_agent(&cand_cnt[idx], 0u);
+        redo_list[atomicAdd(redo_cnt, 1u)] = (uint32_t)(fi * kOrbLevels + l);
+      }
+      return;
+    }
+    if (lane == 0) {
+      st_agent(&tau[idx], T);
+      st_agent(&tau_first[idx], T);
+    }
+  }
+  stage1_from_list<3>(S, g, src, pyr, l, fi, n, cm, cand_key, cand_sc, s1_cnt, s1, status, 1, lane, 64u);
+  if (lane == 0) st_agent(&qs[kQFin], 1u);
 }
 
 __global__ __launch_bounds__(64) void k_walk(OrbGeometry g, FrameSrc src, uint8_t* pyr, const uint32_t* __restrict__ tab,
@@ -1136,37 +1353,22 @@
                                              uint32_t* redo_cnt, uint32_t* redo_list,
                                              uint32_t* status, uint32_t* abort_word, int l_lo, int l_hi, int n_frames,
                                              int margin_pct, int dyn, int force_tau, int predict_pct, int chain,
-                                             int resize_mask, int test_stall_frame) {
+                                             int resize_mask, int test_stall_frame, int finish, uint32_t* s1_cnt,
+                                             uint4* s1) {
   __shared__ StreamSmem sm;
-  const int xcd = (int)(blockIdx.x & 7u);
-  int r = (int)(blockIdx.x >> 3);
-  const int nf8 = n_frames >> 3, nrem = n_frames & 7;
-  const int nfx = nf8 + (xcd < nrem ? 1 : 0), f0 = xcd * nf8 + (xcd < nrem ? xcd : nrem);
-  int l = l_lo, S = 0;
-  for (;; l++) {
-    if (l > l_hi) return;
-    S = g.lv[l].wk_nx * g.lv[l].wk_ny;
-    const int units = nfx * (1 + S);
-    if (r < units) break;
-    r -= units;
-  }
-  if (r < nfx) {
-    if (f0 + r == test_stall_frame && l == 3) return;
+  const WalkUnit u = walk_unit(g, l_lo, l_hi, n_frames, finish, blockIdx.x);
+  if (u.kind == kWalkNone) return;
+  const int l = u.level, fi = u.frame, ts = u.strip;
+  if (u.kind == kWalkThreshold) {
+    if (fi == test_stall_frame && l == 3) return;
     tau_unit(*reinterpret_cast<TauSmem*>(&sm), g, src, pyr, tau, tau_first, redo_cnt, redo_list, qstat, status, abort_word,
-             force_tau, predict_pct, chain, l, f0 + r);
+             force_tau, predict_pct, chain, l, fi);
     return;
   }
-  r -= nfx;
-  const int Sq = (S + 3) >> 2, Sr = S - Sq;
-  int fi, ts;
-  if (r < nfx * Sq) {
-    fi = f0 + r / Sq;
-    ts = 4 * (r % Sq);
-  } else {
-    r -= nfx * Sq;
-    fi = f0 + r / Sr;
-    const int ip = r % Sr;
-    ts = 4 * (ip / 3) + ip % 3 + 1;
+  if (u.kind == kWalkFinish) {
+    finish_unit(*reinterpret_cast<FinishSmem*>(&sm), g, src, pyr, tau, tau_first, qstat, cand_cnt, cand_key, cand_sc, cmap,
+                redo_cnt, redo_list, s1_cnt, s1, status, abort_word, l, fi);
+    return;
   }
   if ((resize_mask >> l) & 1)
     walk_strip<true>(sm, g, src, pyr, tab, qstat, cand_cnt, cand_key, cand_sc, cmap, status, abort_word, margin_pct, dyn, chain, l, fi, ts);
@@ -1180,6 +1382,7 @@
   const int fi = blockIdx.x / kOrbLevels, l = blockIdx.x - fi * kOrbLevels, lane = threadIdx.x;
   if (fi >= n_frames || l >= g.nlevels) return;
   const int idx = (slot0 + fi) * kOrbLevels + l;
+  if (qstat[(size_t)idx * kQStat + kQFin] != 0u) return;
   if (tau[idx] <= (uint32_t)kFastT) return;
   const uint32_t T = max(tau[idx], qstat[(size_t)idx * kQStat + kQTau]);
   const OrbLevelInfo L = g.lv[l];
@@ -1187,16 +1390,7 @@
   const bool over = cand_cnt[idx] > cm.y;
   const uint32_t n = min(cand_cnt[idx], cm.y);
   const uint8_t* scs = cand_sc + cm.x;
-  uint32_t found = 0;
-  for (uint32_t i = 16u * lane; i < n; i += 16u * 64u) {
-    const uint4 v = *reinterpret_cast<const uint4*>(scs + i);
-    const uint32_t w[4] = {v.x, v.y, v.z, v.w};
-#pragma unroll
-    for (int b = 0; b < 16; b++)
-      if (i + b < n && ((w[b >> 2] >> (8 * (b & 3))) & 255u) >= T) found++;
-  }
-#pragma unroll
-  for (int o = 32; o >= 1; o >>= 1) found += __shfl_xor(found, o);
+  const uint32_t found = count_scores_from(scs, n, T, lane);
   if (lane == 0) {
     if (over || found < 2u * (uint32_t)L.quota) {
       tau[idx] = kFastT;
@@ -1268,142 +1462,27 @@
   }
 }
 
-__device__ __forceinline__ float harris_at(const uint8_t* img, int step, int x0, int y0) {
-  const int xb = (x0 - 4) & ~3;
-  const uint32_t o = (uint32_t)(x0 - 4) & 3u;
-  const uint8_t* base = img + (long long)(y0 - 4) * step + xb;
-  constexpr int kWG = 0x000100FF;
-  constexpr int kWH = 0x00010201;
-  int Gm2[7], Gm1[7], Hm2[7], Hm1[7];
-  int a = 0, b = 0, c = 0;
-#pragma unroll
-  for (int t = 0; t < 9; t++) {
-    const uint32_t* rp = reinterpret_cast<const uint32_t*>(base + (long long)t * step);
-    const uint32_t d0 = rp[0] ^ 0x80808080u, d1 = rp[1] ^ 0x80808080u, d2 = rp[2] ^ 0x80808080u;
-    const uint32_t w0 = __builtin_amdgcn_alignbyte(d1, d0, o);
-    const uint32_t w1 = __builtin_amdgcn_alignbyte(d2, d1, o);
-    const uint32_t w2 = d2 >> (8u * o);
-    const uint32_t win[7] = {w0, __builtin_amdgcn_alignbyte(w1, w0, 1), __builtin_amdgcn_alignbyte(w1, w0, 2),
-                             __builtin_amdgcn_alignbyte(w1, w0, 3), w1, __builtin_amdgcn_alignbyte(w2, w1, 1),
-                             __builtin_amdgcn_alignbyte(w2, w1, 2)};
-    int G[7], H[7];
-#pragma unroll
-    for (int j = 0; j < 7; j++) {
-      G[j] = __builtin_amdgcn_sdot4((int)win[j], kWG, 0, false);
-      H[j] = __builtin_amdgcn_sdot4((int)win[j], kWH, 0, false);
-    }
-    if (t >= 2) {
-#pragma unroll
-      for (int j = 0; j < 7; j++) {
-        const int Ix = Gm2[j] + 2 * Gm1[j] + G[j];
-        const int Iy = H[j] - Hm2[j];
-        a += Ix * Ix;
-        b += Iy * Iy;
-        c += Ix * Iy;
-      }
-    }
-#pragma unroll
-    for (int j = 0; j < 7; j++) { Gm2[j] = Gm1[j]; Gm1[j] = G[j]; Hm2[j] = Hm1[j]; Hm1[j] = H[j]; }
-  }
-  const float scale = 1.f / ((1 << 2) * 7 * 255.f);
-  const float scale_sq_sq = scale * scale * scale * scale;
-  const float fa = (float)a, fb = (float)b, fc = (float)c;
-  return (fa * fb - fc * fc - 0.04f * (fa + fb) * (fa + fb)) * scale_sq_sq;
-}
-
 __global__ __launch_bounds__(256) void k_thr_harris(OrbGeometry g, FrameSrc src, const uint8_t* pyr,
                                                     const uint32_t* cand_cnt, const uint32_t* cand_key,
                                                     const uint8_t* cand_sc, const uint2* cmap,
-                                                    uint32_t* s1_cnt, uint4* s1, uint32_t* status, int do_harris) {
-  __shared__ uint32_t hist[256];
-  __shared__ uint32_t thr_s, lcount;
+                                                    uint32_t* s1_cnt, uint4* s1, uint32_t* status, int do_harris,
+                                                    const uint32_t* fin) {
+  __shared__ Stage1Smem S;
   const int l = blockIdx.x, fi = blockIdx.y, slot = src.slot0 + fi, tid = threadIdx.x;
-  const uint32_t nt = blockDim.x;
   if (l >= g.nlevels) return;
-  const OrbLevelInfo L = g.lv[l];
+  if (fin && fin[(size_t)(slot * kOrbLevels + l) * kQStat + kQFin] != 0u) return;
   uint32_t n = cand_cnt[slot * kOrbLevels + l];
   const uint2 cm = cmap[slot * kOrbLevels + l];
   if (n > cm.y) {
     if (tid == 0) atomicOr(&status[slot], kStatusOverflow);
     n = cm.y;
   }
-  const uint32_t* keys = cand_key + cm.x;
-  const uint8_t* scs = cand_sc + cm.x;
-  uint4* out = s1 + (long long)slot * g.s1_total + L.s1_off;
-  for (uint32_t b = tid; b < 256u; b += nt) hist[b] = 0;
-  if (tid == 0) lcount = 0;
-  __syncthreads();
-  for (uint32_t i = 16u * tid; i < n; i += 16u * nt) {
-    const uint4 v = *reinterpret_cast<const uint4*>(scs + i);
-    const uint32_t w[4] = {v.x, v.y, v.z, v.w};
-#pragma unroll
-    for (int b = 0; b < 16; b++)
-      if (i + b < n) atomicAdd(&hist[(w[b >> 2] >> (8 * (b & 3))) & 255u], 1u);
-  }
-  __syncthreads();
-  if (tid < 64) {
-    const uint32_t keep = 2u * (uint32_t)L.quota;
-    const uint32_t h0 = hist[4 * tid], h1 = hist[4 * tid + 1], h2 = hist[4 * tid + 2], h3 = hist[4 * tid + 3];
-    uint32_t above = h0 + h1 + h2 + h3;
-#pragma unroll
-    for (int o = 1; o < 64; o <<= 1) {
-      const uint32_t up = __shfl_down(above, o);
-      if (tid + o < 64) above += up;
-    }
-    above -= h0 + h1 + h2 + h3;
-    const uint32_t c3 = above + h3, c2 = c3 + h2, c1 = c2 + h1, c0 = c1 + h0;
-    const int mine = c3 >= keep ? 4 * tid + 3 : c2 >= keep ? 4 * tid + 2 : c1 >= keep ? 4 * tid + 1 : c0 >= keep ? 4 * tid : -1;
-    const unsigned long long ok = __ballot(mine >= 0);
-    uint32_t thr = 0;
-    if (n > keep) {
-      thr = 256;
-      if (keep > 0 && ok) thr = (uint32_t)__shfl(mine, 63 - __builtin_clzll(ok));
-    }
-    if (tid == 0) thr_s = thr;
-  }
-  __syncthreads();
-  const uint32_t thr = thr_s;
-  int pitch;
-  const uint8_t* img = level_ptr(g, src, pyr, fi, l, &pitch);
-  for (uint32_t i0 = 0; i0 < n; i0 += 16u * nt) {
-    const uint32_t i = i0 + 16u * tid;
-    uint32_t mask = 0;
-    uint4 v = make_uint4(0u, 0u, 0u, 0u);
-    if (i < n) {
-      v = *reinterpret_cast<const uint4*>(scs + i);
-      const uint32_t w[4] = {v.x, v.y, v.z, v.w};
-#pragma unroll
-      for (int b = 0; b < 16; b++)
-        if (i + b < n && ((w[b >> 2] >> (8 * (b & 3))) & 255u) >= thr) mask |= 1u << b;
-    }
-    if (__ballot(mask != 0u) == 0ull) continue;
-    uint32_t k = reserve_packed(__popc(mask), &lcount, tid & 63);
-    const uint32_t w[4] = {v.x, v.y, v.z, v.w};
-    while (mask) {
-      const int b = __ffs(mask) - 1;
-      mask &= mask - 1;
-      if (k < (uint32_t)kS1Cap)
-        out[k] = make_uint4(keys[i + b], 0u, (w[b >> 2] >> (8 * (b & 3))) & 255u, 0u);
-      k++;
-    }
-  }
-  __syncthreads();
-  const uint32_t kept = !do_harris ? 0u : min(lcount, (uint32_t)kS1Cap);
-  for (uint32_t i = tid; i < kept; i += nt) {
-    const uint32_t key = out[i].x;
-    const float r = harris_at(img, pitch, key & 0xFFFF, key >> 16);
-    out[i].y = __float_as_uint(r);
-  }
-  __syncthreads();
-  if (tid == 0) {
-    uint32_t m = lcount;
-    if (m > (uint32_t)kS1Cap) { atomicOr(&status[slot], kStatusOverflow); m = kS1Cap; }
-    s1_cnt[slot * kOrbLevels + l] = m;
-  }
+  stage1_from_list<9>(S, g, src, pyr, l, fi, n, cm, cand_key, cand_sc, s1_cnt, s1, status, do_harris, tid, blockDim.x);
 }
 
 __global__ __launch_bounds__(256) void k_harris_flat(OrbGeometry g, FrameSrc src, const uint8_t* pyr, HarrisUnits hw,
-                                                     const uint32_t* __restrict__ s1_cnt, uint4* s1) {
+                                                     const uint32_t* __restrict__ s1_cnt, uint4* s1,
+                                                     const uint32_t* fin) {
   const int fi = blockIdx.y, slot = src.slot0 + fi, lane = threadIdx.x & 63;
   const int u = blockIdx.x * 4 + (threadIdx.x >> 6);
   if (u >= hw.base[g.nlevels]) return;
@@ -1411,6 +1490,7 @@
 #pragma unroll
   for (int i = 1; i < kOrbLevels; i++)
     if (i < g.nlevels && u >= hw.base[i]) l = i;
+  if (fin && fin[(size_t)(slot * kOrbLevels + l) * kQStat + kQFin] != 0u) return;
   const OrbLevelInfo L = g.lv[l];
   const uint32_t kept = min(s1_cnt[slot * kOrbLevels + l], (uint32_t)kS1Cap);
   uint4* out = s1 + (long long)slot * g.s1_total + L.s1_off;
@@ -1927,6 +2007,10 @@
   if (getenv("MSF_TEST_HOOKS"))
     if (const char* e = getenv("MSF_ORB_TEST_STALL_FRAME")) test_stall_frame_ = atoi(e);
   if (const char* e = getenv("MSF_ORB_WALK_PER_LEVEL")) walk_per_level_ = atoi(e) != 0;
+  if (const char* e = getenv("MSF_ORB_WALK_FINISH")) {
+    const int v = atoi(e);
+    if (v >= kWalkFinishOff && v <= kWalkFinishQuarter) walk_finish_ = v;
+  }
   if (const char* e = getenv("MSF_ORB_TAU_PREDICT")) {
     const int v = atoi(e);
     if (v >= 0 && v <= 2000) tau_predict_pct_ = v;
@@ -2055,16 +2139,16 @@
   const int dyn = (fast_two_part_ && force_tau == 0) ? 1 : 0;
   bool fused = fused_ && !dense && g.total_tiles > 0;
   for (int l = 1; l < g.nlevels; l++) fused = fused && g.lv[l].wk_fused != 0;
-  auto launch_walk = [&](int l_lo, int l_hi, int chain, int resize_mask, int predict_pct) {
-    long long per_frame = 0;
-    for (int l = l_lo; l <= l_hi; l++) per_frame += 1 + g.lv[l].wk_nx * g.lv[l].wk_ny;
-    const long long wgs = 8ll * ((n + 7) / 8) * per_frame;
+  auto launch_walk = [&](int l_lo, int l_hi, int chain, int resize_mask, int predict_pct, int finish) {
+    const long long wgs = walk_grid(g, l_lo, l_hi, n, finish);
     hipLaunchKernelGGL(k_walk, dim3((unsigned)wgs), dim3(64), 0, st, g, src, d_pyr_, d_tab_, tau, tau_first, d_qstat_,
                        d_cand_cnt_, d_cand_, d_cand_sc_, d_cmap_, d_redo_, d_redo_ + 1, d_status_, d_walk_abort_, l_lo, l_hi, n,
-                       tau2_margin_pct_, dyn, force_tau, predict_pct, chain, resize_mask, test_stall_frame_);
+                       tau2_margin_pct_, dyn, force_tau, predict_pct, chain, resize_mask, test_stall_frame_, finish,
+                       this->d_s1_cnt_ - back * kOrbLevels, this->d_s1_ - back * g.s1_total);
   };
   last_fused_ = fused;
   last_dense_ = dense;
+  last_finish_ = false;
   if (!dense && g.total_tiles > 0) {
     if ((e = hipMemsetAsync(this->d_qstat_, 0, (size_t)n * kOrbLevels * kQStat * 4, st))) return e;
     if ((e = hipMemsetAsync(d_walk_abort_, 0, 4, st))) return e;
@@ -2073,9 +2157,10 @@
     const int mask = (1 << (g.nlevels - 1)) - 1;
     const int predict = dyn ? tau_predict_pct_ : 0;
     if (walk_per_level_) {
-      for (int l = 0; l < g.nlevels; l++) launch_walk(l, l, 1, mask, predict);
+      for (int l = 0; l < g.nlevels; l++) launch_walk(l, l, 1, mask, predict, kWalkFinishOff);
     } else {
-      launch_walk(0, g.nlevels - 1, 1, mask, predict);
+      launch_walk(0, g.nlevels - 1, 1, mask, predict, walk_finish_);
+      last_finish_ = walk_finish_ != kWalkFinishOff;
     }
     hipMemcpyAsync(h_walk_abort_, d_walk_abort_, 8, hipMemcpyDeviceToHost, st);
     if (evs) hipEventRecord(evs[1], st);
@@ -2089,7 +2174,7 @@
         hipLaunchKernelGGL(k_fast, dim3((unsigned)g.total_tiles * (unsigned)n), dim3(kFastThreads), 0, st, g, src, d_pyr_,
                            d_cand_cnt_, d_cand_, d_cand_sc_, d_cmap_);
       } else {
-        launch_walk(0, g.nlevels - 1, 0, 0, 0);
+        launch_walk(0, g.nlevels - 1, 0, 0, 0, kWalkFinishOff);
       }
     }
   }
@@ -2107,7 +2192,7 @@
                        g.max_level_tiles, d_cand_cnt_, d_cand_, d_cand_sc_, d_cmap_, (uint32_t*)nullptr, d_redo_thr_);
   }
   if (evs) hipEventRecord(evs[2], st);
-  launch_tail(src, n, dense, st, evs);
+  launch_tail(src, n, dense, st, evs, !dense && g.total_tiles > 0 ? d_qstat_ : nullptr);
   return hipGetLastError();
 }
 
@@ -2128,7 +2213,7 @@
                      magic_groups);
 }
 
-void OrbPipeline::launch_tail(const FrameSrc& src, int n, bool dense, hipStream_t st, hipEvent_t* evs) {
+void OrbPipeline::launch_tail(const FrameSrc& src, int n, bool dense, hipStream_t st, hipEvent_t* evs, const uint32_t* fin) {
   const OrbGeometry& g = g_;
   const ptrdiff_t back = (ptrdiff_t)src.slot0;
   uint8_t* const d_pyr_ = this->d_pyr_ - back * g.pyr_bytes;
@@ -2137,11 +2222,11 @@
   uint32_t* const d_s1_cnt_ = this->d_s1_cnt_ - back * kOrbLevels;
   uint4* const d_s1_ = this->d_s1_ - back * g.s1_total;
   hipLaunchKernelGGL(k_thr_harris, dim3(g.nlevels, n), dim3(dense ? 256 : 64), 0, st, g, src, d_pyr_,
-                     d_cand_cnt_, d_cand_, d_cand_sc_, d_cmap_, d_s1_cnt_, d_s1_, d_status_, dense ? 1 : 0);
+                     d_cand_cnt_, d_cand_, d_cand_sc_, d_cmap_, d_s1_cnt_, d_s1_, d_status_, dense ? 1 : 0, fin);
   if (!dense) {
     const HarrisUnits& hw = harris_;
     const int nu = hw.base[kOrbLevels];
-    hipLaunchKernelGGL(k_harris_flat, dim3((nu + 3) / 4, n), dim3(256), 0, st, g, src, d_pyr_, hw, d_s1_cnt_, d_s1_);
+    hipLaunchKernelGGL(k_harris_flat, dim3((nu + 3) / 4, n), dim3(256), 0, st, g, src, d_pyr_, hw, d_s1_cnt_, d_s1_, fin);
   }
   hipLaunchKernelGGL(k_select, dim3(n), dim3(256), 0, st, g, src.slot0, d_s1_cnt_, d_s1_, d_kp_, d_kp_cnt_,
                      d_status_);
@@ -2203,7 +2288,7 @@
   }
   if (!e) e = hipMemcpyAsync(this->d_cand_cnt_, cnt.data(), cnt.size() * 4, hipMemcpyHostToDevice, st);
   if (!e) {
-    launch_tail(src, n, form == 0, st, nullptr);
+    launch_tail(src, n, form == 0, st, nullptr, nullptr);
     e = hipGetLastError();
   }
   const hipError_t es = hipStreamSynchronize(st);
@@ -2418,6 +2503,19 @@
       memcpy(host_out, v, sizeof(v) < cap ? sizeof(v) : cap);
       return 0;
     }
+    case MSF_DBG_WALK_FINISHED: {
+      int32_t mask = 0;
+      if (last_finish_) {
+        for (int l = 0; l < g.nlevels; l++) {
+          uint32_t f = 0;
+          hipMemcpy(&f, d_qstat_ + ((size_t)row * kOrbLevels + l) * kQStat + kQFin, 4, hipMemcpyDeviceToHost);
+          if (f) mask |= 1 << l;
+        }
+      }
+      *n_bytes = sizeof(mask);
+      memcpy(host_out, &mask, sizeof(mask) < cap ? sizeof(mask) : cap);
+      return 0;
+    }
     case MSF_DBG_STAGE1: {
       if (level < 0 || level >= g.nlevels) return fail("bad level");
       uint32_t n = 0;
diff --git a/mono_slam_framework_amd/csrc/orb_pipeline.h b/mono_slam_framework_amd/csrc/orb_pipeline.h
--- a/mono_slam_framework_amd/csrc/orb_pipeline.h
+++ b/mono_slam_framework_amd/csrc/orb_pipeline.h
@@ -79,6 +79,8 @@
   int tau_predict_pct_ = 300;
   bool fused_ = true;
   bool walk_per_level_ = false;
+  int walk_finish_ = kWalkFinishThr;
+  bool last_finish_ = false;
   int test_stall_frame_ = -1;
   int tau2_margin_pct_ = 200;
   bool resize_generic_ = false;
@@ -120,7 +122,7 @@
   hipError_t extract_range(const FrameSrc& src, int n, hipStream_t st, hipEvent_t* evs);
   int call_force_tau(int n) const { return (force_tau_ == 0 && n < stream_min_frames_) ? kFastT : force_tau_; }
   void launch_resize(const FrameSrc& src, int n, int l, hipStream_t st);
-  void launch_tail(const FrameSrc& src, int n, bool dense_form, hipStream_t st, hipEvent_t* evs);
+  void launch_tail(const FrameSrc& src, int n, bool dense_form, hipStream_t st, hipEvent_t* evs, const uint32_t* fin);
 };
 
 }
diff --git a/mono_slam_framework_amd/csrc/orb_plan.h b/mono_slam_framework_amd/csrc/orb_plan.h
--- a/mono_slam_framework_amd/csrc/orb_plan.h
+++ b/mono_slam_framework_amd/csrc/orb_plan.h
@@ -70,6 +70,51 @@
   int base[kOrbLevels + 1];
   int n[kOrbLevels];
 };
+
+#if defined(__HIPCC__)
+#define MSF_PLAN_HD __host__ __device__
+#else
+#define MSF_PLAN_HD
+#endif
+constexpr int kWalkNone = 0, kWalkThreshold = 1, kWalkStrip = 2, kWalkFinish = 3;
+constexpr int kWalkFinishOff = 0, kWalkFinishThr = 1, kWalkFinishQuarter = 2;
+struct WalkUnit {
+  int kind, level, frame, strip;
+};
+MSF_PLAN_HD inline WalkUnit walk_unit(const OrbGeometry& g, int l_lo, int l_hi, int n_frames, int finish, unsigned wg) {
+  const int xcd = (int)(wg & 7u);
+  int r = (int)(wg >> 3);
+  const int nf8 = n_frames >> 3, nrem = n_frames & 7;
+  const int nfx = nf8 + (xcd < nrem ? 1 : 0), f0 = xcd * nf8 + (xcd < nrem ? xcd : nrem);
+  for (int l = l_lo; l <= l_hi; l++) {
+    const int S = g.lv[l].wk_nx * g.lv[l].wk_ny;
+    if (r < nfx) return WalkUnit{kWalkThreshold, l, f0 + r, 0};
+    r -= nfx;
+    if (finish == kWalkFinishThr && l > l_lo) {
+      if (r < nfx) return WalkUnit{kWalkFinish, l - 1, f0 + r, 0};
+      r -= nfx;
+    }
+    const int Sq = (S + 3) >> 2, Sr = S - Sq;
+    if (r < nfx * Sq) return WalkUnit{kWalkStrip, l, f0 + r / Sq, 4 * (r % Sq)};
+    r -= nfx * Sq;
+    if (finish == kWalkFinishQuarter && l > l_lo) {
+      if (r < nfx) return WalkUnit{kWalkFinish, l - 1, f0 + r, 0};
+      r -= nfx;
+    }
+    if (r < nfx * Sr) {
+      const int ip = r % Sr;
+      return WalkUnit{kWalkStrip, l, f0 + r / Sr, 4 * (ip / 3) + ip % 3 + 1};
+    }
+    r -= nfx * Sr;
+  }
+  if (finish != kWalkFinishOff && r < nfx) return WalkUnit{kWalkFinish, l_hi, f0 + r, 0};
+  return WalkUnit{kWalkNone, 0, 0, 0};
+}
+inline long long walk_grid(const OrbGeometry& g, int l_lo, int l_hi, int n_frames, int finish) {
+  long long per_frame = 0;
+  for (int l = l_lo; l <= l_hi; l++) per_frame += 1 + g.lv[l].wk_nx * g.lv[l].wk_ny + (finish != kWalkFinishOff ? 1 : 0);
+  return 8ll * ((n_frames + 7) / 8) * per_frame;
+}
 
 struct OrbPlanRequest {
   int width = 0, height = 0;
diff --git a/mono_slam_framework_amd/matcher.py b/mono_slam_framework_amd/matcher.py
--- a/mono_slam_framework_amd/matcher.py
+++ b/mono_slam_framework_amd/matcher.py
@@ -761,6 +761,9 @@
         v = self._debug(_lib.DBG_WALK_MODE, 0, 0, np.int32, 8)
         return bool(v[0]), int(v[1])
 
+    def walk_finished(self, slot, cache=False):
+        return int(self._debug(_lib.DBG_WALK_FINISHED, self._slot(slot, cache), 0, np.int32, 4)[0])
+
     def walker_launches(self, stage):
         return 8 if (stage == "pyramid_fast" and self.walk_mode()[0]) else 1
 
```

Result: faster. 168,900 frame-pairs/sec, median of 6 (+1.8%).
